# ch4r10t33r/zigz

Hardware: AMD Instinct MI355X
Metric: trace steps/sec proved (BabyBear, 2^20 RV64I trace) (higher is better)
Workload: dtype u32

## Files before the change

bindings/zig/zigz_hip.zig:

```

pub const Status = i32;
pub const BABYBEAR_P = 2013265921;
pub const NUM_COLUMNS = 43;
pub const HASH_SIZE = 32;
pub const ABI_VERSION = 1;
pub const NO_MEM_ACCESS = 4294967295;
pub const NO_MEM_ACCESS16 = 134217727;
pub const RCCL_UNIQUE_ID_BYTES = 128;
pub const BATCH_MAX = 4096;
pub const VERIFY_BATCH_MAX = 4194304;

pub const OK: Status = 0;
pub const ERR_EMPTY_EVALUATIONS: Status = 1;
pub const ERR_LENGTH_NOT_POWER_OF_TWO: Status = 2;
pub const ERR_WRONG_NUMBER_OF_VARIABLES: Status = 3;
pub const ERR_NO_VARIABLES_TO_FIX: Status = 4;
pub const ERR_NO_VARIABLES: Status = 5;
pub const ERR_PROTOCOL_ERROR: Status = 6;
pub const ERR_EMPTY_VALUES: Status = 7;
pub const ERR_TOO_MANY_VALUES: Status = 8;
pub const ERR_INDEX_OUT_OF_BOUNDS: Status = 9;
pub const ERR_POINT_DIMENSION_MISMATCH: Status = 10;
pub const ERR_NO_QUERIES: Status = 11;
pub const ERR_TOO_MANY_QUERIES: Status = 12;
// ... 108 lines not shown
    structure_us: f64,
    list_hash_us: f64,
    list_hash_perms: u64,
    top_us: f64,
    top_perms: u64,
    rebuilds: u64,
    eval_constant_columns: u64,
};
pub const BenchResult = extern struct {
    avg_us: f64,
    min_us: f64,
    max_us: f64,
    algorithmic_bytes: u64,
    units: u64,
    launches: u32,
};
pub const LaunchRec = extern struct {
    cls: u32,
    reserved: u32,
    perms: u64,
    start_us: f64,
    end_us: f64,
};

pub extern "c" fn zigz_abi_version() u32;
pub extern "c" fn zigz_status_name(s: Status) [*c]const u8;
pub extern "c" fn zigz_device_count(count: [*c]c_int) Status;
pub extern "c" fn zigz_ctx_create(device: c_int, out: [*c]?*Ctx) Status;
pub extern "c" fn zigz_device_set_blocking_sync(device: c_int, on: c_int) Status;
pub extern "c" fn zigz_ctx_destroy(ctx: ?*Ctx) void;
pub extern "c" fn zigz_last_error(ctx: ?*const Ctx) [*c]const u8;
pub extern "c" fn zigz_ctx_set_stream(ctx: ?*Ctx, hip_stream: ?*anyopaque) Status;
pub extern "c" fn zigz_ctx_get_stream(ctx: ?*Ctx) ?*anyopaque;
pub extern "c" fn zigz_ctx_synchronize(ctx: ?*Ctx) Status;
pub extern "c" fn zigz_dev_alloc(ctx: ?*Ctx, bytes: usize, d_out: [*c]?*anyopaque) Status;
pub extern "c" fn zigz_dev_free(ctx: ?*Ctx, d_ptr: ?*anyopaque) Status;
pub extern "c" fn zigz_ctx_release_workspaces(ctx: ?*Ctx) Status;
pub extern "c" fn zigz_dev_mem_info(ctx: ?*Ctx, free_bytes: [*c]usize, total_bytes: [*c]usize) Status;
pub extern "c" fn zigz_dev_upload_u64(ctx: ?*Ctx, h_in: [*c]const u64, n: usize, d_out: [*c]u32) Status;
pub extern "c" fn zigz_dev_download_u64(ctx: ?*Ctx, d_in: [*c]const u32, n: usize, h_out: [*c]u64) Status;
pub extern "c" fn zigz_mle_bind(ctx: ?*Ctx, in: [*c]const u64, n: usize, r: u64, out: [*c]u64) Status;
pub extern "c" fn zigz_mle_round_poly(ctx: ?*Ctx, in: [*c]const u64, n: usize, out: [*c]u64) Status;
pub extern "c" fn zigz_mle_sum(ctx: ?*Ctx, in: [*c]const u64, n: usize, out: [*c]u64) Status;
pub extern "c" fn zigz_mle_eval(ctx: ?*Ctx, in: [*c]const u64, n: usize, point: [*c]const u64, point_len: usize, out: [*c]u64) Status;
pub extern "c" fn zigz_sumcheck_prove(ctx: ?*Ctx, in: [*c]const u64, n: usize, rounds: [*c]u64, point: [*c]u64, final_eval: [*c]u64) Status;
pub extern "c" fn zigz_sumcheck_prove_interactive(ctx: ?*Ctx, in: [*c]const u64, n: usize, challenges: [*c]const u64, n_challenges: usize, rounds: [*c]u64, point: [*c]u64, final_eval: [*c]u64) Status;
pub extern "c" fn zigz_merkle_commit(ctx: ?*Ctx, values: [*c]const u64, n: usize, root: [*c]u8, height: [*c]usize, out: [*c]?*Merkle) Status;
pub extern "c" fn zigz_merkle_open(ctx: ?*Ctx, tree: ?*const Merkle, index: usize, siblings: [*c]u8, dirs: [*c]u8, leaf_value: [*c]u64) Status;
pub extern "c" fn zigz_merkle_destroy(ctx: ?*Ctx, tree: ?*Merkle) void;
pub extern "c" fn zigz_commit_open(ctx: ?*Ctx, evals: [*c]const u64, n: usize, tree: ?*const Merkle, point: [*c]const u64, point_len: usize, value: [*c]u64, index: [*c]u64, siblings: [*c]u8, dirs: [*c]u8, leaf_value: [*c]u64) Status;
pub extern "c" fn zigz_commit_begin(ctx: ?*Ctx, cols: [*c]const u64, ncols: usize, col_stride: usize, nv: usize, out: [*c]?*CommitJob) Status;
pub extern "c" fn zigz_commit_begin_dev(ctx: ?*Ctx, d_cols: [*c]const u32, ncols: usize, col_stride: usize, nv: usize, out: [*c]?*CommitJob) Status;
pub extern "c" fn zigz_commit_begin_batch(ctx: ?*Ctx, d_cols: [*c][*c]u32, nproofs: usize, ncols: usize, col_stride: usize, nv: usize, out: [*c]?*CommitJob) Status;
pub extern "c" fn zigz_commit_roots(job: ?*CommitJob, roots: [*c]u8) Status;
pub extern "c" fn zigz_commit_open_all(job: ?*CommitJob, points: [*c]const u64, values: [*c]u64, indices: [*c]u64, leaves: [*c]u64, siblings: [*c]u8, dirs: [*c]u8) Status;
pub extern "c" fn zigz_commit_job_tree(job: ?*CommitJob, d_tree: [*c]?*anyopaque, bytes_per_column: [*c]usize) Status;
pub extern "c" fn zigz_commit_end(job: ?*CommitJob) void;
pub extern "c" fn zigz_lasso_prove(ctx: ?*Ctx, table: [*c]const u64, table_rows: usize, queries: [*c]const u64, n_queries: usize, n_in: usize, n_out: usize, nv_out: [*c]usize, rounds: [*c]u64, point: [*c]u64, final_eval: [*c]u64, query_commitment: [*c]u8, table_commitment: [*c]u8) Status;
pub extern "c" fn zigz_lasso_prove_with_mapping(ctx: ?*Ctx, table: [*c]const u64, table_rows: usize, queries: [*c]const u64, n_queries: usize, n_in: usize, n_out: usize, mapping: [*c]const u64, n_mapping: usize, nv_out: [*c]usize, rounds: [*c]u64, point: [*c]u64, final_eval: [*c]u64, query_commitment: [*c]u8, table_commitment: [*c]u8) Status;
pub extern "c" fn zigz_lasso_fingerprints(ctx: ?*Ctx, rows_in: [*c]const u64, rows: usize, width: usize, out: [*c]u64) Status;
pub extern "c" fn zigz_dev_reduce_u64(ctx: ?*Ctx, h_in: [*c]const u64, n: usize, d_out: [*c]u32) Status;
pub extern "c" fn zigz_dev_witness_from_rows(ctx: ?*Ctx, h_rows: [*c]const u64, num_steps: usize, nv: usize, d_cols: [*c]u32, col_stride: usize) Status;
pub extern "c" fn zigz_dev_witness_from_steps(ctx: ?*Ctx, h_steps: [*c]const TraceStep, num_steps: usize, nv: usize, initial_regs: [*c]const u64, d_cols: [*c]u32, col_stride: usize) Status;
pub extern "c" fn zigz_dev_witness_from_steps_async(ctx: ?*Ctx, h_steps: [*c]const TraceStep, num_steps: usize, nv: usize, initial_regs: [*c]const u64, d_cols: [*c]u32, col_stride: usize) Status;
pub extern "c" fn zigz_dev_witness_from_steps_ws(ctx: ?*Ctx, h_steps: [*c]const TraceStep, num_steps: usize, nv: usize, initial_regs: [*c]const u64, d_cols: [*c][*c]u32, col_stride: [*c]usize) Status;
pub extern "c" fn zigz_dev_witness_from_steps32(ctx: ?*Ctx, h_steps: [*c]const TraceStep32, num_steps: usize, h_mem: [*c]const MemAccess, num_mem: usize, nv: usize, initial_regs: [*c]const u64, d_cols: [*c]u32, col_stride: usize) Status;
pub extern "c" fn zigz_dev_witness_from_steps32_ws(ctx: ?*Ctx, h_steps: [*c]const TraceStep32, num_steps: usize, h_mem: [*c]const MemAccess, num_mem: usize, nv: usize, initial_regs: [*c]const u64, d_cols: [*c][*c]u32, col_stride: [*c]usize) Status;
pub extern "c" fn zigz_dev_witness_from_steps16(ctx: ?*Ctx, h_steps: [*c]const TraceStep16, num_steps: usize, h_mem: [*c]const MemAccess, num_mem: usize, code_base: u64, h_code: [*c]const CodeEntry, num_code: usize, nv: usize, initial_regs: [*c]const u64, d_cols: [*c]u32, col_stride: usize) Status;
pub extern "c" fn zigz_dev_witness_from_steps16_ws(ctx: ?*Ctx, h_steps: [*c]const TraceStep16, num_steps: usize, h_mem: [*c]const MemAccess, num_mem: usize, code_base: u64, h_code: [*c]const CodeEntry, num_code: usize, nv: usize, initial_regs: [*c]const u64, d_cols: [*c][*c]u32, col_stride: [*c]usize) Status;
pub extern "c" fn zigz_host_register(ctx: ?*Ctx, h_ptr: ?*anyopaque, bytes: usize) Status;
pub extern "c" fn zigz_host_unregister(ctx: ?*Ctx, h_ptr: ?*anyopaque) Status;
pub extern "c" fn zigz_dev_mle_bind(ctx: ?*Ctx, d_in: [*c]const u32, n: usize, r: u64, d_out: [*c]u32) Status;
pub extern "c" fn zigz_dev_mle_bind_sums(ctx: ?*Ctx, d_in: [*c]const u32, n: usize, r: u64, d_out: [*c]u32, half_sums: [*c]u64) Status;
pub extern "c" fn zigz_dev_mle_half_sums(ctx: ?*Ctx, d_in: [*c]const u32, n: usize, half_sums: [*c]u64) Status;
pub extern "c" fn zigz_dev_mle_eval(ctx: ?*Ctx, d_in: [*c]const u32, n: usize, point: [*c]const u64, point_len: usize, out: [*c]u64) Status;
pub extern "c" fn zigz_dev_sumcheck_prove(ctx: ?*Ctx, d_in: [*c]const u32, n: usize, d_scratch: [*c]u32, fixed_challenges: [*c]const u64, rounds: [*c]u64, point: [*c]u64, final_eval: [*c]u64) Status;
pub extern "c" fn zigz_dev_sumcheck_prove_sharded(ctx: ?*Ctx, d_local: [*c]const u32, n_local: usize, rank: c_int, world: c_int, allgather: AllgatherFn, user: ?*anyopaque, rounds: [*c]u64, point: [*c]u64, final_eval: [*c]u64) Status;
pub extern "c" fn zigz_shm_comm_create(name: [*c]const u8, rank: c_int, world: c_int, max_bytes: usize, timeout_s: f64, out: [*c]?*ShmComm) Status;
pub extern "c" fn zigz_shm_allgather(comm: ?*anyopaque, send: ?*const anyopaque, bytes: usize, recv: ?*anyopaque) c_int;
pub extern "c" fn zigz_shm_comm_destroy(comm: ?*ShmComm) void;
pub extern "c" fn zigz_rccl_unique_id(id: [*c]u8) Status;
pub extern "c" fn zigz_rccl_comm_create(device: c_int, id: [*c]const u8, rank: c_int, world: c_int, max_bytes: usize, out: [*c]?*RcclComm) Status;
pub extern "c" fn zigz_rccl_allgather(comm: ?*anyopaque, send: ?*const anyopaque, bytes: usize, recv: ?*anyopaque) c_int;
pub extern "c" fn zigz_rccl_allreduce_u64(comm: ?*RcclComm, send: [*c]const u64, n: usize, recv: [*c]u64) c_int;
pub extern "c" fn zigz_rccl_allreduce_u64_dev(comm: ?*RcclComm, d_words: [*c]u64, n: usize, hip_stream: ?*anyopaque) c_int;
pub extern "c" fn zigz_rccl_stream_wait(comm: ?*RcclComm, hip_stream: ?*anyopaque) c_int;
pub extern "c" fn zigz_rccl_comm_set_timeout(comm: ?*RcclComm, seconds: f64) void;
pub extern "c" fn zigz_rccl_comm_abort(comm: ?*RcclComm) void;
pub extern "c" fn zigz_rccl_comm_rank(comm: ?*const RcclComm) c_int;
pub extern "c" fn zigz_rccl_comm_world(comm: ?*const RcclComm) c_int;
pub extern "c" fn zigz_rccl_comm_destroy(comm: ?*RcclComm) void;
pub extern "c" fn zigz_dev_sumcheck_prove_rccl(ctx: ?*Ctx, d_local: [*c]const u32, n_local: usize, comm: ?*RcclComm, rounds: [*c]u64, point: [*c]u64, final_eval: [*c]u64) Status;
pub extern "c" fn zigz_sumcheck_radix_run(ops: [*c]const RadixOps, n_local: usize, rank: c_int, world: c_int, allgather: AllgatherFn, comm_user: ?*anyopaque, fixed_challenges: [*c]const u64, rounds: [*c]u64, point: [*c]u64, final_eval: [*c]u64) Status;
pub extern "c" fn zigz_sumcheck_radix_run_reduced(ops: [*c]const RadixOps, n_local: usize, rank: c_int, world: c_int, allgather: AllgatherFn, comm_user: ?*anyopaque, fixed_challenges: [*c]const u64, rounds: [*c]u64, point: [*c]u64, final_eval: [*c]u64) Status;
pub extern "c" fn zigz_dev_sumcheck_prove_batch(ctx: ?*Ctx, d_tables: [*c][*c]u32, ns: [*c]const usize, k: usize, fixed_challenges: [*c]const u64, rounds: [*c]u64, points: [*c]u64, final_evals: [*c]u64, bad_index: [*c]usize) Status;
pub extern "c" fn zigz_sumcheck_prove_batch(ctx: ?*Ctx, tables: [*c][*c]u64, ns: [*c]const usize, k: usize, fixed_challenges: [*c]const u64, rounds: [*c]u64, points: [*c]u64, final_evals: [*c]u64, bad_index: [*c]usize) Status;
pub extern "c" fn zigz_lasso_prove_batch(ctx: ?*Ctx, k: usize, tables: [*c][*c]u64, table_rows: [*c]const usize, queries: [*c][*c]u64, n_queries: [*c]const usize, n_in: [*c]const usize, n_out: [*c]const usize, mappings: [*c][*c]u64, n_mappings: [*c]const usize, nv_out: [*c]usize, rounds: [*c][*c]u64, points: [*c][*c]u64, final_evals: [*c]u64, query_commitments: [*c]u8, table_commitments: [*c]u8, bad_index: [*c]usize) Status;
pub extern "c" fn zigz_sumcheck_radix_run_batch(user: ?*anyopaque, block_sums: RadixBatchSumsFn, fold: RadixBatchFoldFn, read_tail: RadixBatchTailFn, k: usize, ns: [*c]const usize, fixed_challenges: [*c]const u64, rounds: [*c]u64, points: [*c]u64, final_evals: [*c]u64) Status;
pub extern "c" fn zigz_dev_merkle_commit_batch(ctx: ?*Ctx, d_values: [*c][*c]u32, ns: [*c]const usize, k: usize, roots: [*c]u8, heights: [*c]usize, out: [*c]?*MerkleBatch, bad_index: [*c]usize) Status;
pub extern "c" fn zigz_merkle_commit_batch(ctx: ?*Ctx, values: [*c][*c]u64, ns: [*c]const usize, k: usize, roots: [*c]u8, heights: [*c]usize, out: [*c]?*MerkleBatch, bad_index: [*c]usize) Status;
pub extern "c" fn zigz_merkle_open_batch(ctx: ?*Ctx, b: ?*const MerkleBatch, indices: [*c]const u64, siblings: [*c]u8, dirs: [*c]u8, leaf_values: [*c]u64, bad_index: [*c]usize) Status;
pub extern "c" fn zigz_commit_open_batch(ctx: ?*Ctx, b: ?*const MerkleBatch, points: [*c]const u64, values: [*c]u64, indices: [*c]u64, siblings: [*c]u8, dirs: [*c]u8, leaf_values: [*c]u64, bad_index: [*c]usize) Status;
pub extern "c" fn zigz_merkle_batch_destroy(ctx: ?*Ctx, b: ?*MerkleBatch) void;
pub extern "c" fn zigz_merkle_verify_batch(ctx: ?*Ctx, k: usize, roots: [*c]const u8, heights: [*c]const usize, leaf_values: [*c]const u64, siblings: [*c]const u8, dirs: [*c]const u8, verdicts: [*c]u8, n_rejected: [*c]usize, bad_index: [*c]usize) Status;
pub extern "c" fn zigz_dev_merkle_verify_batch(ctx: ?*Ctx, k: usize, d_roots: [*c]const u8, heights: [*c]const usize, d_leaf_values: [*c]const u64, d_siblings: [*c]const u8, d_dirs: [*c]const u8, verdicts: [*c]u8, n_rejected: [*c]usize, bad_index: [*c]usize) Status;
pub extern "c" fn zigz_transcript_new() ?*Transcript;
// ... 20 lines not shown
```

include/zigz_hip.h:

```cpp
#ifndef ZIGZ_HIP_H
#define ZIGZ_HIP_H

#include <stddef.h>
#include <stdint.h>

#ifdef __cplusplus
extern "C" {
#endif

#define ZIGZ_BABYBEAR_P 2013265921ull
#define ZIGZ_NUM_COLUMNS 43
#define ZIGZ_HASH_SIZE 32
#define ZIGZ_ABI_VERSION 1

typedef int32_t zigz_status;
enum {
    ZIGZ_OK = 0,
    ZIGZ_ERR_EMPTY_EVALUATIONS = 1,
    ZIGZ_ERR_LENGTH_NOT_POWER_OF_TWO = 2,
    ZIGZ_ERR_WRONG_NUMBER_OF_VARIABLES = 3,
    ZIGZ_ERR_NO_VARIABLES_TO_FIX = 4,
    ZIGZ_ERR_NO_VARIABLES = 5,
    ZIGZ_ERR_PROTOCOL_ERROR = 6,
    ZIGZ_ERR_EMPTY_VALUES = 7,
// ... 16 lines not shown
    ZIGZ_ERR_COMM = 105
};

typedef struct zigz_ctx zigz_ctx;
typedef struct zigz_merkle zigz_merkle;
typedef struct zigz_commit_job zigz_commit_job;
typedef struct zigz_transcript zigz_transcript;
typedef struct zigz_merkle_batch zigz_merkle_batch;

uint32_t zigz_abi_version(void);
const char *zigz_status_name(zigz_status s);
zigz_status zigz_device_count(int *count);
zigz_status zigz_ctx_create(int device, zigz_ctx **out);
zigz_status zigz_device_set_blocking_sync(int device, int on);
void zigz_ctx_destroy(zigz_ctx *ctx);
const char *zigz_last_error(const zigz_ctx *ctx);
zigz_status zigz_ctx_set_stream(zigz_ctx *ctx, void *hip_stream);
void *zigz_ctx_get_stream(zigz_ctx *ctx);
zigz_status zigz_ctx_synchronize(zigz_ctx *ctx);
zigz_status zigz_dev_alloc(zigz_ctx *ctx, size_t bytes, void **d_out);
zigz_status zigz_dev_free(zigz_ctx *ctx, void *d_ptr);
zigz_status zigz_ctx_release_workspaces(zigz_ctx *ctx);
zigz_status zigz_dev_mem_info(zigz_ctx *ctx, size_t *free_bytes, size_t *total_bytes);
zigz_status zigz_dev_upload_u64(zigz_ctx *ctx, const uint64_t *h_in, size_t n, uint32_t *d_out);
zigz_status zigz_dev_download_u64(zigz_ctx *ctx, const uint32_t *d_in, size_t n, uint64_t *h_out);

zigz_status zigz_mle_bind(zigz_ctx *ctx, const uint64_t *in, size_t n, uint64_t r, uint64_t *out);
zigz_status zigz_mle_round_poly(zigz_ctx *ctx, const uint64_t *in, size_t n, uint64_t out[2]);
zigz_status zigz_mle_sum(zigz_ctx *ctx, const uint64_t *in, size_t n, uint64_t *out);
zigz_status zigz_mle_eval(zigz_ctx *ctx, const uint64_t *in, size_t n, const uint64_t *point,
                          size_t point_len, uint64_t *out);

zigz_status zigz_sumcheck_prove(zigz_ctx *ctx, const uint64_t *in, size_t n, uint64_t *rounds,
                                uint64_t *point, uint64_t *final_eval);
zigz_status zigz_sumcheck_prove_interactive(zigz_ctx *ctx, const uint64_t *in, size_t n,
                                            const uint64_t *challenges, size_t n_challenges,
                                            uint64_t *rounds, uint64_t *point, uint64_t *final_eval);

zigz_status zigz_merkle_commit(zigz_ctx *ctx, const uint64_t *values, size_t n, uint8_t root[32],
                               size_t *height, zigz_merkle **out);
zigz_status zigz_merkle_open(zigz_ctx *ctx, const zigz_merkle *tree, size_t index, uint8_t *siblings,
                             uint8_t *dirs, uint64_t *leaf_value);
void zigz_merkle_destroy(zigz_ctx *ctx, zigz_merkle *tree);
zigz_status zigz_commit_open(zigz_ctx *ctx, const uint64_t *evals, size_t n, const zigz_merkle *tree,
                             const uint64_t *point, size_t point_len, uint64_t *value, uint64_t *index,
                             uint8_t *siblings, uint8_t *dirs, uint64_t *leaf_value);

zigz_status zigz_commit_begin(zigz_ctx *ctx, const uint64_t *cols, size_t ncols, size_t col_stride,
                              size_t nv, zigz_commit_job **out);
zigz_status zigz_commit_begin_dev(zigz_ctx *ctx, const uint32_t *d_cols, size_t ncols, size_t col_stride,
                                  size_t nv, zigz_commit_job **out);
zigz_status zigz_commit_begin_batch(zigz_ctx *ctx, const uint32_t *const *d_cols, size_t nproofs, size_t ncols,
                                    size_t col_stride, size_t nv, zigz_commit_job **out);
zigz_status zigz_commit_roots(zigz_commit_job *job, uint8_t *roots);
zigz_status zigz_commit_open_all(zigz_commit_job *job, const uint64_t *points, uint64_t *values,
                                 uint64_t *indices, uint64_t *leaves, uint8_t *siblings, uint8_t *dirs);
zigz_status zigz_commit_job_tree(zigz_commit_job *job, const void **d_tree, size_t *bytes_per_column);
void zigz_commit_end(zigz_commit_job *job);

zigz_status zigz_lasso_prove(zigz_ctx *ctx, const uint64_t *table, size_t table_rows, const uint64_t *queries,
                             size_t n_queries, size_t n_in, size_t n_out, size_t *nv_out, uint64_t *rounds,
                             uint64_t *point, uint64_t *final_eval, uint8_t query_commitment[32],
                             uint8_t table_commitment[32]);
zigz_status zigz_lasso_prove_with_mapping(zigz_ctx *ctx, const uint64_t *table, size_t table_rows,
                                          const uint64_t *queries, size_t n_queries, size_t n_in, size_t n_out,
                                          const uint64_t *mapping, size_t n_mapping, size_t *nv_out,
                                          uint64_t *rounds, uint64_t *point, uint64_t *final_eval,
                                          uint8_t query_commitment[32], uint8_t table_commitment[32]);
zigz_status zigz_lasso_fingerprints(zigz_ctx *ctx, const uint64_t *rows_in, size_t rows, size_t width,
                                    uint64_t *out);

zigz_status zigz_dev_reduce_u64(zigz_ctx *ctx, const uint64_t *h_in, size_t n, uint32_t *d_out);
zigz_status zigz_dev_witness_from_rows(zigz_ctx *ctx, const uint64_t *h_rows, size_t num_steps, size_t nv,
                                       uint32_t *d_cols, size_t col_stride);

typedef struct zigz_trace_step {
    uint64_t pc;
    uint64_t rd_value;
    uint64_t mem_addr;
    uint64_t mem_value;
    int64_t imm;
    uint8_t opcode, rd, rs1, rs2, funct3, funct7;
    uint8_t wr_reg;
    uint8_t mem_is_read;
} zigz_trace_step;
zigz_status zigz_dev_witness_from_steps(zigz_ctx *ctx, const zigz_trace_step *h_steps, size_t num_steps, size_t nv,
                                        const uint64_t *initial_regs, uint32_t *d_cols, size_t col_stride);
zigz_status zigz_dev_witness_from_steps_async(zigz_ctx *ctx, const zigz_trace_step *h_steps, size_t num_steps, size_t nv,
                                              const uint64_t *initial_regs, uint32_t *d_cols, size_t col_stride);
zigz_status zigz_dev_witness_from_steps_ws(zigz_ctx *ctx, const zigz_trace_step *h_steps, size_t num_steps, size_t nv,
                                           const uint64_t *initial_regs, const uint32_t **d_cols, size_t *col_stride);
typedef struct zigz_trace_step32 {
    uint64_t pc;
    uint64_t rd_value;
    int32_t imm;
    uint32_t mem_index;
    uint8_t opcode, rd, rs1, rs2, funct3, funct7;
    uint8_t wr_reg;
    uint8_t mem_is_read;
} zigz_trace_step32;
typedef struct zigz_mem_access {
    uint64_t addr, value;
} zigz_mem_access;
#define ZIGZ_NO_MEM_ACCESS 4294967295
zigz_status zigz_dev_witness_from_steps32(zigz_ctx *ctx, const zigz_trace_step32 *h_steps, size_t num_steps,
                                          const zigz_mem_access *h_mem, size_t num_mem, size_t nv, const uint64_t *initial_regs,
// ... 190 lines not shown
```

zigz_amd/_ffi.py:

```python
import ctypes as C
import os

HERE = os.path.dirname(os.path.abspath(__file__))
LIB_PATH = os.path.join(HERE, "lib", "libzigz_hip.so")

if not os.path.exists(LIB_PATH):
    raise ImportError(
        f"{LIB_PATH} is missing: build it with `python -m zigz_amd.build` (hipcc, --offload-arch=gfx950). "
        "zigz_amd has no CPU fallback.")

lib = C.CDLL(LIB_PATH, mode=C.RTLD_GLOBAL)

u64p = C.POINTER(C.c_uint64)
u32p = C.POINTER(C.c_uint32)
u8p = C.POINTER(C.c_uint8)
szp = C.POINTER(C.c_size_t)
vp = C.c_void_p


class LaunchRec(C.Structure):
    _fields_ = [("cls", C.c_uint32), ("reserved", C.c_uint32), ("perms", C.c_uint64), ("start_us", C.c_double), ("end_us", C.c_double)]


class KernelStats(C.Structure):
# ... 11 lines not shown
                ("small_domain_fallback_waves", C.c_uint64),
                ("structure_us", C.c_double), ("list_hash_us", C.c_double), ("list_hash_perms", C.c_uint64),
                ("top_us", C.c_double), ("top_perms", C.c_uint64), ("rebuilds", C.c_uint64),
                ("eval_constant_columns", C.c_uint64)]


class BenchResult(C.Structure):
    _fields_ = [("avg_us", C.c_double), ("min_us", C.c_double), ("max_us", C.c_double), ("algorithmic_bytes", C.c_uint64),
                ("units", C.c_uint64), ("launches", C.c_uint32)]


ALLGATHER_FN = C.CFUNCTYPE(C.c_int, vp, vp, C.c_size_t, vp)
RADIX_BLOCK_SUMS_FN = C.CFUNCTYPE(C.c_int32, vp, C.c_uint, u64p)
RADIX_FOLD_FN = C.CFUNCTYPE(C.c_int32, vp, C.c_uint, u64p, C.c_uint, u64p)
RADIX_READ_TAIL_FN = C.CFUNCTYPE(C.c_int32, vp, C.c_size_t, u64p)


class RadixOps(C.Structure):
    _fields_ = [("user", vp), ("block_sums", RADIX_BLOCK_SUMS_FN), ("fold", RADIX_FOLD_FN), ("read_tail", RADIX_READ_TAIL_FN)]


RB_BLOCK_SUMS_FN = C.CFUNCTYPE(C.c_int32, vp, C.c_size_t, szp, C.POINTER(C.c_uint), u64p)
RB_FOLD_FN = C.CFUNCTYPE(C.c_int32, vp, C.c_size_t, szp, C.POINTER(C.c_uint), u64p, C.POINTER(C.c_uint), u64p)
RB_READ_TAIL_FN = C.CFUNCTYPE(C.c_int32, vp, C.c_size_t, szp, szp, u64p)


SIGNATURES = {
    "zigz_abi_version": (C.c_uint32, []),
    "zigz_status_name": (C.c_char_p, [C.c_int32]),
    "zigz_device_count": (C.c_int32, [C.POINTER(C.c_int)]),
    "zigz_ctx_create": (C.c_int32, [C.c_int, C.POINTER(vp)]),
    "zigz_ctx_destroy": (None, [vp]),
    "zigz_last_error": (C.c_char_p, [vp]),
    "zigz_ctx_set_stream": (C.c_int32, [vp, vp]),
    "zigz_ctx_get_stream": (vp, [vp]),
    "zigz_ctx_synchronize": (C.c_int32, [vp]),
    "zigz_dev_alloc": (C.c_int32, [vp, C.c_size_t, C.POINTER(vp)]),
    "zigz_dev_free": (C.c_int32, [vp, vp]),
    "zigz_dev_upload_u64": (C.c_int32, [vp, u64p, C.c_size_t, vp]),
    "zigz_dev_download_u64": (C.c_int32, [vp, vp, C.c_size_t, u64p]),
    "zigz_mle_bind": (C.c_int32, [vp, u64p, C.c_size_t, C.c_uint64, u64p]),
    "zigz_mle_round_poly": (C.c_int32, [vp, u64p, C.c_size_t, u64p]),
    "zigz_mle_sum": (C.c_int32, [vp, u64p, C.c_size_t, u64p]),
    "zigz_mle_eval": (C.c_int32, [vp, u64p, C.c_size_t, u64p, C.c_size_t, u64p]),
    "zigz_sumcheck_prove": (C.c_int32, [vp, u64p, C.c_size_t, u64p, u64p, u64p]),
    "zigz_sumcheck_prove_interactive": (C.c_int32, [vp, u64p, C.c_size_t, u64p, C.c_size_t, u64p, u64p, u64p]),
    "zigz_merkle_commit": (C.c_int32, [vp, u64p, C.c_size_t, u8p, szp, C.POINTER(vp)]),
    "zigz_merkle_open": (C.c_int32, [vp, vp, C.c_size_t, u8p, u8p, u64p]),
    "zigz_merkle_destroy": (None, [vp, vp]),
    "zigz_commit_open": (C.c_int32, [vp, u64p, C.c_size_t, vp, u64p, C.c_size_t, u64p, u64p, u8p, u8p, u64p]),
    "zigz_commit_begin": (C.c_int32, [vp, u64p, C.c_size_t, C.c_size_t, C.c_size_t, C.POINTER(vp)]),
    "zigz_commit_begin_dev": (C.c_int32, [vp, vp, C.c_size_t, C.c_size_t, C.c_size_t, C.POINTER(vp)]),
    "zigz_commit_begin_batch": (C.c_int32, [vp, C.POINTER(vp), C.c_size_t, C.c_size_t, C.c_size_t, C.c_size_t, C.POINTER(vp)]),
    "zigz_commit_roots": (C.c_int32, [vp, u8p]),
    "zigz_commit_open_all": (C.c_int32, [vp, u64p, u64p, u64p, u64p, u8p, u8p]),
    "zigz_commit_job_tree": (C.c_int32, [vp, C.POINTER(vp), C.POINTER(C.c_size_t)]),
    "zigz_commit_end": (None, [vp]),
    "zigz_lasso_prove": (C.c_int32, [vp, u64p, C.c_size_t, u64p, C.c_size_t, C.c_size_t, C.c_size_t, szp, u64p, u64p,
                                     u64p, u8p, u8p]),
    "zigz_lasso_prove_with_mapping": (C.c_int32, [vp, u64p, C.c_size_t, u64p, C.c_size_t, C.c_size_t, C.c_size_t, u64p,
                                                  C.c_size_t, szp, u64p, u64p, u64p, u8p, u8p]),
    "zigz_lasso_fingerprints": (C.c_int32, [vp, u64p, C.c_size_t, C.c_size_t, u64p]),
    "zigz_dev_reduce_u64": (C.c_int32, [vp, u64p, C.c_size_t, vp]),
    "zigz_dev_witness_from_rows": (C.c_int32, [vp, u64p, C.c_size_t, C.c_size_t, vp, C.c_size_t]),
    "zigz_dev_witness_from_steps": (C.c_int32, [vp, vp, C.c_size_t, C.c_size_t, u64p, vp, C.c_size_t]),
    "zigz_dev_witness_from_steps_async": (C.c_int32, [vp, vp, C.c_size_t, C.c_size_t, u64p, vp, C.c_size_t]),
    "zigz_dev_witness_from_steps32": (C.c_int32, [vp, vp, C.c_size_t, vp, C.c_size_t, C.c_size_t, u64p, vp, C.c_size_t]),
    "zigz_dev_witness_from_steps32_ws": (C.c_int32, [vp, vp, C.c_size_t, vp, C.c_size_t, C.c_size_t, u64p, C.POINTER(vp), szp]),
    "zigz_dev_witness_from_steps16": (C.c_int32, [vp, vp, C.c_size_t, vp, C.c_size_t, C.c_uint64, vp, C.c_size_t, C.c_size_t, u64p, vp, C.c_size_t]),
    "zigz_dev_witness_from_steps16_ws": (C.c_int32, [vp, vp, C.c_size_t, vp, C.c_size_t, C.c_uint64, vp, C.c_size_t, C.c_size_t, u64p,
                                                     C.POINTER(vp), szp]),
    "zigz_dev_witness_from_steps_ws": (C.c_int32, [vp, vp, C.c_size_t, C.c_size_t, u64p, C.POINTER(vp), szp]),
    "zigz_dev_mem_info": (C.c_int32, [vp, szp, szp]),
    "zigz_ctx_set_epoch": (C.c_int32, [vp, vp]),
    "zigz_ctx_launch_log": (C.c_int32, [vp, C.POINTER(LaunchRec), C.c_size_t, szp]),
    "zigz_ctx_release_workspaces": (C.c_int32, [vp]),
    "zigz_host_register": (C.c_int32, [vp, vp, C.c_size_t]),
    "zigz_host_unregister": (C.c_int32, [vp, vp]),
    "zigz_dev_mle_bind": (C.c_int32, [vp, vp, C.c_size_t, C.c_uint64, vp]),
    "zigz_dev_mle_bind_sums": (C.c_int32, [vp, vp, C.c_size_t, C.c_uint64, vp, u64p]),
    "zigz_dev_mle_half_sums": (C.c_int32, [vp, vp, C.c_size_t, u64p]),
    "zigz_dev_mle_eval": (C.c_int32, [vp, vp, C.c_size_t, u64p, C.c_size_t, u64p]),
    "zigz_dev_sumcheck_prove": (C.c_int32, [vp, vp, C.c_size_t, vp, u64p, u64p, u64p, u64p]),
    "zigz_dev_sumcheck_prove_sharded": (C.c_int32, [vp, vp, C.c_size_t, C.c_int, C.c_int, ALLGATHER_FN, vp, u64p, u64p, u64p]),
    "zigz_sumcheck_radix_run": (C.c_int32, [C.POINTER(RadixOps), C.c_size_t, C.c_int, C.c_int, ALLGATHER_FN, vp, u64p, u64p,
                                            u64p, u64p]),
    "zigz_sumcheck_radix_run_reduced": (C.c_int32, [C.POINTER(RadixOps), C.c_size_t, C.c_int, C.c_int, ALLGATHER_FN, vp, u64p, u64p,
                                                    u64p, u64p]),
    "zigz_shm_comm_create": (C.c_int32, [C.c_char_p, C.c_int, C.c_int, C.c_size_t, C.c_double, C.POINTER(vp)]),
    "zigz_shm_allgather": (C.c_int, [vp, vp, C.c_size_t, vp]),
    "zigz_shm_comm_destroy": (None, [vp]),
    "zigz_rccl_unique_id": (C.c_int32, [u8p]),
    "zigz_rccl_comm_create": (C.c_int32, [C.c_int, u8p, C.c_int, C.c_int, C.c_size_t, C.POINTER(vp)]),
    "zigz_rccl_allgather": (C.c_int, [vp, vp, C.c_size_t, vp]),
    "zigz_rccl_allreduce_u64": (C.c_int, [vp, u64p, C.c_size_t, u64p]),
    "zigz_rccl_allreduce_u64_dev": (C.c_int, [vp, vp, C.c_size_t, vp]),
    "zigz_rccl_stream_wait": (C.c_int, [vp, vp]),
    "zigz_rccl_comm_set_timeout": (None, [vp, C.c_double]),
    "zigz_rccl_comm_abort": (None, [vp]),
    "zigz_rccl_comm_rank": (C.c_int, [vp]),
    "zigz_rccl_comm_world": (C.c_int, [vp]),
    "zigz_rccl_comm_destroy": (None, [vp]),
    "zigz_dev_sumcheck_prove_batch": (C.c_int32, [vp, C.POINTER(vp), szp, C.c_size_t, u64p, u64p, u64p, u64p, szp]),
    "zigz_sumcheck_prove_batch": (C.c_int32, [vp, C.POINTER(u64p), szp, C.c_size_t, u64p, u64p, u64p, u64p, szp]),
    "zigz_lasso_prove_batch": (C.c_int32, [vp, C.c_size_t, C.POINTER(u64p), szp, C.POINTER(u64p), szp, szp, szp, C.POINTER(u64p), szp,
                                           szp, C.POINTER(u64p), C.POINTER(u64p), u64p, u8p, u8p, szp]),
# ... 36 lines not shown
```

zigz_amd/build.py:

```python
import os
import shutil
import subprocess
import sys

HERE = os.path.dirname(os.path.abspath(__file__))
ROOT = os.path.dirname(HERE)
CSRC = os.path.join(HERE, "csrc")
LIB = os.path.join(HERE, "lib")
OBJ = os.path.join(HERE, "build")
INC = os.path.join(ROOT, "include")
ARCH = "gfx950"


def _hipcc():
    for c in (shutil.which("hipcc"), "/opt/rocm/bin/hipcc"):
        if c and os.path.exists(c):
            return c
    raise RuntimeError("hipcc not found: the HIP backend cannot be built")


def _newer(target, sources):
    if not os.path.exists(target):
        return True
    t = os.path.getmtime(target)
    return any(os.path.getmtime(s) > t for s in sources)


def _run(cmd):
    print("+", " ".join(cmd), flush=True)
    subprocess.check_call(cmd)


def _headers():
    hs = [os.path.join(INC, f) for f in os.listdir(INC) if f.endswith(".h")]
    for d, _, fs in os.walk(CSRC):
        hs += [os.path.join(d, f) for f in fs if f.endswith(".hpp")]
    return hs


def _host_cxx():
    for c in ("/opt/rocm/lib/llvm/bin/clang++", "/opt/rocm/bin/amdclang++"):
        if os.path.exists(c):
            return c
    return "g++"


def build_hip(force=False):
    os.makedirs(LIB, exist_ok=True)
    os.makedirs(OBJ, exist_ok=True)
    hipcc = _hipcc()
    hdrs = _headers()
    objs = []
    extra = os.environ.get("ZIGZ_EXTRA_HIPCC_FLAGS", "").split()
    units = [
        ("kernels.hip", [hipcc, f"--offload-arch={ARCH}", "-O3", "-std=c++17", "-fPIC", f"-I{INC}", f"-I{CSRC}"] + extra),
        ("merkle_levels.hip", [hipcc, f"--offload-arch={ARCH}", "-O3", "-std=c++17", "-fPIC", f"-I{INC}", f"-I{CSRC}"] + extra),
        ("sumcheck_batch.hip", [hipcc, f"--offload-arch={ARCH}", "-O3", "-std=c++17", "-fPIC", f"-I{INC}", f"-I{CSRC}"] + extra),
        ("merkle_batch.hip", [hipcc, f"--offload-arch={ARCH}", "-O3", "-std=c++17", "-fPIC", f"-I{INC}", f"-I{CSRC}"] + extra),
        ("merkle_verify.hip", [hipcc, f"--offload-arch={ARCH}", "-O3", "-std=c++17", "-fPIC", f"-I{INC}", f"-I{CSRC}"] + extra),
        ("api.cpp", [hipcc, "-O3", "-std=c++17", "-fPIC", f"-I{INC}", f"-I{CSRC}"]),
        ("api_mle.cpp", [hipcc, "-O3", "-std=c++17", "-fPIC", f"-I{INC}", f"-I{CSRC}"]),
        ("api_commit.cpp", [hipcc, "-O3", "-std=c++17", "-fPIC", f"-I{INC}", f"-I{CSRC}"]),
        ("api_misc.cpp", [hipcc, "-O3", "-std=c++17", "-fPIC", f"-I{INC}", f"-I{CSRC}"]),
        ("api_batch.cpp", [hipcc, "-O3", "-std=c++17", "-fPIC", "-pthread", f"-I{INC}", f"-I{CSRC}"]),
        ("api_merkle_batch.cpp", [hipcc, "-O3", "-std=c++17", "-fPIC", "-pthread", f"-I{INC}", f"-I{CSRC}"]),
        ("api_merkle_verify.cpp", [hipcc, "-O3", "-std=c++17", "-fPIC", "-pthread", f"-I{INC}", f"-I{CSRC}"]),
        ("host_hash.cpp", [_host_cxx(), "-O3", "-std=c++17", "-fPIC", f"-I{CSRC}"]),
        ("host_keccak_avx512.cpp", [_host_cxx(), "-O3", "-std=c++17", "-fPIC", f"-I{CSRC}"]),
        ("host_keccak_bmi.cpp", [_host_cxx(), "-O3", "-std=c++17", "-fPIC", f"-I{CSRC}"]),
        ("host_keccak_avx512vl.cpp", [_host_cxx(), "-O3", "-std=c++17", "-fPIC", f"-I{CSRC}"]),
        ("host_sponge_batch.cpp", [_host_cxx(), "-O3", "-std=c++17", "-fPIC", "-pthread", f"-I{CSRC}"]),
        ("shm_comm.cpp", [_host_cxx(), "-O2", "-std=c++17", "-fPIC", f"-I{INC}", f"-I{CSRC}"]),
        ("rccl_comm.cpp", [hipcc, "-O2", "-std=c++17", "-fPIC", f"-I{INC}", f"-I{CSRC}", "-I/opt/rocm/include"]),
    ]
    for src, cmd in units:
        s = os.path.join(CSRC, src)
        o = os.path.join(OBJ, src.replace(".", "_") + ".o")
        if force or _newer(o, [s] + hdrs):
            _run(cmd + ["-c", s, "-o", o])
        objs.append(o)
    so = os.path.join(LIB, "libzigz_hip.so")
    if force or _newer(so, objs):
        _run([hipcc, f"--offload-arch={ARCH}", "-shared", "-fPIC", "-o", so] + objs + ["-lrt", "-pthread", "-ldl"])
    return so


def build_host(force=False):
    hdir = os.path.join(CSRC, "host")
    if not os.path.isdir(hdir):
        return None
    srcs = sorted(os.path.join(hdir, f) for f in os.listdir(hdir) if f.endswith(".cpp"))
    if not srcs:
        return None
    so = os.path.join(LIB, "libzigz_host.so")
    if force or _newer(so, srcs + _headers() + [os.path.join(LIB, "libzigz_hip.so")]):
        _run(["g++", "-O3", "-std=c++17", "-fPIC", "-pthread", "-shared", f"-I{INC}", f"-I{CSRC}", "-o", so] + srcs +
             [f"-L{LIB}", "-lzigz_hip", "-Wl,-rpath,$ORIGIN"])
    return so


def build_all(force=False):
    a = build_hip(force)
    b = build_host(force)
    return a, b


if __name__ == "__main__":
    print(build_all("--force" in sys.argv))
```

zigz_amd/csrc/api.cpp:

```cpp
#include "api_internal.hpp"

using namespace zk;

void set_err(zigz_ctx *ctx, const char *fmt, ...) {
    if (!ctx) return;
    va_list ap;
    va_start(ap, fmt);
    vsnprintf(ctx->err, sizeof(ctx->err), fmt, ap);
    va_end(ap);
}

zigz_status ws_get(zigz_ctx *ctx, int slot, size_t bytes, void **out) {
    if (bytes == 0) bytes = 16;
    if (ctx->ws_bytes[slot] < bytes) {
        if (ctx->ws[slot]) {
            HIPCHK(ctx, hipStreamSynchronize(ctx->stream));
            HIPCHK(ctx, hipFree(ctx->ws[slot]));
            ctx->ws[slot] = nullptr;
            ctx->ws_bytes[slot] = 0;
        }
        size_t want = align256(bytes + bytes / 8);
        hipError_t e = hipMalloc(&ctx->ws[slot], want);
        if (e != hipSuccess) {
            (void)hipGetLastError();
// ... 249 lines not shown
            ctx->ws[i] = nullptr;
            ctx->ws_bytes[i] = 0;
        }
    ctx->cons_table = nullptr;
    ctx->cons_table_bytes = 0;
    return ZIGZ_OK;
}
extern "C" zigz_status zigz_dev_mem_info(zigz_ctx *ctx, size_t *free_bytes, size_t *total_bytes) {
    ZIGZ_ENTER(ctx);
    if (!ctx || !free_bytes || !total_bytes) return ZIGZ_ERR_INVALID_ARGUMENT;
    HIPCHK(ctx, hipMemGetInfo(free_bytes, total_bytes));
    return ZIGZ_OK;
}
extern "C" zigz_status zigz_dev_free(zigz_ctx *ctx, void *d_ptr) {
    ZIGZ_ENTER(ctx);
    if (!ctx) return ZIGZ_ERR_INVALID_ARGUMENT;
    HIPCHK(ctx, hipStreamSynchronize(ctx->stream));
    HIPCHK(ctx, hipFree(d_ptr));
    return ZIGZ_OK;
}

extern "C" zigz_status zigz_ctx_enable_timing(zigz_ctx *ctx, int enable) {
    ZIGZ_ENTER(ctx);
    if (!ctx) return ZIGZ_ERR_INVALID_ARGUMENT;
    ctx->timing = enable != 0;
    if (enable) ctx->events_recorded = true;
    return ZIGZ_OK;
}
extern "C" zigz_status zigz_ctx_set_option(zigz_ctx *ctx, const char *name, int64_t value) {
    if (!ctx || !name) return ZIGZ_ERR_INVALID_ARGUMENT;
    if (strcmp(name, "per_round_sumcheck") == 0) { ctx->per_round_sumcheck = value != 0; return ZIGZ_OK; }
    if (strcmp(name, "fold_eval") == 0) { ctx->fold_eval = value != 0; return ZIGZ_OK; }
    if (strcmp(name, "merkle_dedup") == 0) { ctx->run_aware_mask = value != 0 ? ~0ull : 0; return ZIGZ_OK; }
    if (strcmp(name, "run_aware_mask") == 0) { ctx->run_aware_mask = (uint64_t)value; return ZIGZ_OK; }
    if (strcmp(name, "run_aware_materialize") == 0) { ctx->run_aware_materialize = value != 0; return ZIGZ_OK; }
    if (strcmp(name, "cons_group_mask") == 0) { ctx->cons_group_mask = (uint64_t)value; return ZIGZ_OK; }
    if (strcmp(name, "cons_always") == 0) { ctx->cons_always = value != 0; return ZIGZ_OK; }
    if (strcmp(name, "debug_skip") == 0) { ctx->debug_skip = (int)value; return ZIGZ_OK; }
    if (strcmp(name, "small_domain_mask") == 0) { ctx->small_domain_mask = (uint64_t)value; return ZIGZ_OK; }
    if (strcmp(name, "verify_pause") == 0) { ctx->verify_pause = value == 1 ? 1 : value == 2 ? 2 : 0; return ZIGZ_OK; }
    if (strcmp(name, "batch_reserve") == 0) { ctx->batch_reserve = value < 0 ? 0 : value > BATCH_MAX ? BATCH_MAX : (unsigned)value; return ZIGZ_OK; }
    return ZIGZ_ERR_INVALID_ARGUMENT;
}
extern "C" zigz_status zigz_ctx_get_option(zigz_ctx *ctx, const char *name, int64_t *value) {
    if (!ctx || !name || !value) return ZIGZ_ERR_INVALID_ARGUMENT;
    if (strcmp(name, "per_round_sumcheck") == 0) { *value = ctx->per_round_sumcheck; return ZIGZ_OK; }
    if (strcmp(name, "fold_eval") == 0) { *value = ctx->fold_eval; return ZIGZ_OK; }
    if (strcmp(name, "run_aware_mask") == 0) { *value = (int64_t)ctx->run_aware_mask; return ZIGZ_OK; }
    if (strcmp(name, "run_aware_materialize") == 0) { *value = ctx->run_aware_materialize; return ZIGZ_OK; }
    if (strcmp(name, "cons_group_mask") == 0) { *value = (int64_t)ctx->cons_group_mask; return ZIGZ_OK; }
    if (strcmp(name, "cons_always") == 0) { *value = ctx->cons_always; return ZIGZ_OK; }
    if (strcmp(name, "small_domain_mask") == 0) { *value = (int64_t)ctx->small_domain_mask; return ZIGZ_OK; }
    if (strcmp(name, "verify_pause") == 0) { *value = ctx->verify_pause; return ZIGZ_OK; }
    return ZIGZ_ERR_INVALID_ARGUMENT;
}
extern "C" zigz_status zigz_ctx_set_epoch(zigz_ctx *ctx, zigz_ctx *owner) {
    ZIGZ_ENTER(ctx);
    if (!ctx || !owner || owner->device != ctx->device) return ZIGZ_ERR_INVALID_ARGUMENT;
    if (owner == ctx) {
        HIPCHK(ctx, hipEventRecord(ctx->epoch_own, ctx->stream));
        HIPCHK(ctx, hipEventSynchronize(ctx->epoch_own));
    }
    ctx->epoch = owner->epoch_own;
    return ZIGZ_OK;
}
extern "C" zigz_status zigz_ctx_launch_log(zigz_ctx *ctx, zigz_launch_rec *out, size_t cap, size_t *n) {
    if (!ctx || !n || (cap && !out)) return ZIGZ_ERR_INVALID_ARGUMENT;
    const size_t k = (size_t)ctx->log_n < cap ? (size_t)ctx->log_n : cap;
    if (k) memcpy(out, ctx->log, k * sizeof(zigz_launch_rec));
    *n = (size_t)ctx->log_n;
    return ZIGZ_OK;
}
zigz_status log_launch(zigz_ctx *ctx, int cls, uint64_t perms, hipEvent_t start, hipEvent_t stop, hipEvent_t first, double *dur_us) {
    float d = 0, b = 0;
    HIPCHK(ctx, hipEventElapsedTime(&d, start, stop));
    *dur_us = (double)d * 1000.0;
    if (ctx->log_n >= KEV_MAX + 2) return ZIGZ_OK;
    const hipEvent_t origin = ctx->epoch ? ctx->epoch : first;
    if (origin == stop || hipEventElapsedTime(&b, origin, stop) != hipSuccess) {
        (void)hipGetLastError();
        b = origin == start ? d : 0.0f;
    }
    zigz_launch_rec &r = ctx->log[ctx->log_n++];
    r.cls = (uint32_t)cls;
    r.reserved = 0;
    r.perms = perms;
    r.end_us = (double)b * 1000.0;
    r.start_us = r.end_us - *dur_us;
    return ZIGZ_OK;
}
extern "C" zigz_status zigz_ctx_get_stats(zigz_ctx *ctx, zigz_kernel_stats *out) {
    ZIGZ_ENTER(ctx);
    if (!ctx || !out) return ZIGZ_ERR_INVALID_ARGUMENT;
    *out = ctx->stats;
    return ZIGZ_OK;
}

zigz_status upload_u64(zigz_ctx *ctx, const uint64_t *h_in, size_t n, uint32_t *d_out, bool reduce) {
    if (n == 0) return ZIGZ_OK;
    void *d64;
    CHK(ws_get(ctx, WS_IN64, n * sizeof(uint64_t), &d64));
    HIPCHK(ctx, hipMemcpyAsync(d64, h_in, n * sizeof(uint64_t), hipMemcpyHostToDevice, ctx->stream));
    if (reduce) {
        launch_reduce_u64((const uint64_t *)d64, d_out, n, ctx->stream);
        HIPCHK(ctx, hipGetLastError());
        return ZIGZ_OK;
// ... 258 lines not shown
```

zigz_amd/csrc/api_commit.cpp:

```cpp
#include "api_internal.hpp"

using namespace zk;

static void caps_for(zigz_ctx *ctx, size_t npad, unsigned rn, unsigned gn) {
    ListCaps &c = ctx->caps;
    if (c.npad == npad && c.rn == rn && c.gn == gn) return;
    c.npad = npad;
    c.rn = rn;
    c.gn = gn;
    c.g_slabs = false;
    c.g_drops = c.g_skip = c.g_kept = 0;
    memset(c.r_last, 0, sizeof(c.r_last));
    memset(c.g_last, 0, sizeof(c.g_last));
    c.last_dropped = false;
    const LevelLists rw = runs_lists(npad, rn ? rn : 1), gw = cons_lists(npad);
    for (unsigned l = 0; l < RUN_MAX_LEVELS; l++) {
        c.r[l] = l <= rw.top ? (rw.cap[l] / 8 > 256 ? rw.cap[l] / 8 : 256) : 0;
        c.g[l] = l <= gw.top ? 256 : 0;
    }
}

zigz_status build_trees(zigz_ctx *ctx, const uint32_t *d_vals, size_t val_stride, size_t n_values, size_t npad,
                               uint8_t *d_slab, size_t ncols, bool record, TreeRef *ref) {
    const unsigned height = log2_floor(npad);
// ... 64 lines not shown
    if (whole || !lists) {
        nslab = ncols;
        for (size_t c = 0; c < ncols && c < 64; c++) t.slab_of_col[c] = (signed char)c;
    } else {
        for (size_t c = 0; c < ncols; c++) {
            const int kd = kind(c);
            if (kd == 0 || kd == 1 || (kd == 3 && ctx->caps.g_slabs)) t.slab_of_col[c] = (signed char)nslab++;
        }
    }
    if (d_slab) t.slab = d_slab;
    else if (nslab) {
        void *w;
        CHK(ws_get(ctx, WS_TREE, nslab * stride * 32, &w));
        t.slab = (uint8_t *)w;
    }
    auto slab_map = [&](const ColMap &m) {
        ColMap o{};
        o.n = m.n;
        for (unsigned k = 0; k < m.n; k++) o.c[k] = (uint8_t)t.slab_of_col[m.c[k]];
        return o;
    };
    if (H.n == 0 && R.n == 0 && G.n == 0) {
        launch_keccak_leaves(d_vals, val_stride, n_values, npad, t.slab, stride, ncols, ctx->stream, stamp(0, (uint64_t)ncols * npad));
    } else if (D.n) {
        const ColMap ds = slab_map(D);
        launch_keccak_leaves(d_vals, val_stride, n_values, npad, t.slab, stride, ncols, ctx->stream, stamp(0, (uint64_t)D.n * npad), &D, &ds);
    }
    void *sd_todo = nullptr;
    if (H.n || GS.n) {
        if (!ctx->d_sd_tables) {
            HIPCHK(ctx, hipMalloc((void **)&ctx->d_sd_tables, SD_TABLE_BYTES));
            HIPCHK(ctx, hipMalloc((void **)&ctx->d_sd_fallbacks, 64));
            launch_sd_tables(ctx->d_sd_tables, ctx->stream);
        }
        CHK(ws_get(ctx, WS_DEDUP, (sd_todo_words(npad, H.n) + sd_todo_words(npad, GS.n)) * 4, &sd_todo));
    }
    if (H.n || GS.n || R.n || G.n)
        launch_zero_counters((H.n || GS.n) ? ctx->d_sd_fallbacks : nullptr, R.n ? r_ctr : nullptr,
                             G.n ? g_ctr : nullptr, ctx->stream);
    if (H.n) {
        const ColMap hs = slab_map(H);
        launch_keccak_small_l01(d_vals, val_stride, n_values, npad, t.slab, stride, H, ctx->d_sd_tables, ctx->d_sd_fallbacks,
                                (uint32_t *)sd_todo, ctx->stream, stamp(3, 0), !virt, nullptr, &hs);
        if (virt)
            for (unsigned k = 0; k < H.n; k++) t.virtual_leaves |= 1ull << H.c[k];
        ctx->stats.small_domain_columns = H.n;
    }
    MerkleBuild b{};
    unsigned top = 0;
    if (lists) {
        top = run_top_level(npad);
        t.lists = 1;
        t.top = top;
        b.vals = d_vals;
        b.val_stride = val_stride;
        b.n_values = n_values;
        b.npad = npad;
        b.rcols = R;
        b.gcols = G;
        b.gcols_sd = GS;
        uint64_t level_nodes = 0;
        for (unsigned l = 0; l <= top; l++) level_nodes += npad >> l;
        const bool keep = ref != nullptr;
        const size_t upper_bytes = ncols * 512 * 32;
        if (R.n) {
            t.r_lists = runs_lists(npad, R.n, ref ? ctx->caps.r : nullptr);
            unsigned long long uoff[RUN_MAX_LEVELS] = {0};
            const size_t units = runs_units(npad, R.n, uoff);
            for (unsigned l = 0; l < RUN_MAX_LEVELS; l++) t.ubase_off[l] = uoff[l];
            const size_t list_bytes = (size_t)t.r_lists.entries * 4, stage_bytes = runs_stage_scratch_bytes(npad, R.n);
            const size_t meta_n = runs_meta_words(npad, R.n);
            const size_t kept = meta_n * 12 + units * 4 + 64 + (size_t)t.r_lists.entries * 32 + 64;
            void *w, *mw;
            CHK(ws_get(ctx, WS_RUNS, ((list_bytes + 63) & ~(size_t)63) + stage_bytes + 64 + (keep ? 0 : kept), &w));
            b.r_list = (uint32_t *)w;
            b.r_stage = (uint8_t *)w + ((list_bytes + 63) & ~(size_t)63);
            if (keep) CHK(ws_get(ctx, WS_RUNMETA, kept + upper_bytes, &mw));
            else mw = (uint8_t *)w + ((((list_bytes + 63) & ~(size_t)63) + stage_bytes + 64 + 63) & ~(size_t)63);
            uint8_t *q = (uint8_t *)mw;
            t.bitmap = (unsigned long long *)q; q += meta_n * 8;
            t.prev = (unsigned short *)q; q += meta_n * 2;
            t.woff = (unsigned short *)q; q += meta_n * 2;
            t.ubase = (uint32_t *)q; q += (units * 4 + 63) & ~(size_t)63;
            t.r_store = q; q += (size_t)t.r_lists.entries * 32;
            if (keep) t.upper = (uint8_t *)mw + kept;
            t.ncols = R.n;
            for (unsigned y = 0; y < R.n; y++) t.y_of_col[R.c[y]] = (signed char)y;
            b.r_ctr = r_ctr;
            ctx->stats.run_aware_columns = R.n;
            ctx->stats.run_aware_dense_nodes = (uint64_t)R.n * level_nodes;
        }
        if (G.n) {
            t.g_lists = cons_lists(npad, ref ? ctx->caps.g : nullptr);
            const size_t key_bytes = 2 * npad * 8, idx_bytes = 2 * npad * 4, list_bytes = ((size_t)t.g_lists.entries * 4 + 63) & ~(size_t)63;
            const size_t kept = 2 * npad * 4 + (size_t)t.g_lists.entries * G.n * 32 + 64;
            const bool upper_here = keep && !R.n;
            void *w, *mw;
            CHK(ws_get(ctx, WS_CONS, key_bytes + idx_bytes + list_bytes + 64 + (keep ? 0 : kept), &w));
            b.g_keys = (unsigned long long *)w;
            b.g_idx = (uint32_t *)((uint8_t *)w + key_bytes);
            b.g_list = (uint32_t *)((uint8_t *)w + key_bytes + idx_bytes);
            if (keep) CHK(ws_get(ctx, WS_CONSMETA, kept + (upper_here ? upper_bytes : 0), &mw));
            else mw = (uint8_t *)w + ((key_bytes + idx_bytes + list_bytes + 64 + 63) & ~(size_t)63);
            b.g_rep = (uint32_t *)mw;
            t.g_rep = b.g_rep;
            t.g_store = (uint8_t *)mw + 2 * npad * 4;
            if (upper_here) t.upper = (uint8_t *)mw + kept;
            if (ctx->cons_table != w || ctx->cons_table_bytes != ctx->ws_bytes[WS_CONS] || ctx->cons_gen + RUN_MAX_LEVELS + 1 >= 4096) {
// ... 187 lines not shown
    HIPCHK(ctx, hipMemcpyAsync(hl.data(), d_leaf, leaf_b, hipMemcpyDeviceToHost, ctx->stream));
    HIPCHK(ctx, hipStreamSynchronize(ctx->stream));
    for (size_t c = 0; c < ncols; c++) leaves[c] = hl[c];
    return ZIGZ_OK;
    ZIGZ_NOTHROW_END(ctx)
}

extern "C" zigz_status zigz_merkle_open(zigz_ctx *ctx, const zigz_merkle *t, size_t index, uint8_t *siblings,
                                        uint8_t *dirs, uint64_t *leaf_value) {
    ZIGZ_ENTER(ctx);
    if (!ctx || !t || !leaf_value) return ZIGZ_ERR_INVALID_ARGUMENT;
    if (index >= t->n_values) return ZIGZ_ERR_INDEX_OUT_OF_BOUNDS;
    if (t->height && (!siblings || !dirs)) return ZIGZ_ERR_INVALID_ARGUMENT;
    uint64_t idx = index;
    return open_paths(ctx, slab_tree_ref(t->d_tree, t->npad), t->height, t->d_vals, t->n_values, &idx, 1, siblings, dirs, leaf_value);
}

extern "C" zigz_status zigz_commit_open(zigz_ctx *ctx, const uint64_t *evals, size_t n, const zigz_merkle *tree,
                                        const uint64_t *point, size_t point_len, uint64_t *value, uint64_t *index,
                                        uint8_t *siblings, uint8_t *dirs, uint64_t *leaf_value) {
    ZIGZ_ENTER(ctx);
    if (!ctx || !tree || !value || !index || !leaf_value) return ZIGZ_ERR_INVALID_ARGUMENT;
    CHK(mle_check(n));
    if (point_len != log2_floor(n)) return ZIGZ_ERR_POINT_DIMENSION_MISMATCH;
    const uint32_t *d_ev = tree->d_vals;
    if (evals) {
        uint32_t *d;
        CHK(stage_in(ctx, evals, n, &d));
        d_ev = d;
    } else if (tree->n_values != n) {
        return ZIGZ_ERR_INVALID_ARGUMENT;
    }
    CHK(zigz_dev_mle_eval(ctx, d_ev, n, point, point_len, value));
    size_t idx = point_len == 0 ? 0 : (size_t)(point[0] % ((uint64_t)1 << point_len));
    *index = idx;
    return zigz_merkle_open(ctx, tree, idx, siblings, dirs, leaf_value);
}

struct zigz_commit_job {
    zigz_ctx *ctx;
    size_t ncols, nv, N, col_stride;
    const uint32_t *d_cols;
    int state;
    hipEvent_t built;
    uint64_t const_cols;
    uint64_t roots_seq;
    TreeRef tree;
    bool whole;
    uint64_t m_small, m_run, m_cons;
    bool m_whole;
    uint64_t run_cols, run_dense, sd_cols, cons_hinted, cons_levels_nodes, cons_sd, perms0;
    unsigned nz;
    size_t ncols1, zstride;
    size_t off_r_ctr, off_g_ctr;
    bool no_eval_skip;
};

static zigz_status job_build(zigz_commit_job *job) {
    zigz_ctx *ctx = job->ctx;
    const size_t ncols = job->ncols, nv = job->nv;
    CHK(timed_begin(ctx, 2));
    job->whole = job->m_whole;
    {
        const uint64_t s0 = ctx->small_domain_mask, r0 = ctx->run_aware_mask, c0 = ctx->cons_group_mask;
        const bool w0 = ctx->run_aware_materialize;
        ctx->small_domain_mask = job->m_small;
        ctx->run_aware_mask = job->m_run;
        ctx->cons_group_mask = job->m_cons;
        ctx->run_aware_materialize = job->m_whole;
        const zigz_status bs = build_trees(ctx, job->d_cols, job->col_stride, job->N, job->N, nullptr, ncols, ctx->timing, &job->tree);
        ctx->small_domain_mask = s0;
        ctx->run_aware_mask = r0;
        ctx->cons_group_mask = c0;
        ctx->run_aware_materialize = w0;
        CHK(bs);
    }
    if (ctx->timing) HIPCHK(ctx, hipEventRecord(ctx->ev[3], ctx->stream));
    const DoneFlag done = done_flag(ctx, 0);
    job->roots_seq = done.seq;
    launch_job_summary(job->tree, (unsigned)nv, ctx->h_roots, ncols,
                       ctx->stats.run_aware_columns ? ctx->d_run_count : nullptr,
                       (ctx->stats.small_domain_columns || ctx->build_cons_sd) ? ctx->d_sd_fallbacks : nullptr,
                       ctx->build_cons_hinted ? ctx->d_cons_count : nullptr, ctx->stream, done);
    HIPCHK(ctx, hipGetLastError());
    HIPCHK(ctx, hipEventRecord(job->built, ctx->stream));
    job->run_cols = ctx->stats.run_aware_columns;
    job->run_dense = ctx->stats.run_aware_dense_nodes;
    job->sd_cols = ctx->stats.small_domain_columns;
    job->cons_hinted = ctx->build_cons_hinted;
    job->cons_levels_nodes = ctx->build_cons_levels_nodes;
    job->cons_sd = ctx->build_cons_sd;
    job->perms0 = (uint64_t)ncols * (2 * job->N - 1) - job->sd_cols * (job->N + job->N / 2);
    job->no_eval_skip = ctx->debug_skip == 2;
    return ZIGZ_OK;
}

static zigz_status job_begin(zigz_ctx *ctx, const uint32_t *d_cols, size_t ncols, size_t col_stride, size_t nv,
                             zigz_commit_job **out) {
    if (ctx->active_job) {
        set_err(ctx, "a commit job is already active on this context");
        return ZIGZ_ERR_BAD_STATE;
    }
    zigz_commit_job *job = new (std::nothrow) zigz_commit_job();
    if (!job) return ZIGZ_ERR_OUT_OF_MEMORY;
    memset(job, 0, sizeof(*job));
    job->ctx = ctx;
    job->ncols = ncols;
    job->nv = nv;
    job->N = (size_t)1 << nv;
    job->col_stride = col_stride;
    job->d_cols = d_cols;
    job->m_small = ctx->small_domain_mask;
    job->m_run = ctx->run_aware_mask;
    job->m_cons = ctx->cons_group_mask;
    job->m_whole = ctx->run_aware_materialize;
    auto body = [&]() -> zigz_status {
        HIPCHK(ctx, hipEventCreateWithFlags(&job->built, hipEventDisableTiming));
        return job_build(job);
    };
    zigz_status st = body();
    if (st != ZIGZ_OK) {
        if (job->built) (void)hipEventDestroy(job->built);
        delete job;
        return st;
    }
    ctx->active_job = job;
    *out = job;
    return ZIGZ_OK;
}

static zigz_status job_build_batch_arena(zigz_commit_job *job, const uint32_t *const *srcs, size_t src_stride) {
    zigz_ctx *ctx = job->ctx;
    const size_t nc = job->ncols1, N = job->N, npad = N;
    const unsigned nz = job->nz, height = (unsigned)job->nv;
    ColMap R{}, G{};
    for (size_t c = 0; c < nc; c++) {
        if ((job->m_cons >> c) & 1) G.c[G.n++] = (uint8_t)c;
        else if ((job->m_run >> c) & 1) R.c[R.n++] = (uint8_t)c;
        else return ZIGZ_ERR_INVALID_ARGUMENT;
    }
    const size_t stride = N;
    TreeRef t{};
    t.npad = npad;
    for (int c = 0; c < 64; c++) {
        t.slab_of_col[c] = -1;
        t.y_of_col[c] = -1;
        t.g_j_of_col[c] = -1;
    }
    t.lists = 1;
    t.top = run_top_level(npad);
    size_t at = 0;
    auto take = [&](size_t bytes) { const size_t o = at; at += align256(bytes); return o; };
    const size_t o_cols = take(nc * stride * 4);
    const size_t o_rctr = take(RUN_CTR_WORDS * 8), o_gctr = take(RUN_CTR_WORDS * 8);
    size_t o_rlist = 0, o_rstage = 0, o_bitmap = 0, o_prev = 0, o_woff = 0, o_ubase = 0, o_rstore = 0;
    size_t meta_n = 0;
    if (R.n) {
        t.r_lists = runs_lists(npad, R.n, nullptr);
        unsigned long long uoff[RUN_MAX_LEVELS] = {0};
        const size_t units = runs_units(npad, R.n, uoff);
        for (unsigned l = 0; l < RUN_MAX_LEVELS; l++) t.ubase_off[l] = uoff[l];
        meta_n = runs_meta_words(npad, R.n);
        o_rlist = take((size_t)t.r_lists.entries * 4);
        o_rstage = take(runs_stage_scratch_bytes(npad, R.n) + 64);
        o_bitmap = take(meta_n * 8);
        o_prev = take(meta_n * 2);
        o_woff = take(meta_n * 2);
        o_ubase = take(units * 4 + 64);
        o_rstore = take((size_t)t.r_lists.entries * 32);
        t.ncols = R.n;
        for (unsigned y = 0; y < R.n; y++) t.y_of_col[R.c[y]] = (signed char)y;
    }
    size_t o_keys = 0, o_idx = 0, o_glist = 0, o_grep = 0, o_gstore = 0, o_slab = 0;
    const size_t key_bytes = 2 * npad * 8;
    if (G.n) {
        t.g_lists = cons_lists(npad, nullptr);
        o_keys = take(key_bytes);
        o_idx = take(2 * npad * 4);
        o_glist = take((size_t)t.g_lists.entries * 4);
        o_grep = take(2 * npad * 4);
        o_gstore = take((size_t)t.g_lists.entries * G.n * 32);
        o_slab = take((size_t)G.n * tree_nodes(npad) * 32);
        t.g_ncols = G.n;
        for (unsigned k = 0; k < G.n; k++) {
            t.g_j_of_col[G.c[k]] = (signed char)k;
            t.slab_of_col[G.c[k]] = (signed char)k;
        }
    }
    const size_t o_upper = take(nc * 512 * 32);
    const size_t S = align256(at);
    if ((size_t)nz * S > ((size_t)48 << 30)) return ZIGZ_ERR_OUT_OF_MEMORY;
    void *w;
    const void *w_before = ctx->ws[WS_BATCH];
    const size_t n_res = nz > ctx->batch_reserve ? nz : ctx->batch_reserve;
    if ((size_t)n_res * S <= ((size_t)48 << 30)) CHK(ws_get(ctx, WS_BATCH, (size_t)n_res * S, &w));
    else CHK(ws_get(ctx, WS_BATCH, (size_t)nz * S, &w));
    uint8_t *a0 = (uint8_t *)w;
    if (G.n && (w != w_before || ctx->batch_tab_S != S || ctx->batch_tab_nz < nz || ctx->batch_tab_off != o_keys ||
                ctx->batch_gen == 0 || ctx->batch_gen + RUN_MAX_LEVELS + 1 >= 4096)) {
        const size_t n_tabs = ctx->ws_bytes[WS_BATCH] / S;
        HIPCHK(ctx, hipMemset2DAsync(a0 + o_keys, S, 0, key_bytes, n_tabs, ctx->stream));
        ctx->batch_tab_S = S;
        ctx->batch_tab_nz = (unsigned)n_tabs;
        ctx->batch_tab_off = o_keys;
        ctx->batch_gen = 1;
    }
    t.upper = a0 + o_upper;
    MerkleBuild b{};
    b.vals = (const uint32_t *)(a0 + o_cols);
    b.val_stride = stride;
    b.n_values = N;
    b.npad = npad;
    b.rcols = R;
    b.gcols = G;
    if (R.n) {
        t.bitmap = (unsigned long long *)(a0 + o_bitmap);
        t.prev = (unsigned short *)(a0 + o_prev);
        t.woff = (unsigned short *)(a0 + o_woff);
        t.ubase = (uint32_t *)(a0 + o_ubase);
        t.r_store = a0 + o_rstore;
        b.r_list = (uint32_t *)(a0 + o_rlist);
        b.r_stage = a0 + o_rstage;
        b.r_ctr = (unsigned long long *)(a0 + o_rctr);
    }
    if (G.n) {
        t.slab = a0 + o_slab;
        t.g_rep = (const uint32_t *)(a0 + o_grep);
        t.g_store = a0 + o_gstore;
        t.g_dropped = (const unsigned long long *)(a0 + o_gctr) + 8;
        b.g_keys = (unsigned long long *)(a0 + o_keys);
        b.g_idx = (uint32_t *)(a0 + o_idx);
        b.g_list = (uint32_t *)(a0 + o_glist);
        b.g_rep = (uint32_t *)(a0 + o_grep);
        b.g_ctr = (unsigned long long *)(a0 + o_gctr);
        b.g_has_slabs = 1;
        b.g_gen = ctx->batch_gen;
        ctx->batch_gen += t.top + 1;
    }
    b.t = t;
    set_zstride(b, S, nz);
    t = b.t;
    ColSrcs cs{};
    for (unsigned z = 0; z < nz; z++) cs.p[z] = srcs[z];
    launch_gather_cols(cs, nz, nc, N, src_stride, (uint32_t *)(a0 + o_cols), stride, S, ctx->stream);
    launch_zero_counters(nullptr, R.n ? b.r_ctr : nullptr, G.n ? b.g_ctr : nullptr, ctx->stream, nz, S);
    if (ctx->debug_skip != 2) launch_structure(b, ctx->stream, ctx->debug_skip == 0);
    for (unsigned l = 0; l <= t.top; l++)
        if (ctx->debug_skip != 1) launch_level_hash(b, l, ctx->stream, nullptr, 0, ctx->debug_skip == 0);
    if (height && ctx->debug_skip != 1) launch_merkle_top(t, t.top, height, nc, ctx->stream, nullptr);
    HIPCHK(ctx, hipGetLastError());
    job->tree = t;
    job->d_cols = (const uint32_t *)(a0 + o_cols);
    job->col_stride = stride;
    job->zstride = S;
    job->off_r_ctr = o_rctr;
    job->off_g_ctr = o_gctr;
    job->whole = false;
    const DoneFlag done = done_flag(ctx, 0);
    job->roots_seq = done.seq;
    launch_job_summary(t, height, ctx->h_roots, nc, R.n ? b.r_ctr : nullptr, nullptr, G.n ? b.g_ctr : nullptr, ctx->stream, done);
    HIPCHK(ctx, hipGetLastError());
    HIPCHK(ctx, hipEventRecord(job->built, ctx->stream));
    uint64_t level_nodes = 0;
    for (unsigned l = 0; l <= t.top; l++) level_nodes += npad >> l;
    job->run_cols = R.n;
    job->run_dense = (uint64_t)R.n * level_nodes;
    job->sd_cols = 0;
    job->cons_hinted = G.n;
    job->cons_levels_nodes = level_nodes;
    job->cons_sd = 0;
    job->perms0 = (uint64_t)nc * (2 * N - 1);
    job->no_eval_skip = ctx->debug_skip == 2;
    return ZIGZ_OK;
}

extern "C" zigz_status zigz_commit_begin_batch(zigz_ctx *ctx, const uint32_t *const *d_cols, size_t nproofs, size_t ncols,
                                               size_t col_stride, size_t nv, zigz_commit_job **out) {
    ZIGZ_ENTER(ctx);
    if (!ctx || !d_cols || !out || ncols == 0 || nproofs == 0 || nproofs > BATCH_MAX || nv > 40) return ZIGZ_ERR_INVALID_ARGUMENT;
    if (ncols * nproofs > ROOTS_MAX_COLS || col_stride < ((size_t)1 << nv)) return ZIGZ_ERR_INVALID_ARGUMENT;
    for (size_t z = 0; z < nproofs; z++)
        if (!d_cols[z]) return ZIGZ_ERR_INVALID_ARGUMENT;
    if (nproofs == 1) return job_begin(ctx, d_cols[0], ncols, col_stride, nv, out);
    if (ctx->active_job) {
        set_err(ctx, "a commit job is already active on this context");
        return ZIGZ_ERR_BAD_STATE;
    }
    const size_t N = (size_t)1 << nv;
    const bool arena = N >= RUN_MIN_LEAVES && N <= ((size_t)1 << BATCH_ARENA_MAX_NV) && ncols <= 64 && (ctx->run_aware_mask || ctx->cons_group_mask);
    if (N >= RUN_MIN_LEAVES && !arena) return ZIGZ_ERR_INVALID_ARGUMENT;
    zigz_commit_job *job = new (std::nothrow) zigz_commit_job();
    if (!job) return ZIGZ_ERR_OUT_OF_MEMORY;
    memset(job, 0, sizeof(*job));
    job->ctx = ctx;
    job->nz = (unsigned)nproofs;
    job->ncols1 = ncols;
    job->ncols = ncols * nproofs;
    job->nv = nv;
    job->N = N;
    auto body = [&]() -> zigz_status {
        HIPCHK(ctx, hipEventCreateWithFlags(&job->built, hipEventDisableTiming));
        if (arena) {
            job->m_small = 0;
            job->m_run = ctx->run_aware_mask;
            job->m_cons = ctx->cons_group_mask;
            return job_build_batch_arena(job, d_cols, col_stride);
        }
        const size_t dstride = N < 4 ? 4 : N;
        void *d;
        CHK(ws_get(ctx, WS_COLS, (job->nz > ctx->batch_reserve ? job->nz : ctx->batch_reserve) * ncols * dstride * 4, &d));
        ColSrcs cs{};
        for (size_t z = 0; z < nproofs; z++) cs.p[z] = d_cols[z];
        launch_gather_cols(cs, job->nz, ncols, N, col_stride, (uint32_t *)d, dstride, ncols * dstride * 4, ctx->stream);
        HIPCHK(ctx, hipGetLastError());
        job->d_cols = (const uint32_t *)d;
        job->col_stride = dstride;
        job->m_small = job->m_run = job->m_cons = 0;
        job->m_whole = false;
        return job_build(job);
    };
    const zigz_status st = body();
    if (st != ZIGZ_OK) {
        if (job->built) (void)hipEventDestroy(job->built);
        delete job;
        return st;
    }
    ctx->active_job = job;
    *out = job;
    return ZIGZ_OK;
}

extern "C" zigz_status zigz_commit_begin_dev(zigz_ctx *ctx, const uint32_t *d_cols, size_t ncols, size_t col_stride,
                                             size_t nv, zigz_commit_job **out) {
    ZIGZ_ENTER(ctx);
    if (!ctx || !d_cols || !out || ncols == 0 || nv > 40) return ZIGZ_ERR_INVALID_ARGUMENT;
    if (ncols > ROOTS_MAX_COLS) return ZIGZ_ERR_INVALID_ARGUMENT;
    if (col_stride < ((size_t)1 << nv)) return ZIGZ_ERR_INVALID_ARGUMENT;
    return job_begin(ctx, d_cols, ncols, col_stride, nv, out);
}

extern "C" zigz_status zigz_commit_begin(zigz_ctx *ctx, const uint64_t *cols, size_t ncols, size_t col_stride,
                                         size_t nv, zigz_commit_job **out) {
    ZIGZ_ENTER(ctx);
    if (!ctx || !cols || !out || ncols == 0 || nv > 40) return ZIGZ_ERR_INVALID_ARGUMENT;
    if (ncols > ROOTS_MAX_COLS) return ZIGZ_ERR_INVALID_ARGUMENT;
    const size_t N = (size_t)1 << nv;
    if (col_stride < N) return ZIGZ_ERR_INVALID_ARGUMENT;
    if (ctx->active_job) return ZIGZ_ERR_BAD_STATE;
    const size_t dstride = N < 4 ? 4 : N;
    void *d;
    CHK(ws_get(ctx, WS_COLS, ncols * dstride * 4, &d));
    uint32_t *d_cols = (uint32_t *)d;
    if (col_stride == N && dstride == N) {
        CHK(upload_u64(ctx, cols, ncols * N, d_cols, false));
    } else {
        for (size_t c = 0; c < ncols; c++) CHK(upload_u64(ctx, cols + c * col_stride, N, d_cols + c * dstride, false));
    }
    return job_begin(ctx, d_cols, ncols, dstride, nv, out);
}

extern "C" zigz_status zigz_commit_roots(zigz_commit_job *job, uint8_t *roots) {
    if (job) ZIGZ_ENTER(job->ctx);
    if (!job || !roots) return ZIGZ_ERR_INVALID_ARGUMENT;
    zigz_ctx *ctx = job->ctx;
    if (job->state != 0) return ZIGZ_ERR_BAD_STATE;
    const unsigned long long *h_cnt = (const unsigned long long *)(ctx->h_roots + job->ncols * 32);
    for (int attempt = 0;; attempt++) {
        const unsigned long long *h_done = (const unsigned long long *)(ctx->h_roots + ROOTS_MAX_COLS * 32 + JOB_SUMMARY_WORDS * 8);
        if (!(g_sleep_wait.load() && !ctx->timing && sleep_wait(h_done, job->roots_seq)))
            HIPCHK(ctx, hipEventSynchronize(job->built));
        const unsigned long long flags = h_cnt[6];
        const bool r_over = (flags & 1) != 0, g_over = ((flags >> 8) & 1) != 0, g_noslab = ((flags >> 8) & 2) != 0;
        const bool dropped = h_cnt[4] != 0;
        ListCaps &c = ctx->caps;
        bool again = false;
        if (job->zstride) {
            for (unsigned z = 0; z < job->nz; z++)
                if (h_cnt[(size_t)z * JOB_SUMMARY_WORDS + 6]) {
                    set_err(ctx, "batched commit job: a list ran out of its worst-case room (proof %u)", z);
                    return ZIGZ_ERR_BAD_STATE;
                }
        } else if (job->tree.lists && c.npad == job->N) {
// ... 66 lines not shown
    ctx->stats.small_domain_fallback_waves = job->sd_cols ? h_cnt[1] : 0;
    ctx->stats.list_hash_perms = ctx->stats.run_aware_hashed;
    ctx->stats.cons_columns = ctx->stats.cons_dense_nodes = ctx->stats.cons_hashed = 0;
    ctx->stats.cons_probe_distinct = 0;
    if (job->cons_hinted) {
        ctx->stats.cons_probe_distinct = h_cnt[5];
        if (!h_cnt[4]) {
            ctx->stats.cons_columns = job->cons_hinted;
            ctx->stats.cons_dense_nodes = job->cons_hinted * job->cons_levels_nodes;
            ctx->stats.cons_hashed = h_cnt[3];
            ctx->stats.keccak_permutations -= ctx->stats.cons_dense_nodes - ctx->stats.cons_hashed;
            ctx->stats.list_hash_perms += ctx->stats.cons_hashed;
        } else {
            ctx->stats.small_domain_columns += job->cons_sd;
            ctx->stats.keccak_permutations -= job->cons_sd * (N + N / 2);
            ctx->stats.small_domain_fallback_waves += h_cnt[2];
            ctx->stats.list_hash_perms += job->cons_hinted * job->cons_levels_nodes - job->cons_sd * (N + N / 2);
        }
    }
    if (ctx->timing) {
        float ms = 0;
        HIPCHK(ctx, hipEventElapsedTime(&ms, ctx->ev[2], ctx->ev[3]));
        ctx->stats.merkle_build_us = (double)ms * 1000.0;
        CHK(keccak_times_collect(ctx));
    }
    job->state = 1;
    return ZIGZ_OK;
}

extern "C" zigz_status zigz_commit_open_all(zigz_commit_job *job, const uint64_t *points, uint64_t *values,
                                            uint64_t *indices, uint64_t *leaves, uint8_t *siblings, uint8_t *dirs) {
    ZIGZ_NOTHROW_BEGIN
    if (job) ZIGZ_ENTER(job->ctx);
    if (!job || !values || !indices || !leaves) return ZIGZ_ERR_INVALID_ARGUMENT;
    zigz_ctx *ctx = job->ctx;
    if (job->state != 1) return ZIGZ_ERR_BAD_STATE;
    const size_t nv = job->nv, ncols = job->ncols;
    if (nv && (!points || !siblings || !dirs)) return ZIGZ_ERR_INVALID_ARGUMENT;
    const size_t sib_b = ncols * nv * 32, leaf_b = ncols * 4, val_b = ncols * 4, dir_b = ncols * nv;
    const size_t out_b = sib_b + leaf_b + val_b + dir_b;
    if (out_b <= PIN_WORDS * 8 / 2 && nv * ncols * 4 + ncols * 8 <= PIN_WORDS * 8 / 2) {
        uint8_t *h = (uint8_t *)ctx->h_pin;
        uint8_t *z_sib = h;
        uint32_t *z_leaf = (uint32_t *)(h + sib_b), *z_val = z_leaf + ncols;
        uint8_t *z_dirs = (uint8_t *)(z_val + ncols);
        uint64_t *h_idx = ctx->h_pin + PIN_WORDS - ncols;
        for (size_t c = 0; c < ncols; c++) {
            h_idx[c] = nv == 0 ? 0 : points[c * nv] % ((uint64_t)1 << nv);
            indices[c] = h_idx[c];
        }
        EvalSkip skip;
        if (job->zstride) {
            skip.ncols1 = (unsigned)job->ncols1;
            skip.z_in = job->zstride / 4;
            skip.z_changed = job->zstride / 8;
            memcpy(skip.y_of_col, job->tree.y_of_col, sizeof(skip.y_of_col));
            if (job->run_cols && !job->no_eval_skip) {
                skip.changed = (const unsigned long long *)((const uint8_t *)ctx->ws[WS_BATCH] + job->off_r_ctr) + RUN_CHANGED;
                ctx->stats.eval_constant_columns = job->const_cols;
            } else {
                ctx->stats.eval_constant_columns = 0;
            }
            CHK(timed_begin(ctx, 4));
            CHK(dev_eval_radix(ctx, job->d_cols, job->col_stride, ncols, nv, points, z_val, &skip));
            CHK(timed_end(ctx, 4, &ctx->stats.eval_us));
        } else {
            if (job->tree.lists && job->run_cols && job->col_stride >= job->N && !job->no_eval_skip) {
                skip.changed = ctx->d_run_count + RUN_CHANGED;
                ctx->stats.eval_constant_columns = job->const_cols;
                memcpy(skip.y_of_col, job->tree.y_of_col, sizeof(skip.y_of_col));
            }
            CHK(timed_begin(ctx, 4));
            CHK(dev_eval_folds(ctx, job->d_cols, job->col_stride, ncols, nv, points, z_val, skip.changed ? &skip : nullptr));
            CHK(timed_end(ctx, 4, &ctx->stats.eval_us));
        }
        const DoneFlag done = done_flag(ctx, 1);
        launch_paths(job->tree, job->tree.npad, (unsigned)nv, job->d_cols, job->col_stride, h_idx, z_sib, z_dirs, z_leaf,
                     job->zstride ? job->ncols1 : ncols, ctx->stream, done);
        HIPCHK(ctx, hipGetLastError());
        if (!(g_sleep_wait.load() && !ctx->timing && sleep_wait(done.flag, done.seq)))
            HIPCHK(ctx, hipStreamSynchronize(ctx->stream));
        if (sib_b) memcpy(siblings, z_sib, sib_b);
        for (size_t c = 0; c < ncols; c++) {
            leaves[c] = z_leaf[c];
            values[c] = z_val[c];
        }
        if (dir_b) memcpy(dirs, z_dirs, dir_b);
        CHK(bind_pool_collect(ctx));
        job->state = 2;
        return ZIGZ_OK;
    }
    if (job->zstride) {
        set_err(ctx, "batched commit job: the openings do not fit the staging buffer");
        return ZIGZ_ERR_INVALID_ARGUMENT;
    }
    void *dv;
    CHK(ws_get(ctx, WS_SCRATCH, ncols * 4 + 64, &dv));
    CHK(timed_begin(ctx, 4));
    CHK(dev_eval_folds(ctx, job->d_cols, job->col_stride, ncols, nv, points, (uint32_t *)dv));
    CHK(timed_end(ctx, 4, &ctx->stats.eval_us));
    std::vector<uint32_t> hv(ncols);
    HIPCHK(ctx, hipMemcpyAsync(hv.data(), dv, ncols * 4, hipMemcpyDeviceToHost, ctx->stream));
    std::vector<uint64_t> idx(ncols);
    for (size_t c = 0; c < ncols; c++) {
        idx[c] = nv == 0 ? 0 : points[c * nv] % ((uint64_t)1 << nv);
        indices[c] = idx[c];
    }
    CHK(open_paths(ctx, job->tree, (unsigned)nv, job->d_cols, job->col_stride, idx.data(), ncols, siblings, dirs, leaves));
    for (size_t c = 0; c < ncols; c++) values[c] = hv[c];
    CHK(bind_pool_collect(ctx));
    job->state = 2;
    return ZIGZ_OK;
    ZIGZ_NOTHROW_END(job->ctx)
}

extern "C" zigz_status zigz_commit_job_tree(zigz_commit_job *job, const void **d_tree, size_t *bytes_per_column) {
    if (job) ZIGZ_ENTER(job->ctx);
    if (!job || !d_tree || !bytes_per_column) return ZIGZ_ERR_INVALID_ARGUMENT;
    if (job->tree.lists && !job->whole) return ZIGZ_ERR_BAD_STATE;
    HIPCHK(job->ctx, hipEventSynchronize(job->built));
    *d_tree = job->tree.slab;
    *bytes_per_column = tree_nodes(job->N) * 32;
    return ZIGZ_OK;
}

extern "C" void zigz_commit_end(zigz_commit_job *job) {
    if (job) ZIGZ_ENTER(job->ctx);
    if (!job) return;
    zigz_ctx *ctx = job->ctx;
    (void)hipStreamSynchronize(ctx->stream);
    if (job->built) (void)hipEventDestroy(job->built);
// ... 5 lines not shown
```

zigz_amd/csrc/host/prover.cpp:

```cpp
#include <chrono>
#include <condition_variable>
#include <cstdio>
#include <cstdlib>
#include <cstring>
#include <exception>
#include <functional>
#include <memory>
#include <mutex>
#include <thread>

#include "zigz_host.hpp"
#if defined(__x86_64__)
#include <immintrin.h>
#endif

namespace zigz {

static double now_s() {
    return std::chrono::duration<double>(std::chrono::steady_clock::now().time_since_epoch()).count();
}

namespace {
class Helper {
  public:
// ... 424 lines not shown
        if (g->phase < 0) std::rethrow_exception(g->err);
    }
    memcpy(roots43, g->roots.data() + (size_t)*idx * ZIGZ_NUM_COLUMNS * 32, ZIGZ_NUM_COLUMNS * 32);
    return g;
}

void GpuBatcher::open(const std::shared_ptr<Group> &g, unsigned idx, const F *points, F *values, F *indices, F *leaves,
                      uint8_t *sib, uint8_t *dirs, zigz_kernel_stats *stats) {
    const size_t nc = ZIGZ_NUM_COLUMNS, nv = g->nv, k = g->cols.size();
    bool run_open = false;
    {
        std::unique_lock<std::mutex> lk(m_);
        if (g->phase < 0) std::rethrow_exception(g->err);
        memcpy(g->points.data() + (size_t)idx * nc * nv, points, nc * nv * sizeof(F));
        if (++g->handed_in == k) {
            g->phase = 3;
            run_open = true;
        }
    }
    if (run_open) run_open_all(g);
    {
        std::unique_lock<std::mutex> lk(m_);
        g->cv.wait(lk, [&] { return g->phase == 4 || g->phase < 0; });
        if (g->phase < 0) std::rethrow_exception(g->err);
    }
    memcpy(values, g->values.data() + (size_t)idx * nc, nc * sizeof(F));
    memcpy(indices, g->indices.data() + (size_t)idx * nc, nc * sizeof(F));
    memcpy(leaves, g->leaves.data() + (size_t)idx * nc, nc * sizeof(F));
    if (nv) {
        memcpy(sib, g->sib.data() + (size_t)idx * nc * nv * 32, nc * nv * 32);
        memcpy(dirs, g->dirs.data() + (size_t)idx * nc * nv, nc * nv);
    }
    if (stats) {
        *stats = g->stats;
        stats->keccak_permutations /= k;
        stats->list_hash_perms /= k;
        stats->run_aware_hashed /= k;
        stats->cons_hashed /= k;
    }
}

void GpuBatcher::abandon(const std::shared_ptr<Group> &g, unsigned idx) {
    bool run_open = false;
    {
        std::unique_lock<std::mutex> lk(m_);
        if (idx >= g->present.size() || !g->present[idx] || g->phase < 2 || g->phase >= 3) return;
        g->present[idx] = 0;
        if (++g->handed_in == g->cols.size()) {
            g->phase = 3;
            run_open = true;
        }
    }
    if (run_open) run_open_all(g);
}

Proof Prover::proveWitnessImpl(const PublicIO &io, size_t num_lookups, const Witness *witness, const uint32_t *d_cols,
                               size_t d_col_stride, size_t num_vars, const std::vector<uint64_t> *initial_regs,
                               std::vector<uint8_t> *bytes_out, const TraceRecords &records) {
    const bool steps = (bool)records;
    bindPublicInputs(io.program_hash, io.initial_pc, initial_regs);
    const size_t num_steps = io.num_steps;
    if (num_steps == 0) throw Error(ZIGZ_ERR_EMPTY_TRACE, "error.EmptyTrace");
    Proof proof = Proof::init(num_steps);
    if (proof.metadata.num_vars != num_vars) throw Error(ZIGZ_ERR_INVALID_ARGUMENT, "witness num_vars != log2_int_ceil(num_steps)");
    for (double &t : timings) t = 0;
    GpuSlots::Lease lease;
    struct MaskRestore {
        zigz_ctx *ctx = nullptr;
        int64_t sd = 0, ra = 0, cg = 0;
        void arm(zigz_ctx *c) {
            ctx = c;
            (void)zigz_ctx_get_option(ctx, "small_domain_mask", &sd);
            (void)zigz_ctx_get_option(ctx, "run_aware_mask", &ra);
            (void)zigz_ctx_get_option(ctx, "cons_group_mask", &cg);
        }
        void restore() {
            if (!ctx) return;
            (void)zigz_ctx_set_option(ctx, "small_domain_mask", sd);
            (void)zigz_ctx_set_option(ctx, "run_aware_mask", ra);
            (void)zigz_ctx_set_option(ctx, "cons_group_mask", cg);
            ctx = nullptr;
        }
        ~MaskRestore() { restore(); }
    } mask_restore;
    struct JobGuard {
        zigz_commit_job *job = nullptr;
        ~JobGuard() { if (job) zigz_commit_end(job); }
    } guard;
    size_t c0 = 0, c1 = ZIGZ_NUM_COLUMNS;
    if (shard_.world > 1) {
        if (shard_.rank < 0 || shard_.rank >= shard_.world || shard_.world > (int)ZIGZ_NUM_COLUMNS)
            throw Error(ZIGZ_ERR_INVALID_ARGUMENT, "sharded prove: bad rank / world");
        columnBlock(ZIGZ_NUM_COLUMNS, shard_.world, shard_.rank, c0, c1);
    }
    uint64_t m_small = 0, m_run = 0, m_cons = 0;
    {
        const uint64_t structural = (1ull << 1) | (0x3full << 33) | (1ull << 42), sel = (1ull << (c1 - c0)) - 1;
        if (small_domain_tables) m_small = (structural >> c0) & sel;
        if (run_aware) {
            const uint64_t small = small_domain_tables ? structural : 0;
            const uint64_t regs = 0x7fffffffull << 2, mem = 3ull << 40;
            const uint64_t hinted = run_aware == 2 ? ((1ull << ZIGZ_NUM_COLUMNS) - 1) & ~small : run_aware >= 3 ? regs | mem : regs;
            if (run_aware == 4) m_cons = ((1ull | (1ull << 1) | (0x7full << 33) | (1ull << 42)) >> c0) & sel;
            m_run = (hinted >> c0) & sel;
        }
    }
// ... 436 lines not shown
```

zigz_amd/csrc/kernels.hip:

```cpp
#include "kernels.hpp"
#include <hip/hip_ext.h>

#include "field.hpp"
#include "keccak.hpp"
#include "tree_dev.hpp"

namespace zk {

constexpr int UNROLL = 4;
constexpr size_t VEC_MIN_HALF = 4096;


__device__ __forceinline__ unsigned long long wave_sum(unsigned long long v) {
#pragma unroll
    for (int off = 32; off > 0; off >>= 1) v += __shfl_down(v, off, 64);
    return v;
}

__device__ __forceinline__ void block_add2(unsigned long long s0, unsigned long long s1,
                                           unsigned long long *sums) {
    __shared__ unsigned long long lds[2][TPB / 64];
    s0 = wave_sum(s0);
    s1 = wave_sum(s1);
    int lane = threadIdx.x & 63, wave = threadIdx.x >> 6;
// ... 173 lines not shown
}

SumsLayout half_sums_layout(size_t n, size_t ncols, size_t max_words) {
    if (n < 2048 || (n & (n - 1))) return SumsLayout{2, 1, 0, 1};
    const size_t per_addr = (n / 2) / (256 * block_sums_iters(n, floor_log2(n) - 1, ncols));
    size_t slots = (per_addr + 63) / 64;
    if (slots > 64) slots = 64;
    while (slots > 1 && slots * ncols * 32 > max_words) slots--;
    if (ncols * 32 > max_words) return SumsLayout{2, 1, 0, 1};
    return SumsLayout{32, 16, ncols * 32, (unsigned)(slots < 1 ? 1 : slots)};
}

SumsLayout bind_sums_layout(size_t half, size_t ncols, size_t max_words) {
    const size_t per_addr = half / 2 / 4096;
    if (per_addr <= 64 || ncols * 32 > max_words) return SumsLayout{2, 1, 0, 1};
    size_t slots = (per_addr + 63) / 64;
    if (slots > 64) slots = 64;
    while (slots > 1 && slots * ncols * 32 > max_words) slots--;
    return SumsLayout{32, 16, ncols * 32, (unsigned)slots};
}

void launch_block_sums(const uint32_t *d_in, size_t in_stride, size_t n, unsigned log2_m, size_t ncols,
                       unsigned long long *d_sums, SumsLayout lay, hipStream_t s, const KTime *kt) {
    const size_t iters = block_sums_iters(n, log2_m, ncols);
    const size_t waves = n / (256 * iters);
    if (lay.nslots == 0) lay.nslots = 1;
    dim3 grid((unsigned)((waves + TPB / 64 - 1) / (TPB / 64)), (unsigned)ncols);
    ZK_LAUNCH(kt, k_block_sums, grid, dim3(TPB), 0, s, d_in, in_stride, n, log2_m, (unsigned)iters, d_sums, lay);
}

void launch_half_sums(const uint32_t *d_in, size_t in_stride, size_t n, size_t ncols, unsigned long long *d_sums,
                      hipStream_t s, const KTime *kt, const SumsLayout *lay) {
    if (n == 0 || ncols == 0) return;
    if (n >= 2048 && (n & (n - 1)) == 0 && in_stride % 4 == 0 && aligned16(d_in)) {
        launch_block_sums(d_in, in_stride, n, floor_log2(n) - 1, ncols, d_sums, lay ? *lay : SumsLayout{2, 1, 0, 1}, s, kt);
    } else {
        ZK_LAUNCH(kt, k_half_sums_small, dim3(1, (unsigned)ncols), dim3(TPB), 0, s, d_in, in_stride, n, d_sums);
    }
}

constexpr int RB = 16;
constexpr int RLOOPS = ZK_FOLD_RLOOPS;
__device__ __forceinline__ bool eval_skips(const EvalSkip &skip, size_t col) {
    if (!skip.changed) return false;
    size_t z = 0;
    if (skip.ncols1) {
        z = col / skip.ncols1;
        col -= z * skip.ncols1;
    }
    if (col >= 64) return false;
    const int y = skip.y_of_col[col];
    return y >= 0 && skip.changed[z * skip.z_changed + y] == 0;
}
__device__ __forceinline__ size_t eval_col_off(const EvalSkip &skip, size_t col, size_t stride) {
    if (!skip.ncols1) return col * stride;
    const size_t z = col / skip.ncols1;
    return z * skip.z_in + (col - z * skip.ncols1) * stride;
}
template <bool FULL>
__global__ __launch_bounds__(TPB) void k_radix_fold(const uint32_t *__restrict__ in, size_t in_stride, size_t m, size_t nb,
                                                    const uint32_t *__restrict__ w_m, size_t w_stride,
                                                    unsigned long long *__restrict__ part, size_t part_col_stride, EvalSkip skip,
                                                    int rloops) {
    ZK_PRIO_SMALL();
    const size_t q = (size_t)blockIdx.x * TPB + threadIdx.x;
    if (q * 4 >= m) return;
    const size_t col = blockIdx.z;
    if (eval_skips(skip, col)) return;
    const uint4 *p = reinterpret_cast<const uint4 *>(in + eval_col_off(skip, col, in_stride)) + q;
    const uint32_t *w = w_m + col * w_stride;
    const size_t mq = m / 4;
    unsigned long long lo[4] = {0, 0, 0, 0}, hi[4] = {0, 0, 0, 0};
#pragma unroll 1
    for (int l = 0; l < rloops; l++) {
        const size_t b0 = ((size_t)blockIdx.y * rloops + l) * RB;
        if (!FULL && b0 >= nb) break;
        uint4 v[RB];
#pragma unroll
        for (int j = 0; j < RB; j++) v[j] = ZK_STREAM_LOAD(p + (FULL || b0 + j < nb ? b0 + j : nb - 1) * mq);
#pragma unroll
        for (int j = 0; j < RB; j++) {
            const uint32_t wj = FULL ? w[b0 + j] : (w[b0 + j < nb ? b0 + j : nb - 1] & (b0 + j < nb ? ~0u : 0u));
            const uint32_t e[4] = {v[j].x, v[j].y, v[j].z, v[j].w};
#pragma unroll
            for (int c = 0; c < 4; c++) {
                const unsigned long long pr = (unsigned long long)wj * e[c];
                lo[c] += (uint32_t)pr;
                hi[c] += pr >> 32;
            }
        }
    }
    unsigned long long s[4];
#pragma unroll
    for (int c = 0; c < 4; c++) s[c] = hi[c] + monty_reduce(lo[c]);
    ulonglong2 *o = reinterpret_cast<ulonglong2 *>(part + col * part_col_stride + (size_t)blockIdx.y * m + q * 4);
    o[0] = make_ulonglong2(s[0], s[1]);
    o[1] = make_ulonglong2(s[2], s[3]);
}

size_t radix_fold_groups(size_t nb, int rloops) {
    if (rloops <= 0) rloops = RLOOPS;
    return (nb + (size_t)RB * rloops - 1) / ((size_t)RB * rloops);
}

void launch_radix_fold(const uint32_t *d_in, size_t in_stride, size_t m, size_t nb, const uint32_t *d_w_m,
                       size_t w_stride, unsigned long long *d_part, size_t part_col_stride, size_t ncols, hipStream_t s,
                       hipEvent_t t_start, hipEvent_t t_stop, const EvalSkip *skip, int rloops) {
    if (rloops <= 0) rloops = RLOOPS;
    dim3 grid((unsigned)((m / 4 + TPB - 1) / TPB), (unsigned)radix_fold_groups(nb, rloops), (unsigned)ncols);
    auto kern = nb % ((size_t)RB * rloops) == 0 ? k_radix_fold<true> : k_radix_fold<false>;
    const EvalSkip sk = skip ? *skip : EvalSkip();
    if (t_start && t_stop)
        hipExtLaunchKernelGGL(kern, grid, dim3(TPB), 0, s, t_start, t_stop, 0, d_in, in_stride, m, nb, d_w_m, w_stride,
                              d_part, part_col_stride, sk, rloops);
    else
        hipLaunchKernelGGL(kern, grid, dim3(TPB), 0, s, d_in, in_stride, m, nb, d_w_m, w_stride, d_part, part_col_stride, sk,
                           rloops);
}

__global__ __launch_bounds__(TPB) void k_radix_finalize(const unsigned long long *__restrict__ part, size_t part_col_stride,
                                                        size_t groups, uint32_t *__restrict__ out, size_t out_stride,
                                                        size_t m, unsigned log2_m2, unsigned long long *__restrict__ sums,
                                                        EvalSkip skip, FinalizePublish pub) {
    ZK_PRIO_SMALL();
    __shared__ int s_last;
    const size_t i = (size_t)blockIdx.x * TPB + threadIdx.x;
    const size_t col = blockIdx.z;
    if (eval_skips(skip, col)) return;
    uint32_t v = 0;
    if (i < m) {
        const unsigned long long *pp = part + col * part_col_stride + i;
        unsigned long long t = 0;
        for (size_t g = 0; g < groups; g++) t += pp[g * m];
        v = (uint32_t)(t % (unsigned long long)P);
        out[col * out_stride + i] = v;
    }
    if (sums) {
        unsigned long long t = wave_sum((unsigned long long)v);
        if ((threadIdx.x & 63) == 0 && i < m && t) atomicAdd(&sums[i >> log2_m2], t);
    }
    if (pub.kind) {
        __threadfence();
        __syncthreads();
        if (threadIdx.x == 0) s_last = atomicAdd(pub.count, 1u) == gridDim.x - 1;
        __syncthreads();
        if (s_last) {
            __threadfence();
            if (pub.kind == 1) {
                for (unsigned j = threadIdx.x; j < pub.n; j += TPB) {
                    reinterpret_cast<unsigned long long *>(pub.h_dst)[j] = __hip_atomic_load(&sums[j], __ATOMIC_RELAXED, __HIP_MEMORY_SCOPE_AGENT);
                    sums[j] = 0;
                }
            } else {
                for (unsigned j = threadIdx.x; j < pub.n; j += TPB) reinterpret_cast<uint32_t *>(pub.h_dst)[j] = out[j];
            }
            __threadfence_system();
            __syncthreads();
            if (threadIdx.x == 0) {
                *pub.count = 0;
                __hip_atomic_store(pub.flag, pub.seq, __ATOMIC_RELEASE, __HIP_MEMORY_SCOPE_SYSTEM);
            }
        }
    }
}
// ... 35 lines not shown

__global__ __launch_bounds__(TPB) void k_eq_weights2(const uint32_t *__restrict__ r_m, size_t r_stride, unsigned kA,
                                                     uint32_t *__restrict__ wA, size_t strideA, unsigned kB,
                                                     uint32_t *__restrict__ wB, size_t strideB) {
    ZK_PRIO_SMALL();
    extern __shared__ uint32_t eqw[];
    const size_t col = blockIdx.x;
    const bool second = blockIdx.y != 0;
    const unsigned k = second ? kB : kA;
    const uint32_t *rr = r_m + col * r_stride + (second ? kA : 0);
    uint32_t *w = second ? wB + col * strideB : wA + col * strideA;
    if (threadIdx.x == 0) eqw[0] = R_MOD_P;
    __syncthreads();
    for (unsigned j = 0; j < k; j++) {
        const uint32_t r = rr[j];
        const uint32_t one_minus = sub_mod(R_MOD_P, r);
        const size_t cur = (size_t)1 << j;
        for (size_t base = 0; base < cur; base += TPB) {
            const size_t x = cur - 1 - (base + threadIdx.x);
            uint32_t v = 0;
            const bool live = base + threadIdx.x < cur;
            if (live) v = eqw[x];
            __syncthreads();
            if (live) {
                eqw[2 * x + 1] = mont_mul(v, r);
                eqw[2 * x] = mont_mul(v, one_minus);
            }
            __syncthreads();
        }
    }
    for (size_t i = threadIdx.x; i < ((size_t)1 << k); i += TPB) w[i] = eqw[i];
}
void launch_eq_weights2(const uint32_t *d_r_m, size_t r_stride, unsigned kA, uint32_t *d_wA, size_t strideA, unsigned kB,
                        uint32_t *d_wB, size_t strideB, size_t ncols, hipStream_t s) {
    const unsigned kmax = kA > kB ? kA : kB;
    hipLaunchKernelGGL(k_eq_weights2, dim3((unsigned)ncols, 2), dim3(TPB), ((size_t)1 << kmax) * 4, s, d_r_m, r_stride, kA, d_wA,
                       strideA, kB, d_wB, strideB);
}

void launch_eq_weights(const uint32_t *d_r_m, size_t r_stride, unsigned k, uint32_t *d_w_m, size_t w_stride, size_t ncols,
                       hipStream_t s) {
    hipLaunchKernelGGL(k_eq_weights, dim3((unsigned)ncols), dim3(TPB), ((size_t)1 << k) * 4, s, d_r_m, r_stride, k, d_w_m,
                       w_stride);
}

__global__ __launch_bounds__(TPB) void k_weighted_dot(const uint32_t *__restrict__ in, size_t in_stride,
                                                      const uint32_t *__restrict__ w_m, size_t w_stride, size_t n,
                                                      uint32_t *__restrict__ out, EvalSkip skip, const uint32_t *__restrict__ cols,
                                                      size_t col_stride) {
    ZK_PRIO_SMALL();
    __shared__ unsigned long long red[TPB / 64];
    const size_t col = blockIdx.x;
    if (cols && eval_skips(skip, col)) {
        if (threadIdx.x == 0) out[col] = cols[eval_col_off(skip, col, col_stride)];
        return;
    }
    unsigned long long acc = 0;
    for (size_t i = threadIdx.x; i < n; i += TPB) acc += mont_mul(w_m[col * w_stride + i], in[col * in_stride + i]);
    acc = wave_sum(acc);
    if ((threadIdx.x & 63) == 0) red[threadIdx.x >> 6] = acc;
    __syncthreads();
    if (threadIdx.x == 0) {
        unsigned long long t = 0;
        for (int w = 0; w < TPB / 64; w++) t += red[w];
        out[col] = (uint32_t)(t % (unsigned long long)P);
    }
}

void launch_weighted_dot(const uint32_t *d_in, size_t in_stride, const uint32_t *d_w_m, size_t w_stride, size_t n,
                         uint32_t *d_out, size_t ncols, hipStream_t s, const EvalSkip *skip, const uint32_t *d_cols,
                         size_t col_stride) {
    hipLaunchKernelGGL(k_weighted_dot, dim3((unsigned)ncols), dim3(TPB), 0, s, d_in, in_stride, d_w_m, w_stride, n, d_out,
                       skip ? *skip : EvalSkip(), skip ? d_cols : nullptr, col_stride);
}

__global__ __launch_bounds__(TPB) void k_narrow_u64(const uint64_t *__restrict__ in, uint32_t *__restrict__ out,
                                                    size_t n, uint32_t *flag) {
    size_t i = (size_t)blockIdx.x * TPB + threadIdx.x;
    const size_t step = (size_t)gridDim.x * TPB;
    uint32_t bad = 0;
    for (; i < n; i += step) {
        uint64_t v = in[i];
        bad |= (v >= (uint64_t)P) ? 1u : 0u;
        out[i] = (uint32_t)v;
    }
    if (__any(bad) && (threadIdx.x & 63) == 0) atomicOr(flag, 1u);
}

__global__ __launch_bounds__(TPB) void k_reduce_u64(const uint64_t *__restrict__ in, uint32_t *__restrict__ out,
                                                    size_t n) {
    size_t i = (size_t)blockIdx.x * TPB + threadIdx.x;
    const size_t step = (size_t)gridDim.x * TPB;
    for (; i < n; i += step) out[i] = (uint32_t)(in[i] % (uint64_t)P);
}

__global__ __launch_bounds__(TPB) void k_widen_u32(const uint32_t *__restrict__ in, uint64_t *__restrict__ out,
                                                   size_t n) {
    size_t i = (size_t)blockIdx.x * TPB + threadIdx.x;
    const size_t step = (size_t)gridDim.x * TPB;
    for (; i < n; i += step) out[i] = in[i];
}

constexpr int WROW = 43, WTILE = 64;
__global__ __launch_bounds__(TPB) void k_witness_rows(const uint64_t *__restrict__ rows, size_t num_steps, size_t npad,
                                                      uint32_t *__restrict__ cols, size_t stride) {
    __shared__ uint32_t tile[WTILE * WROW];
    const size_t base = (size_t)blockIdx.x * WTILE;
// ... 376 lines not shown
            }
#pragma unroll
            for (int k = 0; k < 2; k++) nt_store16(nodes + 64 * k + lane, mine[256 + 64 * k + lane]);
        }
    } else if ((threadIdx.x & 63) == 0) {
        const unsigned long long k = atomicAdd(todo_count, 1ull);
        todo[2 * k] = (uint32_t)blockIdx.y;
        todo[2 * k + 1] = (uint32_t)(i >> 6);
    }
}

__global__ __launch_bounds__(TPB) void k_keccak_small_fallback(const uint32_t *__restrict__ vals, size_t val_stride,
                                                               size_t n_values, size_t npad, uint8_t *__restrict__ tree,
                                                               size_t tree_stride_nodes, ColMap cmap,
                                                               const unsigned long long *__restrict__ todo_count,
                                                               const uint32_t *__restrict__ todo, int write_leaves,
                                                               const unsigned long long *__restrict__ only_if, ColMap tmap) {
    if (only_if && !*only_if) return;
    const unsigned long long count = *todo_count;
    const unsigned lane = threadIdx.x & 63;
    for (unsigned long long w = (unsigned long long)blockIdx.x * (TPB / 64) + (threadIdx.x >> 6); w < count;
         w += (unsigned long long)gridDim.x * (TPB / 64)) {
        const size_t col = cmap.c[todo[2 * w]];
        const size_t i = (size_t)todo[2 * w + 1] * 64 + lane;
        if (i >= npad / 2) continue;
        uint8_t *t = tree + (tmap.n ? (size_t)tmap.c[todo[2 * w]] : col) * tree_stride_nodes * 32;
        const uint32_t *v = vals + col * val_stride;
        const uint64_t v0 = 2 * i < n_values ? v[2 * i] : 0, v1 = 2 * i + 1 < n_values ? v[2 * i + 1] : 0;
        const Digest l0 = sha3_leaf(v0), l1 = sha3_leaf(v1);
        if (write_leaves) {
            store_digest(t, 2 * i, l0);
            store_digest(t, 2 * i + 1, l1);
        }
        store_digest(t, npad + i, sha3_node(l0, l1));
    }
}

void launch_keccak_small_l01(const uint32_t *d_vals, size_t val_stride, size_t n_values, size_t npad, uint8_t *d_tree,
                             size_t tree_stride_nodes, const ColMap &cols, const uint8_t *d_tables,
                             unsigned long long *d_todo_count, uint32_t *d_todo, hipStream_t s, const KTime *kt,
                             bool write_leaves, const unsigned long long *d_only_if, const ColMap *slabs) {
    if (cols.n == 0 || npad < 2) return;
    ColMap tm{};
    if (slabs) tm = *slabs;
    dim3 grid((unsigned)((npad / 2 + TPB - 1) / TPB), (unsigned)cols.n);
    ZK_LAUNCH(kt, k_keccak_small_l01, grid, dim3(TPB), 0, s, d_vals, val_stride, n_values, npad, d_tree, tree_stride_nodes, cols,
              d_tables, d_todo_count, d_todo, write_leaves ? 1 : 0, d_only_if, tm);
    hipLaunchKernelGGL(k_keccak_small_fallback, dim3(512), dim3(TPB), 0, s, d_vals, val_stride, n_values, npad, d_tree,
                       tree_stride_nodes, cols, d_todo_count, d_todo, write_leaves ? 1 : 0, d_only_if, tm);
}

__global__ __launch_bounds__(64) void k_paths(TreeRef t, size_t n_values, unsigned height, const uint32_t *__restrict__ vals,
                                              size_t val_stride, const uint64_t *__restrict__ idx, uint8_t *__restrict__ sib,
                                              uint8_t *__restrict__ dirs, uint32_t *__restrict__ leaf, DoneFlag done) {
    ZK_PRIO_SMALL();
    const size_t col = blockIdx.x;
    const size_t fc = (size_t)blockIdx.z * gridDim.x + col;
    if (t.zstride) vals += (size_t)blockIdx.z * (t.zstride / 4);
    const size_t index = idx[fc];
    const unsigned l = threadIdx.x;
    if (l == 0) leaf[fc] = vals[col * val_stride + index];
    if (l < height) {
        const size_t ci = index >> l;
        const size_t node = ci ^ 1;
        bool virt_leaf = l == 0 && col < 64 && ((t.virtual_leaves >> col) & 1);
        if (l == 0 && col < 64 && ((t.g_sd_mask >> col) & 1) && *t.g_dropped) virt_leaf = true;
        Digest d;
        if (virt_leaf) d = sha3_leaf<false>(node < n_values ? (uint64_t)vals[col * val_stride + node] : 0);
        else d = load_digest_at(node_ptr(t, col, l, node));
        d = canonical_digest(d);
        ulonglong2 *q = reinterpret_cast<ulonglong2 *>(sib + (fc * height + l) * 32);
        q[0] = make_ulonglong2(d.w[0], d.w[1]);
        q[1] = make_ulonglong2(d.w[2], d.w[3]);
        dirs[fc * height + l] = (uint8_t)(ci & 1);
    }
    signal_done(done, gridDim.x * gridDim.z);
}

void launch_paths(const TreeRef &t, size_t n_values, unsigned height, const uint32_t *d_vals, size_t val_stride,
                  const uint64_t *d_idx, uint8_t *d_sib, uint8_t *d_dirs, uint32_t *d_leaf, size_t ncols, hipStream_t s,
                  DoneFlag done) {
    hipLaunchKernelGGL(k_paths, dim3((unsigned)ncols, 1, t.nz ? t.nz : 1), dim3(64), 0, s, t, n_values, height, d_vals, val_stride, d_idx,
                       d_sib, d_dirs, d_leaf, done);
}
TreeRef slab_tree_ref(uint8_t *d_tree, size_t npad) {
    TreeRef t{};
    t.npad = npad;
    t.slab = d_tree;
    for (int c = 0; c < 64; c++) {
        t.slab_of_col[c] = (signed char)c;
        t.y_of_col[c] = -1;
        t.g_j_of_col[c] = -1;
    }
    return t;
}

__global__ void k_gather_nodes(const uint8_t *__restrict__ tree, size_t tree_stride_nodes, size_t node,
                               uint8_t *__restrict__ out, size_t ncols) {
    size_t c = (size_t)blockIdx.x * blockDim.x + threadIdx.x;
    if (c >= ncols) return;
    const Digest d = canonical_digest(load_digest(tree + c * tree_stride_nodes * 32, node));
    ulonglong2 *q = reinterpret_cast<ulonglong2 *>(out + c * 32);
    q[0] = make_ulonglong2(d.w[0], d.w[1]);
    q[1] = make_ulonglong2(d.w[2], d.w[3]);
}
__global__ __launch_bounds__(64) void k_job_summary(TreeRef t, unsigned height, uint8_t *__restrict__ out, size_t ncols,
                                                    const unsigned long long *r_ctr, const unsigned long long *sd_ctr,
                                                    const unsigned long long *g_ctr, DoneFlag done) {
    ZK_PRIO_SMALL();
    const size_t c = (size_t)blockIdx.x * blockDim.x + threadIdx.x;
    const unsigned z = blockIdx.z, nz = gridDim.z;
    if (t.zstride && z) {
        const size_t o = (size_t)z * t.zstride;
        if (r_ctr) r_ctr = reinterpret_cast<const unsigned long long *>(reinterpret_cast<uintptr_t>(r_ctr) + o);
        if (sd_ctr) sd_ctr = reinterpret_cast<const unsigned long long *>(reinterpret_cast<uintptr_t>(sd_ctr) + o);
        if (g_ctr) g_ctr = reinterpret_cast<const unsigned long long *>(reinterpret_cast<uintptr_t>(g_ctr) + o);
    }
    if (c < ncols) {
        const Digest d = canonical_digest(load_digest_at(node_ptr(t, c, height, 0)));
        ulonglong2 *q = reinterpret_cast<ulonglong2 *>(out + ((size_t)z * ncols + c) * 32);
        q[0] = make_ulonglong2(d.w[0], d.w[1]);
        q[1] = make_ulonglong2(d.w[2], d.w[3]);
    }
    unsigned long long *cnt = reinterpret_cast<unsigned long long *>(out + (size_t)nz * ncols * 32) + (size_t)z * JOB_SUMMARY_WORDS;
    if (c == 0) {
        cnt[0] = r_ctr ? r_ctr[0] : 0;
        cnt[1] = sd_ctr ? sd_ctr[0] : 0;
        cnt[2] = sd_ctr ? sd_ctr[1] : 0;
        cnt[3] = g_ctr ? g_ctr[0] : 0;
        cnt[4] = g_ctr ? g_ctr[8] : 0;
        cnt[5] = g_ctr ? g_ctr[9] : 0;
        cnt[6] = (r_ctr ? r_ctr[10] : 0) | ((g_ctr ? g_ctr[10] : 0) << 8);
        unsigned long long constant = 0;
        if (r_ctr)
            for (unsigned y = 0; y < t.ncols && y < 64; y++) constant += r_ctr[RUN_CHANGED + y] == 0;
        cnt[7] = constant;
// ... 6 lines not shown
            for (unsigned sub = 0; sub < RUN_SUBS; sub++) {
                const unsigned long long v = ctr[run_ctr_index(l, sub)];
                mx = v > mx ? v : mx;
            }
        cnt[8 + threadIdx.x] = mx;
    }
    signal_done(done, gridDim.x * gridDim.z);
}
template <int W>
__global__ __launch_bounds__(TPB) void k_publish(void *d_src, size_t n, void *h_dst, int rezero, DoneFlag done) {
    ZK_PRIO_SMALL();
    const size_t i = (size_t)blockIdx.x * TPB + threadIdx.x;
    if (i < n) {
        if (W == 8) {
            unsigned long long *s = reinterpret_cast<unsigned long long *>(d_src);
            reinterpret_cast<unsigned long long *>(h_dst)[i] = s[i];
            if (rezero) s[i] = 0;
        } else {
            uint32_t *s = reinterpret_cast<uint32_t *>(d_src);
            reinterpret_cast<uint32_t *>(h_dst)[i] = s[i];
            if (rezero) s[i] = 0;
        }
    }
    signal_done_block(done, gridDim.x);
}
void launch_publish_u64(unsigned long long *d_src, size_t n, unsigned long long *h_dst, bool rezero, hipStream_t s, DoneFlag done) {
    hipLaunchKernelGGL(k_publish<8>, dim3((unsigned)((n + TPB - 1) / TPB)), dim3(TPB), 0, s, (void *)d_src, n, (void *)h_dst, rezero ? 1 : 0, done);
}
void launch_publish_u32(const uint32_t *d_src, size_t n, uint32_t *h_dst, hipStream_t s, DoneFlag done) {
    hipLaunchKernelGGL(k_publish<4>, dim3((unsigned)((n + TPB - 1) / TPB)), dim3(TPB), 0, s, (void *)d_src, n, (void *)h_dst, 0, done);
}

__global__ __launch_bounds__(TPB) void k_zero_counters(unsigned long long *sd, unsigned long long *r, unsigned long long *g, size_t zstride) {
    ZK_PRIO_SMALL();
    const unsigned i = blockIdx.x * TPB + threadIdx.x;
    if (zstride && blockIdx.y) {
        const size_t o = (size_t)blockIdx.y * zstride / 8;
        if (sd) sd += o;
        if (r) r += o;
        if (g) g += o;
    }
    if (i < RUN_CTR_WORDS) {
        if (r) r[i] = 0;
        if (g) g[i] = 0;
    }
    if (sd && i < 2) sd[i] = 0;
}
void launch_zero_counters(unsigned long long *d_sd_ctr, unsigned long long *d_r_ctr, unsigned long long *d_g_ctr, hipStream_t s,
                          unsigned nz, size_t zstride) {
    hipLaunchKernelGGL(k_zero_counters, dim3((RUN_CTR_WORDS + TPB - 1) / TPB, nz ? nz : 1), dim3(TPB), 0, s, d_sd_ctr, d_r_ctr, d_g_ctr,
                       nz > 1 ? zstride : (size_t)0);
}
template <bool VEC>
__global__ __launch_bounds__(TPB) void k_gather_cols(ColSrcs srcs, size_t n, size_t src_stride, uint32_t *__restrict__ dst, size_t dst_stride,
                                                     size_t zstride) {
    const size_t i = (size_t)blockIdx.x * TPB + threadIdx.x;
    const uint32_t *sp = srcs.p[blockIdx.z] + (size_t)blockIdx.y * src_stride;
    uint32_t *dp = reinterpret_cast<uint32_t *>(reinterpret_cast<uint8_t *>(dst) + (size_t)blockIdx.z * zstride) + (size_t)blockIdx.y * dst_stride;
    if (VEC) {
        if (i < n / 4) reinterpret_cast<uint4 *>(dp)[i] = reinterpret_cast<const uint4 *>(sp)[i];
    } else if (i < n) {
        dp[i] = sp[i];
    }
}
void launch_gather_cols(const ColSrcs &srcs, unsigned nz, size_t ncols, size_t n, size_t src_stride, uint32_t *d_dst,
                        size_t dst_stride, size_t zstride, hipStream_t s) {
    bool vec = n % 4 == 0 && src_stride % 4 == 0 && dst_stride % 4 == 0 && zstride % 16 == 0 && aligned16(d_dst);
    for (unsigned z = 0; z < nz; z++) vec = vec && aligned16(srcs.p[z]);
    if (vec)
        hipLaunchKernelGGL(k_gather_cols<true>, dim3((unsigned)((n / 4 + TPB - 1) / TPB), (unsigned)ncols, nz), dim3(TPB), 0, s, srcs, n,
                           src_stride, d_dst, dst_stride, zstride);
    else
        hipLaunchKernelGGL(k_gather_cols<false>, dim3((unsigned)((n + TPB - 1) / TPB), (unsigned)ncols, nz), dim3(TPB), 0, s, srcs, n,
                           src_stride, d_dst, dst_stride, zstride);
}
void launch_job_summary(const TreeRef &t, unsigned height, uint8_t *d_out, size_t ncols, const unsigned long long *d_r_ctr,
                        const unsigned long long *d_sd_ctr, const unsigned long long *d_g_ctr, hipStream_t s, DoneFlag done) {
    hipLaunchKernelGGL(k_job_summary, dim3((unsigned)((ncols + 63) / 64), 1, t.nz ? t.nz : 1), dim3(64), 0, s, t, height, d_out, ncols, d_r_ctr,
                       d_sd_ctr, d_g_ctr, done);
}
void launch_gather_nodes(const uint8_t *d_tree, size_t tree_stride_nodes, size_t node, uint8_t *d_out, size_t ncols,
                         hipStream_t s) {
    hipLaunchKernelGGL(k_gather_nodes, dim3((unsigned)((ncols + 63) / 64)), dim3(64), 0, s, d_tree, tree_stride_nodes, node,
                       d_out, ncols);
}

__global__ void k_gather_first(const uint32_t *__restrict__ in, size_t stride, uint32_t *__restrict__ out,
                               size_t ncols) {
    size_t c = (size_t)blockIdx.x * blockDim.x + threadIdx.x;
    if (c < ncols) out[c] = in[c * stride];
}
void launch_gather_first(const uint32_t *d_in, size_t stride, uint32_t *d_out, size_t ncols, hipStream_t s) {
    hipLaunchKernelGGL(k_gather_first, dim3((unsigned)((ncols + 63) / 64)), dim3(64), 0, s, d_in, stride, d_out, ncols);
}

__device__ __forceinline__ uint64_t xxh3_64_of_u64(uint64_t h) {
    const uint64_t bitflip = 0x1cad21f72c81017cull ^ 0xdb979083e96dd4deull;
    uint64_t in64 = (h >> 32) + (h << 32);
    uint64_t k = in64 ^ bitflip;
    k ^= rotl64(k, 49) ^ rotl64(k, 24);
    k *= 0x9FB21C651E98DF25ull;
    k ^= (k >> 35) + 8;
    k *= 0x9FB21C651E98DF25ull;
    return k ^ (k >> 28);
}

__global__ __launch_bounds__(TPB) void k_lasso_fingerprints(const uint32_t *__restrict__ rows, size_t n_rows,
                                                            size_t width, uint32_t *__restrict__ out) {
    size_t i = (size_t)blockIdx.x * TPB + threadIdx.x;
    if (i >= n_rows) return;
    uint64_t h = 0;
    for (size_t f = 0; f < width; f++) {
        h ^= rows[i * width + f];
        h = xxh3_64_of_u64(h);
    }
    out[i] = (uint32_t)(h % (uint64_t)P);
}

void launch_lasso_fingerprints(const uint32_t *d_rows, size_t rows, size_t width, uint32_t *d_out, hipStream_t s,
                               const KTime *kt) {
    if (rows)
        ZK_LAUNCH(kt, k_lasso_fingerprints, dim3((unsigned)((rows + TPB - 1) / TPB)), dim3(TPB), 0, s, d_rows, rows, width,
                  d_out);
}

__global__ __launch_bounds__(TPB) void k_fill_pattern(uint32_t *__restrict__ out, size_t n, uint32_t seed) {
    size_t i = (size_t)blockIdx.x * TPB + threadIdx.x;
// ... 15 lines not shown
```

zigz_amd/csrc/kernels.hpp:

```cpp
#pragma once
#include <hip/hip_runtime.h>
#include <stddef.h>
#include <stdint.h>

namespace zk {

struct KTime {
    hipEvent_t start, stop;
};

inline size_t tree_level_offset(size_t npad, unsigned level) { return 2 * npad - 2 * (npad >> level); }
inline size_t tree_nodes(size_t npad) { return 2 * npad; }

void launch_narrow_u64(const uint64_t *d_in, uint32_t *d_out, size_t n, uint32_t *d_flag, hipStream_t s);
void launch_reduce_u64(const uint64_t *d_in, uint32_t *d_out, size_t n, hipStream_t s);
void launch_witness_rows(const uint64_t *d_rows, size_t num_steps, size_t npad, uint32_t *d_cols, size_t stride,
                         hipStream_t s);
void launch_widen_u32(const uint32_t *d_in, uint64_t *d_out, size_t n, hipStream_t s);
struct TraceStep {
    uint64_t pc, rd_value, mem_addr, mem_value;
    int64_t imm;
    uint8_t opcode, rd, rs1, rs2, funct3, funct7, wr_reg, mem_is_read;
};
static_assert(sizeof(TraceStep) == 48, "TraceStep must mirror zigz_trace_step (48 bytes)");
struct TraceStep32 {
    uint64_t pc, rd_value;
    int32_t imm;
    uint32_t mem_index;
    uint8_t opcode, rd, rs1, rs2, funct3, funct7, wr_reg, mem_is_read;
};
static_assert(sizeof(TraceStep32) == 32, "TraceStep32 must mirror zigz_trace_step32 (32 bytes)");
struct MemAccess {
    uint64_t addr, value;
};
void launch_steps_widen(const TraceStep32 *d_in, size_t num_steps, const MemAccess *d_mem, size_t num_mem, TraceStep *d_out,
                        hipStream_t s);
struct TraceStep16 {
    uint32_t pc_word, mem_wr;
    uint64_t rd_value;
};
struct CodeEntry {
    int32_t imm;
    uint8_t opcode, rd, rs1, rs2, funct3, funct7, reserved[2];
};
static_assert(sizeof(TraceStep16) == 16 && sizeof(CodeEntry) == 12, "16-byte record / code entry mirrors");
void launch_steps_widen16(const TraceStep16 *d_in, size_t num_steps, const MemAccess *d_mem, size_t num_mem, uint64_t code_base,
                          const CodeEntry *d_code, size_t num_code, TraceStep *d_out, hipStream_t s);
struct Regs32 {
    uint32_t v[32];
};
inline size_t witness_steps_ws_words(size_t npad) {
    const size_t nchunks = (npad + 63) / 64;
    return 65 * nchunks + 64 + 32 * ((nchunks + 255) / 256) + 64;
}
void launch_witness_steps(const TraceStep *d_steps, size_t num_steps, size_t npad, const Regs32 &init, uint32_t *d_ws,
                          uint32_t *d_cols, size_t stride, hipStream_t s, const KTime *kt_expand = nullptr);

struct SumsLayout {
    size_t col_stride, bin_stride, slot_stride;
    unsigned nslots;
};
void launch_bind(const uint32_t *d_in, size_t in_stride, uint32_t *d_out, size_t out_stride, size_t half,
                 size_t ncols, uint32_t r_m, const uint32_t *d_r_m, unsigned long long *d_sums, hipStream_t s,
                 const KTime *kt = nullptr, const SumsLayout *lay = nullptr);
SumsLayout bind_sums_layout(size_t half, size_t ncols, size_t max_words);
bool bind_uses_vec(size_t half, bool with_sums, size_t in_stride, size_t out_stride, const void *in, const void *out);
inline bool aligned16(const void *p) { return ((uintptr_t)p & 15) == 0; }
SumsLayout half_sums_layout(size_t n, size_t ncols, size_t max_words);
void launch_half_sums(const uint32_t *d_in, size_t in_stride, size_t n, size_t ncols,
                      unsigned long long *d_sums, hipStream_t s, const KTime *kt = nullptr, const SumsLayout *lay = nullptr);

void launch_block_sums(const uint32_t *d_in, size_t in_stride, size_t n, unsigned log2_m, size_t ncols,
                       unsigned long long *d_sums, SumsLayout lay, hipStream_t s, const KTime *kt = nullptr);
size_t radix_fold_groups(size_t nb, int rloops = 0);
struct EvalSkip {
    const unsigned long long *changed = nullptr;
    signed char y_of_col[64];
    unsigned ncols1 = 0;
    size_t z_in = 0, z_changed = 0;
};
void launch_radix_fold(const uint32_t *d_in, size_t in_stride, size_t m, size_t nb, const uint32_t *d_w_m,
                       size_t w_stride, unsigned long long *d_part, size_t part_col_stride, size_t ncols, hipStream_t s,
                       hipEvent_t t_start = nullptr, hipEvent_t t_stop = nullptr, const EvalSkip *skip = nullptr, int rloops = 0);
struct DoneFlag;
struct FinalizePublish {
    int kind = 0;
    unsigned n = 0;
    void *h_dst = nullptr;
    unsigned *count = nullptr;
    unsigned long long *flag = nullptr;
    unsigned long long seq = 0;
};
void launch_radix_finalize(const unsigned long long *d_part, size_t part_col_stride, size_t groups, uint32_t *d_out,
                           size_t out_stride, size_t m, unsigned log2_m2, unsigned long long *d_sums, size_t ncols,
                           hipStream_t s, const EvalSkip *skip = nullptr, const FinalizePublish *pub = nullptr);
void launch_eq_weights(const uint32_t *d_r_m, size_t r_stride, unsigned k, uint32_t *d_w_m, size_t w_stride, size_t ncols,
                       hipStream_t s);
void launch_eq_weights2(const uint32_t *d_r_m, size_t r_stride, unsigned kA, uint32_t *d_wA, size_t strideA, unsigned kB,
                        uint32_t *d_wB, size_t strideB, size_t ncols, hipStream_t s);
void launch_weighted_dot(const uint32_t *d_in, size_t in_stride, const uint32_t *d_w_m, size_t w_stride, size_t n,
                         uint32_t *d_out, size_t ncols, hipStream_t s, const EvalSkip *skip = nullptr,
                         const uint32_t *d_cols = nullptr, size_t col_stride = 0);

struct ColMap {
    uint8_t n;
    uint8_t c[64];
};
constexpr unsigned RUN_SEG = 4096;
constexpr unsigned RUN_STAGE_LEVELS = 6;
constexpr unsigned RUN_MAX_LEVELS = 20;
constexpr unsigned RUN_SUBS = 32;
constexpr unsigned RUN_NODE_BITS = 26;
constexpr size_t RUN_MIN_LEAVES = 32768;
constexpr size_t RUN_MAX_LEAVES = (size_t)1 << RUN_NODE_BITS;
constexpr unsigned RUN_CTRS = (1 + RUN_MAX_LEVELS * RUN_SUBS) * 16;
constexpr unsigned RUN_CHANGED = RUN_CTRS;
constexpr unsigned RUN_CTR_WORDS = RUN_CTRS + 64;
__host__ __device__ inline size_t run_ctr_index(unsigned level, unsigned sub) { return (size_t)(1 + level * RUN_SUBS + sub) * 16; }
inline unsigned run_top_level(size_t npad) { unsigned v = 0; while (((size_t)1 << v) < npad) v++; return v - 8; }
__host__ __device__ inline size_t run_tile_nodes(size_t npad, unsigned l) {
    if (l == 0) return RUN_SEG;
    const unsigned s = (l - 1) / RUN_STAGE_LEVELS;
    const size_t n_in = npad >> (s * RUN_STAGE_LEVELS);
    const size_t seg = n_in < RUN_SEG ? n_in : RUN_SEG;
    return seg >> (l - s * RUN_STAGE_LEVELS);
}
struct LevelLists {
    unsigned top;
    unsigned long long base[RUN_MAX_LEVELS];
    unsigned cap[RUN_MAX_LEVELS];
    unsigned long long entries;
};
template <class T>
struct ZPtr {
    T *p;
    size_t zs;
    __host__ __device__ ZPtr &operator=(T *q) {
        p = q;
        return *this;
    }
    __host__ __device__ operator T *() const {
#if defined(__HIP_DEVICE_COMPILE__)
        return reinterpret_cast<T *>(reinterpret_cast<uintptr_t>(p) + (size_t)blockIdx.z * zs);
#else
        return p;
#endif
    }
};
struct TreeRef {
    size_t npad;
    ZPtr<uint8_t> slab;
    signed char slab_of_col[64];
    int lists;
    unsigned top;
    ZPtr<uint8_t> upper;
    ZPtr<unsigned long long> bitmap;
    ZPtr<unsigned short> prev;
    ZPtr<unsigned short> woff;
    ZPtr<uint32_t> ubase;
    unsigned long long ubase_off[RUN_MAX_LEVELS];
    unsigned ncols;
    signed char y_of_col[64];
    ZPtr<uint8_t> r_store;
    LevelLists r_lists;
    signed char g_j_of_col[64];
    unsigned g_ncols;
    ZPtr<const uint32_t> g_rep;
    ZPtr<uint8_t> g_store;
    LevelLists g_lists;
    ZPtr<const unsigned long long> g_dropped;
    unsigned long long g_sd_mask;
    unsigned long long virtual_leaves;
    size_t zstride;
    unsigned nz;
};
__host__ __device__ inline size_t run_meta_base(size_t npad, unsigned ncols, unsigned l) {
    return (size_t)ncols * ((2 * npad - 2 * (npad >> l)) / 64);
}
inline size_t runs_meta_words(size_t npad, size_t ncols) { return ncols * (2 * npad / 64); }
LevelLists runs_lists(size_t npad, size_t ncols, const unsigned *cap_in = nullptr);
LevelLists cons_lists(size_t npad, const unsigned *cap_in = nullptr);
size_t runs_units(size_t npad, size_t ncols, unsigned long long ubase_off[RUN_MAX_LEVELS]);
size_t runs_stage_scratch_bytes(size_t npad, size_t ncols);

struct MerkleBuild {
    ZPtr<const uint32_t> vals;
    size_t val_stride, n_values, npad;
    TreeRef t;
    ColMap rcols;
    ZPtr<uint32_t> r_list;
    ZPtr<unsigned long long> r_ctr;
    ZPtr<uint8_t> r_stage;
    ColMap gcols;
    ColMap gcols_sd;
    int g_has_slabs;
    int g_no_probe;
    ZPtr<unsigned long long> g_keys;
    ZPtr<uint32_t> g_idx;
    ZPtr<uint32_t> g_rep;
    ZPtr<uint32_t> g_list;
    ZPtr<unsigned long long> g_ctr;
    unsigned g_gen;
};
inline void set_zstride(MerkleBuild &b, size_t zs, unsigned nz) {
    TreeRef &t = b.t;
    t.zstride = zs;
    t.nz = nz;
    t.slab.zs = t.upper.zs = t.bitmap.zs = t.prev.zs = t.woff.zs = t.ubase.zs = t.r_store.zs = t.g_rep.zs = t.g_store.zs = t.g_dropped.zs = zs;
    b.vals.zs = b.r_list.zs = b.r_ctr.zs = b.r_stage.zs = b.g_keys.zs = b.g_idx.zs = b.g_rep.zs = b.g_list.zs = b.g_ctr.zs = zs;
}
void launch_runs_structure(const MerkleBuild &b, hipStream_t s, const KTime *kt = nullptr);
void launch_cons_structure(const MerkleBuild &b, hipStream_t s, const KTime *kt = nullptr);
void launch_structure(const MerkleBuild &b, hipStream_t s, bool fused, const KTime *kt = nullptr);
void launch_level_hash(const MerkleBuild &b, unsigned L, hipStream_t s, const KTime *kt = nullptr, size_t expect = 0,
                       bool fused = false);
void launch_fill_virtual(const MerkleBuild &b, hipStream_t s);
void launch_merkle_top(const TreeRef &t, unsigned first_level, unsigned height, size_t ncols, hipStream_t s, const KTime *kt = nullptr);
void launch_keccak_leaves(const uint32_t *d_vals, size_t val_stride, size_t n_values, size_t npad,
                          uint8_t *d_tree, size_t tree_stride_nodes, size_t ncols, hipStream_t s, const KTime *kt = nullptr,
                          const ColMap *cols = nullptr, const ColMap *slabs = nullptr);
void launch_keccak_level(uint8_t *d_tree, size_t tree_stride_nodes, size_t in_off, size_t out_off, size_t n_out,
                         size_t ncols, hipStream_t s, const KTime *kt = nullptr, const ColMap *slabs = nullptr);
constexpr unsigned SD_DOMAIN = 128;
constexpr size_t SD_TABLE_BYTES = (size_t)(SD_DOMAIN + SD_DOMAIN * SD_DOMAIN) * 32;
void launch_sd_tables(uint8_t *d_tables, hipStream_t s);
inline size_t sd_todo_words(size_t npad, size_t ncols) { return 2 * ncols * ((npad / 2 + 63) / 64) + 2; }
void launch_keccak_small_l01(const uint32_t *d_vals, size_t val_stride, size_t n_values, size_t npad, uint8_t *d_tree,
                             size_t tree_stride_nodes, const ColMap &cols, const uint8_t *d_tables,
                             unsigned long long *d_todo_count, uint32_t *d_todo, hipStream_t s, const KTime *kt = nullptr,
                             bool write_leaves = true, const unsigned long long *d_only_if = nullptr,
                             const ColMap *slabs = nullptr);
bool keccak_level_is_wide(size_t n_out, size_t ncols);
struct DoneFlag {
    unsigned *count = nullptr;
    unsigned long long *flag = nullptr;
    unsigned long long seq = 0;
};
void launch_publish_u64(unsigned long long *d_src, size_t n, unsigned long long *h_dst, bool rezero, hipStream_t s, DoneFlag done);
void launch_publish_u32(const uint32_t *d_src, size_t n, uint32_t *h_dst, hipStream_t s, DoneFlag done);
void launch_paths(const TreeRef &t, size_t n_values, unsigned height, const uint32_t *d_vals, size_t val_stride,
                  const uint64_t *d_idx, uint8_t *d_sib, uint8_t *d_dirs, uint32_t *d_leaf, size_t ncols, hipStream_t s,
                  DoneFlag done = DoneFlag());
TreeRef slab_tree_ref(uint8_t *d_tree, size_t npad);
void launch_gather_nodes(const uint8_t *d_tree, size_t tree_stride_nodes, size_t node, uint8_t *d_out, size_t ncols,
                         hipStream_t s);
constexpr unsigned JOB_SUMMARY_WORDS = 8 + 2 * RUN_MAX_LEVELS;
void launch_zero_counters(unsigned long long *d_sd_ctr, unsigned long long *d_r_ctr, unsigned long long *d_g_ctr, hipStream_t s,
                          unsigned nz = 0, size_t zstride = 0);
struct ColSrcs {
    const uint32_t *p[32];
};
void launch_gather_cols(const ColSrcs &srcs, unsigned nz, size_t ncols, size_t n, size_t src_stride, uint32_t *d_dst,
                        size_t dst_stride, size_t zstride, hipStream_t s);
void launch_job_summary(const TreeRef &t, unsigned height, uint8_t *d_out, size_t ncols, const unsigned long long *d_r_ctr,
                        const unsigned long long *d_sd_ctr, const unsigned long long *d_g_ctr, hipStream_t s,
                        DoneFlag done = DoneFlag());
void launch_gather_first(const uint32_t *d_in, size_t stride, uint32_t *d_out, size_t ncols, hipStream_t s);
void launch_lasso_fingerprints(const uint32_t *d_rows, size_t rows, size_t width, uint32_t *d_out, hipStream_t s,
                               const KTime *kt = nullptr);
void launch_fill_pattern(uint32_t *d_out, size_t n, uint32_t seed, hipStream_t s);

constexpr unsigned BATCH_WG = 256;
struct BatchTab {
    const uint32_t *in;
    uint32_t *out;
    unsigned long long *part;
    unsigned long long *sums;
    const uint32_t *w;
    uint64_t tail_off;
    uint32_t log2_n;
    uint32_t k;
    uint32_t log2_m2;
    uint32_t iters;
    uint32_t first_wg;
    uint32_t reserved;
};
struct BatchPublish {
    void *h_dst = nullptr;
    unsigned long long *d_sums = nullptr;
    size_t n = 0;
    unsigned *count = nullptr;
    unsigned long long *flag = nullptr;
    unsigned long long seq = 0;
};
void launch_batch_block_sums(const BatchTab *d_tabs, unsigned nt, unsigned nwg, hipStream_t s);
void launch_batch_fold(const BatchTab *d_tabs, unsigned nt, unsigned nwg, hipStream_t s);
void launch_batch_finalize(const BatchTab *d_tabs, unsigned nt, unsigned nwg, hipStream_t s);
void launch_batch_publish(const BatchPublish &pub, hipStream_t s);
void launch_batch_tails(const BatchTab *d_tabs, unsigned nt, unsigned nwg, const BatchPublish &pub, hipStream_t s);
struct FpTab {
    const uint32_t *in;
    uint32_t *out;
    uint64_t rows, padded;
    uint32_t width, first_wg;
};
void launch_batch_fingerprints(const FpTab *d_tabs, unsigned nt, unsigned nwg, hipStream_t s);

constexpr unsigned MB_BLOCK = 512;
constexpr unsigned MB_STAGE_LEVELS = 9;
constexpr unsigned MB_EVAL_CHUNK = 4096;
struct MBatchTab {
    const uint32_t *src;
    uint32_t *vals;
    uint8_t *tree;
    uint64_t n, npad;
    uint32_t lin;
// ... 51 lines not shown
```

zigz_amd/csrc/merkle_levels.hip:

```cpp
#include "kernels.hpp"
#include "tree_dev.hpp"

namespace zk {

#ifndef ZK_CONS_TPB
#define ZK_CONS_TPB 256
#endif
constexpr int CONS_TPB = ZK_CONS_TPB;

static unsigned log2u(size_t n) { unsigned l = 0; while (((size_t)1 << l) < n) l++; return l; }

static size_t stage_fv_bytes(size_t npad, size_t ncols, unsigned s) { return ncols * (npad >> (s * RUN_STAGE_LEVELS)) * 4; }
static size_t stage_inner_bytes(size_t npad, size_t ncols, unsigned s) {
    const size_t n = npad >> (s * RUN_STAGE_LEVELS);
    return ncols * ((n + 63) / 64) * 8;
}
static size_t stage_off(size_t npad, size_t ncols, unsigned s) {
    size_t off = 0;
    for (unsigned t = 1; t < s; t++) off += stage_fv_bytes(npad, ncols, t) + stage_inner_bytes(npad, ncols, t);
    return off;
}
size_t runs_stage_scratch_bytes(size_t npad, size_t ncols) {
    const unsigned top = run_top_level(npad);
    size_t b = 64;
    for (unsigned s = 1; s * RUN_STAGE_LEVELS < top; s++) b += stage_fv_bytes(npad, ncols, s) + stage_inner_bytes(npad, ncols, s);
    return b;
}

static void stage_shape(size_t npad, unsigned l, size_t &seg, size_t &nseg, unsigned &rel) {
    const unsigned s = l == 0 ? 0 : (l - 1) / RUN_STAGE_LEVELS;
    const size_t n_in = npad >> (s * RUN_STAGE_LEVELS);
    seg = n_in < RUN_SEG ? n_in : RUN_SEG;
    nseg = n_in / seg;
    rel = l - s * RUN_STAGE_LEVELS;
}
LevelLists runs_lists(size_t npad, size_t ncols, const unsigned *cap_in) {
    LevelLists L{};
    L.top = run_top_level(npad);
    unsigned long long at = 0;
    for (unsigned l = 0; l <= L.top; l++) {
        size_t seg, nseg;
        unsigned rel;
        stage_shape(npad, l, seg, nseg, rel);
        const size_t units = ncols * nseg;
        const size_t worst = (units + RUN_SUBS - 1) / RUN_SUBS * (seg >> rel);
        L.base[l] = at;
        L.cap[l] = (unsigned)(cap_in && cap_in[l] && cap_in[l] < worst ? cap_in[l] : worst);
        at += (unsigned long long)L.cap[l] * RUN_SUBS;
    }
    L.entries = at;
    return L;
}
size_t runs_units(size_t npad, size_t ncols, unsigned long long ubase_off[RUN_MAX_LEVELS]) {
    size_t at = 0;
    const unsigned top = run_top_level(npad);
    for (unsigned l = 0; l <= top; l++) {
        size_t seg, nseg;
        unsigned rel;
        stage_shape(npad, l, seg, nseg, rel);
        ubase_off[l] = at;
        at += ncols * nseg;
// ... 16 lines not shown

constexpr unsigned long long BITS_ODD = 0xAAAAAAAAAAAAAAAAull;
__device__ __forceinline__ unsigned long long compress_even64(unsigned long long x) {
    x &= 0x5555555555555555ull;
    x = (x | (x >> 1)) & 0x3333333333333333ull;
    x = (x | (x >> 2)) & 0x0f0f0f0f0f0f0f0full;
    x = (x | (x >> 4)) & 0x00ff00ff00ff00ffull;
    x = (x | (x >> 8)) & 0x0000ffff0000ffffull;
    x = (x | (x >> 16)) & 0x00000000ffffffffull;
    return x;
}

template <int CTRL, int ROW_MASK, int BANK_MASK>
__device__ __forceinline__ int dpp_i32(int old, int v) { return __builtin_amdgcn_update_dpp(old, v, CTRL, ROW_MASK, BANK_MASK, false); }
__device__ __forceinline__ unsigned wave_scan_add(unsigned v) {
    int s = (int)v;
    s += dpp_i32<0x111, 0xf, 0xf>(0, s);
    s += dpp_i32<0x112, 0xf, 0xf>(0, s);
    s += dpp_i32<0x114, 0xf, 0xf>(0, s);
    s += dpp_i32<0x118, 0xf, 0xf>(0, s);
    s += dpp_i32<0x142, 0xa, 0xf>(0, s);
    s += dpp_i32<0x143, 0xc, 0xf>(0, s);
    return (unsigned)s;
}
__device__ __forceinline__ int wave_scan_max(int v) {
    int s = v, t;
    t = dpp_i32<0x111, 0xf, 0xf>(-1, s); s = s > t ? s : t;
    t = dpp_i32<0x112, 0xf, 0xf>(-1, s); s = s > t ? s : t;
    t = dpp_i32<0x114, 0xf, 0xf>(-1, s); s = s > t ? s : t;
    t = dpp_i32<0x118, 0xf, 0xf>(-1, s); s = s > t ? s : t;
    t = dpp_i32<0x142, 0xa, 0xf>(-1, s); s = s > t ? s : t;
    t = dpp_i32<0x143, 0xc, 0xf>(-1, s); s = s > t ? s : t;
    return s;
}

constexpr int RUNS_WAVES = TPB / 64;
template <bool STAGE0>
__device__ __forceinline__ void runs_stage_wg(const MerkleBuild &b, unsigned bx, unsigned y, unsigned stage, unsigned seg_log2,
                                              unsigned rmax, unsigned nseg, size_t in_off, size_t out_off) {
    ZK_PRIO_SMALL();
    const unsigned lane = threadIdx.x & 63, wave = threadIdx.x >> 6;
    const unsigned segi = bx * RUNS_WAVES + wave;
    if (segi >= nseg) return;
    const unsigned seg = 1u << seg_log2, words = seg / 64;
    const unsigned l_in = stage * RUN_STAGE_LEVELS;
    const size_t n_in = b.npad >> l_in;
    const size_t first = (size_t)segi * seg;
    unsigned long long E = 0, I = 0;
    uint32_t fv_mine = 0;
    {
        const uint32_t *src;
        size_t limit;
        if (STAGE0) {
            src = b.vals + (size_t)b.rcols.c[y] * b.val_stride + first;
            limit = b.n_values > first ? b.n_values - first : 0;
        } else {
            src = reinterpret_cast<const uint32_t *>(b.r_stage + in_off) + (size_t)y * n_in + first;
            limit = seg;
            const unsigned long long *inner = reinterpret_cast<const unsigned long long *>(
                b.r_stage + in_off + (size_t)b.rcols.n * n_in * 4) + ((size_t)y * n_in + first) / 64;
            if (lane < words) I = inner[lane];
        }
        uint32_t prev_last = 0;
        for (unsigned q0 = 0; q0 < words; q0 += 32) {
            uint32_t x[32];
#pragma unroll
            for (unsigned j = 0; j < 32; j++) {
                const unsigned i = (q0 + j) * 64 + lane;
                x[j] = (q0 + j < words && i < limit) ? src[i] : 0u;
            }
#pragma unroll
            for (unsigned j = 0; j < 32; j++) {
                const unsigned q = q0 + j;
                uint32_t left = (uint32_t)__builtin_amdgcn_update_dpp(0, (int)x[j], 0x138 , 0xf, 0xf, false);
                if (lane == 0) left = prev_last;
                const bool c = (q == 0 && lane == 0) || x[j] != left;
                const unsigned long long m = __ballot(c);
                const uint32_t x_first = (uint32_t)__builtin_amdgcn_readfirstlane((int)x[j]);
                if (q < words) {
                    if (lane == q) { E = m; fv_mine = x_first; }
                    prev_last = (uint32_t)__builtin_amdgcn_readlane((int)x[j], 63);
                }
            }
        }
    }
    if (STAGE0) {
        const unsigned long long inside = lane < words ? (lane == 0 ? E & ~1ull : E) : 0;
        const uint32_t col_first = b.n_values ? b.vals[(size_t)b.rcols.c[y] * b.val_stride] : 0u;
        const uint32_t seg_first = (uint32_t)__builtin_amdgcn_readfirstlane((int)fv_mine);
        if (__ballot(inside != 0) || seg_first != col_first)
            if (lane == 0) b.r_ctr[RUN_CHANGED + y] = 1;
    }
    unsigned w = words;
    unsigned long long need_r[RUN_STAGE_LEVELS + 1];
    unsigned off_r[RUN_STAGE_LEVELS + 1];
    unsigned my_tot = 0;
#pragma unroll
    for (unsigned r = 0; r <= RUN_STAGE_LEVELS; r++) {
        need_r[r] = 0;
        off_r[r] = 0;
        if (r > rmax) continue;
        if (r) {
            const unsigned long long t = I | (E & BITS_ODD);
            const unsigned long long i32 = compress_even64(t | (t >> 1)), e32 = compress_even64(E);
            const unsigned long long ilo = __shfl(i32, (2 * lane) & 63), ihi = __shfl(i32, (2 * lane + 1) & 63);
            const unsigned long long elo = __shfl(e32, (2 * lane) & 63), ehi = __shfl(e32, (2 * lane + 1) & 63);
            w >>= 1;
            I = lane < w ? (ilo | (ihi << 32)) : 0;
            E = lane < w ? (elo | (ehi << 32)) : 0;
        }
        if (!STAGE0 && r == 0) continue;
        unsigned carry = (unsigned)__builtin_amdgcn_update_dpp(0, (int)(I >> 63), 0x138 , 0xf, 0xf, false);
        if (lane == 0) carry = 1;
        const unsigned long long need = lane < w ? (I | (I << 1) | carry | E) : 0;
        const unsigned cnt = (unsigned)__builtin_popcountll(need);
        const unsigned incl = wave_scan_add(cnt);
        const int last = wave_scan_max(need ? (int)(lane * 64 + 63 - __builtin_clzll(need)) : -1);
        int prev = __builtin_amdgcn_update_dpp(0, last, 0x138 , 0xf, 0xf, false);
        if (lane == 0) prev = 0;
        const unsigned tot = (unsigned)__builtin_amdgcn_readlane((int)incl, 63);
        if (lane == r) my_tot = tot;
        const unsigned l_abs = l_in + r;
        if (lane < w) {
            const size_t e = run_meta_base(b.npad, b.t.ncols, l_abs) + ((size_t)y * (b.npad >> l_abs) + (first >> r)) / 64 + lane;
            b.t.bitmap[e] = need;
            b.t.prev[e] = (unsigned short)prev;
            b.t.woff[e] = (unsigned short)(incl - cnt);
        }
        need_r[r] = need;
        off_r[r] = incl - cnt;
    }
    if (out_off != ~(size_t)0) {
        const size_t n_out = n_in >> RUN_STAGE_LEVELS;
        uint32_t *fv = reinterpret_cast<uint32_t *>(b.r_stage + out_off) + (size_t)y * n_out + (size_t)segi * 64;
        unsigned long long *inner = reinterpret_cast<unsigned long long *>(b.r_stage + out_off + (size_t)b.rcols.n * n_out * 4) +
                                    ((size_t)y * n_out) / 64 + segi;
        fv[lane] = fv_mine;
        if (lane == 0) *inner = I;
    }
    unsigned my_slot = 0, my_room = 0;
    if (lane <= rmax && (STAGE0 || lane != 0)) {
// ... 34 lines not shown
    unsigned stage, seg_log2, rmax, nseg, wgs;
    size_t in_off, out_off;
};
static unsigned runs_nstages(const MerkleBuild &b) {
    unsigned nstages = 1;
    while (nstages * RUN_STAGE_LEVELS < b.t.r_lists.top) nstages++;
    return b.rcols.n ? nstages : 0;
}
static RunsStage runs_stage_shape(const MerkleBuild &b, unsigned st) {
    RunsStage r{};
    if (st >= runs_nstages(b)) return r;
    const unsigned top = b.t.r_lists.top;
    const size_t n_in = b.npad >> (st * RUN_STAGE_LEVELS);
    const size_t seg = n_in < RUN_SEG ? n_in : RUN_SEG;
    r.stage = st;
    r.seg_log2 = log2u(seg);
    r.rmax = top - st * RUN_STAGE_LEVELS < RUN_STAGE_LEVELS ? top - st * RUN_STAGE_LEVELS : RUN_STAGE_LEVELS;
    r.nseg = (unsigned)(n_in / seg);
    r.wgs = (r.nseg + RUNS_WAVES - 1) / RUNS_WAVES;
    r.in_off = st ? stage_off(b.npad, b.rcols.n, st) : 0;
    r.out_off = st + 1 < runs_nstages(b) ? stage_off(b.npad, b.rcols.n, st + 1) : ~(size_t)0;
    return r;
}

void launch_runs_structure(const MerkleBuild &b, hipStream_t s, const KTime *kt) {
    if (b.rcols.n == 0) return;
    const unsigned nstages = runs_nstages(b);
    for (unsigned st = 0; st < nstages; st++) {
        const RunsStage r = runs_stage_shape(b, st);
        const dim3 grid(r.wgs, b.rcols.n, b.t.nz ? b.t.nz : 1);
        hipEvent_t e0 = kt && st == 0 ? kt->start : nullptr, e1 = kt && st + 1 == nstages ? kt->stop : nullptr;
        if (st == 0) {
            if (e0 || e1) hipExtLaunchKernelGGL(k_runs_stage<true>, grid, dim3(TPB), 0, s, e0, e1, 0, b, st, r.seg_log2, r.rmax, r.nseg, r.in_off, r.out_off);
            else hipLaunchKernelGGL(k_runs_stage<true>, grid, dim3(TPB), 0, s, b, st, r.seg_log2, r.rmax, r.nseg, r.in_off, r.out_off);
        } else {
            if (e0 || e1) hipExtLaunchKernelGGL(k_runs_stage<false>, grid, dim3(TPB), 0, s, e0, e1, 0, b, st, r.seg_log2, r.rmax, r.nseg, r.in_off, r.out_off);
            else hipLaunchKernelGGL(k_runs_stage<false>, grid, dim3(TPB), 0, s, b, st, r.seg_log2, r.rmax, r.nseg, r.in_off, r.out_off);
        }
    }
}

constexpr unsigned CONS_GEN_SHIFT = 52;
__device__ __forceinline__ unsigned long long cons_mix(unsigned long long x) {
    x ^= x >> 30; x *= 0xbf58476d1ce4e5b9ull;
    x ^= x >> 27; x *= 0x94d049bb133111ebull;
    return x ^ (x >> 31);
}
constexpr unsigned CONS_TUP = 16;
__device__ __forceinline__ unsigned long long cons_leaf_payload(const MerkleBuild &b, size_t k, uint32_t *tup = nullptr) {
    unsigned long long h = 0x243f6a8885a308d3ull;
    if (tup && b.gcols.n <= CONS_TUP) {
#pragma unroll
        for (unsigned j = 0; j < CONS_TUP; j++) {
            tup[j] = (j < b.gcols.n && k < b.n_values) ? b.vals[(size_t)b.gcols.c[j] * b.val_stride + k] : 0u;
            if (j < b.gcols.n) h = cons_mix(h ^ tup[j]);
        }
    } else {
        for (unsigned j = 0; j < b.gcols.n; j++)
            h = cons_mix(h ^ (k < b.n_values ? b.vals[(size_t)b.gcols.c[j] * b.val_stride + k] : 0u));
    }
    return h & ((1ull << CONS_GEN_SHIFT) - 1);
}
__device__ __forceinline__ unsigned wave_leader(unsigned long long key, bool valid, unsigned lane) {
    unsigned long long pend = __ballot(valid);
    unsigned mine = lane;
    while (pend) {
        const unsigned ld = (unsigned)__builtin_ctzll(pend);
        const unsigned long long kk = __shfl(key, ld);
        const bool same = valid && key == kk;
        if (same) mine = ld;
        pend &= ~__ballot(same);
    }
    return mine;
}
__device__ __forceinline__ unsigned cons_take_slot(const MerkleBuild &b, unsigned l, bool want, unsigned lane, size_t wave_global) {
    const unsigned long long m = __ballot(want);
    if (!m) return 0;
    const unsigned sub = (unsigned)(wave_global % RUN_SUBS);
    const unsigned cap = b.t.g_lists.cap[l];
    unsigned long long base = 0;
    if (lane == (unsigned)__builtin_ctzll(m)) base = atomicAdd(&b.g_ctr[run_ctr_index(l, sub)], (unsigned long long)__builtin_popcountll(m));
    base = __shfl(base, (unsigned)__builtin_ctzll(m));
    unsigned long long pos = base + (unsigned)__builtin_popcountll(m & ((1ull << lane) - 1));
    if (want && pos >= cap) {
        atomicOr(&b.g_ctr[10], 1ull);
        pos = cap - 1;
    }
    return sub * cap + (unsigned)pos;
}
__device__ __forceinline__ bool cons_insert(unsigned long long *keys, size_t mask, unsigned long long key, unsigned g_cur, unsigned g_prev,
                                            size_t *where) {
    size_t slot = cons_mix(key) & mask;
    for (size_t tries = 0; tries <= mask; tries++) {
        if (keys[slot] == key) return false;
        unsigned long long cur = __atomic_load_n(&keys[slot], __ATOMIC_RELAXED);
        for (;;) {
            if (cur == key) return false;
            const unsigned g = (unsigned)(cur >> CONS_GEN_SHIFT);
            if (g == g_cur || g == g_prev) break;
            const unsigned long long old = atomicCAS(&keys[slot], cur, key);
            if (old == cur) {
                *where = slot;
                return true;
            }
            cur = old;
        }
        slot = (slot + 1) & mask;
    }
    return false;
}
__device__ __forceinline__ uint32_t cons_lookup(const unsigned long long *keys, const uint32_t *idx, size_t mask, unsigned long long key) {
    size_t slot = cons_mix(key) & mask;
// ... 28 lines not shown

constexpr unsigned CONS_SAMPLE = 16;
__device__ __forceinline__ void cons_leaf_insert_wg(const MerkleBuild &b, int sample, unsigned bx, unsigned long long *s_set) {
    ZK_PRIO_SMALL();
    if (!sample && b.g_ctr[8]) return;
    for (unsigned i = threadIdx.x; i < CONS_SET; i += CONS_TPB) s_set[i] = 0;
    __syncthreads();
    const size_t k = (size_t)bx * CONS_TPB + threadIdx.x;
    if (sample && ((k / 64) % CONS_SAMPLE) != 0) return;
    const unsigned lane = threadIdx.x & 63;
    const bool valid = k < b.npad;
    const unsigned long long key = ((unsigned long long)b.g_gen << CONS_GEN_SHIFT) | (valid ? cons_leaf_payload(b, k) : 0);
    const unsigned ld = wave_leader(key, valid, lane);
    cons_insert_level(b, s_set, 0, key, valid && ld == lane, (uint32_t)k, lane, k / 64);
}
__global__ __launch_bounds__(CONS_TPB) void k_cons_leaf_insert(MerkleBuild b, int sample) {
    __shared__ unsigned long long s_set[CONS_SET];
    cons_leaf_insert_wg(b, sample, blockIdx.x, s_set);
}

template <bool LEAF>
__device__ __forceinline__ void cons_pass_wg(const MerkleBuild &b, unsigned lr, int do_insert, unsigned bx, unsigned long long *s_set) {
    ZK_PRIO_SMALL();
    if (b.g_ctr[8]) return;
    for (unsigned i = threadIdx.x; i < CONS_SET; i += CONS_TPB) s_set[i] = 0;
    __syncthreads();
    const size_t n = b.npad >> lr, c = (size_t)bx * CONS_TPB + threadIdx.x;
    const unsigned lane = threadIdx.x & 63;
    const bool valid = c < n;
    const size_t mask = 2 * b.npad - 1;
    const unsigned g_r = b.g_gen + lr;
    const size_t off = 2 * b.npad - 2 * n;
    const size_t off_in = LEAF ? 0 : 2 * b.npad - 2 * (b.npad >> (lr - 1));
    unsigned long long key = (unsigned long long)g_r << CONS_GEN_SHIFT;
    uint32_t tup[CONS_TUP];
    if (valid) {
        if (LEAF) key |= cons_leaf_payload(b, c, tup);
        else {
            const uint2 p = *reinterpret_cast<const uint2 *>(b.g_rep + off_in + 2 * c);
            key |= ((unsigned long long)p.x << RUN_NODE_BITS) | p.y;
        }
    }
    const unsigned ld = wave_leader(key, valid, lane);
    uint32_t r = 0xffffffffu;
    if (valid && ld == lane) r = cons_lookup(b.g_keys, b.g_idx, mask, key);
    r = __shfl(r, ld);
    bool alone = false;
    if (LEAF && valid && r != 0xffffffffu) {
        const size_t rn = b.g_list[b.t.g_lists.base[0] + r];
        if (rn != c) {
            if (b.gcols.n <= CONS_TUP) {
#pragma unroll
                for (unsigned j = 0; j < CONS_TUP; j++)
                    if (j < b.gcols.n && tup[j] != (rn < b.n_values ? b.vals[(size_t)b.gcols.c[j] * b.val_stride + rn] : 0u)) alone = true;
            } else {
                for (unsigned j = 0; j < b.gcols.n; j++) {
                    const uint32_t *v = b.vals + (size_t)b.gcols.c[j] * b.val_stride;
                    if ((c < b.n_values ? v[c] : 0u) != (rn < b.n_values ? v[rn] : 0u)) { alone = true; break; }
                }
            }
        }
    }
    if (valid && r == 0xffffffffu) alone = true;
    const unsigned own = cons_take_slot(b, lr, alone, lane, c / 64);
    if (LEAF) {
        const unsigned long long am = __ballot(alone);
        if (am && lane == (unsigned)__builtin_ctzll(am)) atomicAdd(&b.g_ctr[11], (unsigned long long)__builtin_popcountll(am));
    }
    if (alone) {
        r = own;
        b.g_list[b.t.g_lists.base[lr] + own] = (uint32_t)c;
    }
    if (valid) b.g_rep[off + c] = r;
    if (do_insert) {
        const uint32_t r_hi = __shfl_down(r, 1);
        const bool mine = valid && !(c & 1);
        const unsigned long long k2 = ((unsigned long long)(g_r + 1) << CONS_GEN_SHIFT) | ((unsigned long long)r << RUN_NODE_BITS) | r_hi;
        const unsigned ld2 = wave_leader(k2, mine, lane);
        cons_insert_level(b, s_set, lr + 1, k2, mine && ld2 == lane, (uint32_t)(c >> 1), lane, c / 128);
    }
}
template <bool LEAF>
__global__ __launch_bounds__(CONS_TPB) void k_cons_pass(MerkleBuild b, unsigned lr, int do_insert) {
    __shared__ unsigned long long s_set[CONS_SET];
    cons_pass_wg<LEAF>(b, lr, do_insert, blockIdx.x, s_set);
}

__global__ __launch_bounds__(64) void k_cons_decide(MerkleBuild b, int sample) {
    ZK_PRIO_SMALL();
    unsigned long long c = threadIdx.x < RUN_SUBS ? b.g_ctr[run_ctr_index(0, threadIdx.x)] : 0;
#pragma unroll
    for (int off = 32; off > 0; off >>= 1) c += __shfl_down(c, off);
    if (threadIdx.x == 0) {
        if (sample) {
            const bool drop = c > b.npad / CONS_SAMPLE / 4;
            b.g_ctr[8] = drop ? 1 : 0;
            b.g_ctr[9] = drop ? c * CONS_SAMPLE : 0;
        } else if (!b.g_ctr[8]) {
            const bool out_of_room = (b.g_ctr[10] & 1) != 0;
            if (out_of_room) c -= b.g_ctr[11] < c ? b.g_ctr[11] : c;
            b.g_ctr[9] = c;
            b.g_ctr[8] = c > b.npad / 4 ? 1 : 0;
        }
        if (!sample && b.g_ctr[8] && !b.g_has_slabs) atomicOr(&b.g_ctr[10], 2ull);
    }
}

static bool cons_probe(const MerkleBuild &b) { return b.npad >= ((size_t)1 << 16) && !b.g_no_probe; }

void launch_cons_structure(const MerkleBuild &b, hipStream_t s, const KTime *kt) {
// ... 76 lines not shown
            out = b.t.upper + (e & 4095) * 32;
            in0 = b.t.upper + ((2 * e) & 4095) * 32;
            in1 = in0 + 32;
        } else
#endif
        if (e < cR) {
            unsigned sub = 0;
#pragma unroll
            for (unsigned step = RUN_SUBS / 2; step; step >>= 1)
                if (s_r[sub + step] <= e) sub += step;
            const size_t slot = (size_t)sub * r_cap + (e - s_r[sub]);
            const uint32_t ent = b.r_list[rl.list_base + slot];
            const unsigned y = ent >> RUN_NODE_BITS;
            col = b.rcols.c[y];
            k = ent & ((1u << RUN_NODE_BITS) - 1);
            out = r_slot_ptr(b.t, rl, slot);
            if (!LEAF) {
                size_t c0, c1;
                r_slot_pair(b.t, rc, y, 2 * k, &c0, &c1);
                in0 = r_slot_ptr(b.t, rc, c0);
                in1 = r_slot_ptr(b.t, rc, c1);
            }
        } else if (e < cR + cG) {
            const unsigned t32 = (unsigned)(e - cR);
            unsigned ei = __umulhi(t32, g_magic), j = t32 - ei * gn;
            if (j >= gn) {
                ei++;
                j -= gn;
            }
            col = b.gcols.c[j];
            unsigned sub = 0;
#pragma unroll
            for (unsigned step = RUN_SUBS / 2; step; step >>= 1)
                if (s_g[sub + step] <= ei) sub += step;
            const size_t slot = (size_t)sub * g_cap + (ei - s_g[sub]);
            k = b.g_list[g_base + slot];
            out = b.t.g_store + ((g_base + slot) * gn + j) * 32;
            if (!LEAF) {
                const uint2 p = *reinterpret_cast<const uint2 *>(b.g_rep + g_rep_c + 2 * k);
                in0 = b.t.g_store + ((g_base_c + p.x) * gn + j) * 32;
                in1 = b.t.g_store + ((g_base_c + p.y) * gn + j) * 32;
            }
        } else {
            const size_t t = e - cR - cG;
            col = gdense.c[t >> n_L_log2];
            k = t & (n_L - 1);
            out = slab_ptr(b.t, col, L, k);
            if (!LEAF) {
                in0 = slab_ptr(b.t, col, L - 1, 2 * k);
                in1 = in0 + 32;
            }
        }
        Digest d;
        if (LEAF) d = sha3_leaf<PAUSE>((uint64_t)(k < b.n_values ? b.vals[col * b.val_stride + k] : 0u));
        else d = sha3_node<PAUSE>(load_digest_at(in0), load_digest_at(in1));
        store_digest_at(out, d);
    }
}
template <bool LEAF, bool PAUSE>
__global__ __launch_bounds__(TPB, ZK_LEVEL_HASH_MIN_WAVES) void k_level_hash(MerkleBuild b, unsigned L, ColMap gdense, int prio) {
    level_hash_wg<LEAF, PAUSE>(b, L, gdense, prio, blockIdx.x, gridDim.x);
}

#ifndef ZK_STRUCT_SEPARATE
static_assert(CONS_TPB == TPB, "the fused structure launches share the 256-thread workgroups of the hash and runs kernels "
                               "(build with -DZK_STRUCT_SEPARATE for another ZK_CONS_TPB)");
template <bool FIRST>
__global__ __launch_bounds__(TPB) void k_structure(MerkleBuild b, unsigned nruns, RunsStage rs) {
    __shared__ unsigned long long s_set[CONS_SET];
    if (blockIdx.x < nruns) {
        runs_stage_wg<FIRST>(b, blockIdx.x % rs.wgs, blockIdx.x / rs.wgs, rs.stage, rs.seg_log2, rs.rmax, rs.nseg, rs.in_off, rs.out_off);
        return;
    }
    const unsigned w = blockIdx.x - nruns;
    if (FIRST) cons_leaf_insert_wg(b, 0, w, s_set);
    else cons_pass_wg<true>(b, 0u, b.t.g_lists.top >= 1 ? 1 : 0, w, s_set);
}
static_assert((RUN_NODE_BITS - 8 + RUN_STAGE_LEVELS - 1) / RUN_STAGE_LEVELS <= 3, "a runs stage would ride above level 0");
template <bool LEAF, bool PAUSE, bool STAGE>
__global__ __launch_bounds__(TPB, ZK_LEVEL_HASH_MIN_WAVES) void k_level_hash_rides(MerkleBuild b, unsigned L, ColMap gdense, int prio,
                                                                                   unsigned npass, RunsStage rs) {
    extern __shared__ unsigned long long s_dyn[];
    if (blockIdx.x < npass) {
        cons_pass_wg<false>(b, L + 1, L + 1 < b.t.g_lists.top ? 1 : 0, blockIdx.x, s_dyn);
        return;
    }
    const unsigned w = blockIdx.x - npass, nrs = STAGE ? rs.wgs * b.rcols.n : 0;
    if (STAGE && w < nrs) {
        runs_stage_wg<false>(b, w % rs.wgs, w / rs.wgs, rs.stage, rs.seg_log2, rs.rmax, rs.nseg, rs.in_off, rs.out_off);
        return;
    }
    level_hash_wg<LEAF, PAUSE>(b, L, gdense, prio, w - nrs, gridDim.x - npass - nrs);
}
#endif

#define ZK_LAUNCH_EV(e0, e1, kern, grid, block, lds, s, ...)                                                      \
    do {                                                                                                          \
        const hipEvent_t ev0_ = (e0), ev1_ = (e1);                                                                \
        if (ev0_ || ev1_) hipExtLaunchKernelGGL(kern, grid, block, lds, s, ev0_, ev1_, 0, __VA_ARGS__);           \
        else hipLaunchKernelGGL(kern, grid, block, lds, s, __VA_ARGS__);                                          \
    } while (0)

static RunsStage runs_stage_riding(const MerkleBuild &b, unsigned L) { return runs_stage_shape(b, L + 2); }

void launch_structure(const MerkleBuild &b, hipStream_t s, bool fused, const KTime *kt) {
#ifdef ZK_STRUCT_SEPARATE
    fused = false;
// ... 136 lines not shown
```

zigz_amd/hip.py:

```python
import ctypes as C

import numpy as np

from . import errors
from ._ffi import BenchResult, KernelStats, lib, u8p, u64p, vp

P = 2013265921
NUM_COLUMNS = 43
TRACE_STEP_DTYPE = np.dtype([("pc", "<u8"), ("rd_value", "<u8"), ("mem_addr", "<u8"), ("mem_value", "<u8"), ("imm", "<i8"),
                             ("opcode", "u1"), ("rd", "u1"), ("rs1", "u1"), ("rs2", "u1"), ("funct3", "u1"), ("funct7", "u1"),
                             ("wr_reg", "u1"), ("mem_is_read", "u1")])
assert TRACE_STEP_DTYPE.itemsize == 48
TRACE_STEP32_DTYPE = np.dtype([("pc", "<u8"), ("rd_value", "<u8"), ("imm", "<i4"), ("mem_index", "<u4"), ("opcode", "u1"), ("rd", "u1"),
                               ("rs1", "u1"), ("rs2", "u1"), ("funct3", "u1"), ("funct7", "u1"), ("wr_reg", "u1"), ("mem_is_read", "u1")])
MEM_ACCESS_DTYPE = np.dtype([("addr", "<u8"), ("value", "<u8")])
assert TRACE_STEP32_DTYPE.itemsize == 32 and MEM_ACCESS_DTYPE.itemsize == 16
NO_MEM_ACCESS = 0xFFFFFFFF


def compact_steps32(steps, has_access):
    steps = np.ascontiguousarray(steps, dtype=TRACE_STEP_DTYPE)
    has_access = np.asarray(has_access, dtype=bool)
    out = np.zeros(len(steps), dtype=TRACE_STEP32_DTYPE)
    for f in ("pc", "rd_value", "opcode", "rd", "rs1", "rs2", "funct3", "funct7", "wr_reg", "mem_is_read"):
# ... 549 lines not shown

    def open(self, indices):
        k, tot = len(self.heights), sum(self.heights)
        ix, ixp = _u64(np.asarray(indices, dtype=np.uint64).reshape(-1))
        if len(indices) != k:
            raise ValueError(f"{len(indices)} indices for {k} trees")
        leaf, lp = _out_u64(k)
        sib, sp = _out_u8(32 * tot)
        dirs, dp = _out_u8(tot)
        bad = C.c_size_t(0)
        self.ctx.check_batch(lib.zigz_merkle_open_batch(self.ctx.h, self.h, ixp, sp, dp, lp, C.byref(bad)), bad)
        out, o = [], 0
        for i, v in enumerate(self.heights):
            out.append(dict(index=int(ix[i]), value=int(leaf[i]), siblings=sib[32 * o: 32 * (o + v)].tobytes(),
                            directions=dirs[o: o + v].tobytes()))
            o += v
        return out

    def deinit(self):
        if self.h:
            lib.zigz_merkle_batch_destroy(self.ctx.h, self.h)
            self.h = None

    def __del__(self):
        try:
            self.deinit()
        except Exception:
            pass


class CommitmentScheme:

    @staticmethod
    def commit(ctx, evals):
        tree = SimpleMerkleTree(ctx, evals)
        return tree.root_hash, tree

    @staticmethod
    def open(ctx, evals, tree, point):
        nv = len(point)
        a, ap = (None, None) if evals is None else _u64(evals)
        n = tree.n_values if evals is None else len(evals)
        q, qp = _u64(point)
        sib, sp = _out_u8(32 * nv)
        dirs, dp = _out_u8(nv)
        val, idx, leaf = C.c_uint64(), C.c_uint64(), C.c_uint64()
        ctx.check(lib.zigz_commit_open(ctx.h, ap, n, tree.t, qp, nv, C.byref(val), C.byref(idx), sp, dp, C.byref(leaf)))
        return dict(value=val.value, index=idx.value, leaf=leaf.value, siblings=sib[: 32 * nv].tobytes(),
                    directions=dirs[:nv].tobytes())


class CommitJob:

    def __init__(self, ctx, cols=None, d_cols=None, ncols=NUM_COLUMNS, nv=None, col_stride=None, d_cols_list=None):
        self.ctx = ctx
        j = vp()
        if d_cols_list is not None:
            k = len(d_cols_list)
            arr = (vp * k)(*[vp(d) for d in d_cols_list])
            ctx.check(lib.zigz_commit_begin_batch(ctx.h, arr, k, ncols, col_stride or (1 << nv), nv, C.byref(j)))
            ncols = ncols * k
        elif cols is not None:
            cols = np.ascontiguousarray(cols, dtype=np.uint64)
            ncols, N = cols.shape
            nv = N.bit_length() - 1
            self._keep = cols
            ctx.check(lib.zigz_commit_begin(ctx.h, cols.ctypes.data_as(u64p), ncols, N, nv, C.byref(j)))
        else:
            ctx.check(lib.zigz_commit_begin_dev(ctx.h, vp(d_cols), ncols, col_stride or (1 << nv), nv, C.byref(j)))
        self.j, self.ncols, self.nv = j, ncols, nv

    def roots(self):
        r, rp = _out_u8(self.ncols * 32)
        self.ctx.check(lib.zigz_commit_roots(self.j, rp))
        return r[: self.ncols * 32].reshape(self.ncols, 32)

    def open_all(self, points):
        nc, nv = self.ncols, self.nv
        p, pp = _u64(np.asarray(points, dtype=np.uint64).reshape(-1))
        values, vpp = _out_u64(nc)
        idx, ip = _out_u64(nc)
        leaves, lp = _out_u64(nc)
        sib, sp = _out_u8(nc * nv * 32)
        dirs, dp = _out_u8(nc * nv)
        self.ctx.check(lib.zigz_commit_open_all(self.j, pp, vpp, ip, lp, sp, dp))
        return dict(values=values[:nc], indices=idx[:nc], leaves=leaves[:nc],
                    siblings=sib[: nc * nv * 32].reshape(nc, nv, 32), dirs=dirs[: nc * nv].reshape(nc, nv))

    def tree(self):
        d, n = vp(), C.c_size_t()
        self.ctx.check(lib.zigz_commit_job_tree(self.j, C.byref(d), C.byref(n)))
        return d.value, n.value

    def end(self):
        if self.j:
            lib.zigz_commit_end(self.j)
            self.j = None

    def __del__(self):
        try:
            self.end()
        except Exception:
            pass


class Transcript:

    def __init__(self):
        self.h = lib.zigz_transcript_new()

    def __del__(self):
        if getattr(self, "h", None):
            lib.zigz_transcript_free(self.h)
# ... 26 lines not shown
```

Baseline: 2.296 billion.

## Read batch commit columns in place via per-proof source pointers instead of gathering

```diff
diff --git a/bindings/zig/zigz_hip.zig b/bindings/zig/zigz_hip.zig
--- a/bindings/zig/zigz_hip.zig
+++ b/bindings/zig/zigz_hip.zig
@@ -184,6 +184,7 @@
 pub extern "c" fn zigz_commit_begin(ctx: ?*Ctx, cols: [*c]const u64, ncols: usize, col_stride: usize, nv: usize, out: [*c]?*CommitJob) Status;
 pub extern "c" fn zigz_commit_begin_dev(ctx: ?*Ctx, d_cols: [*c]const u32, ncols: usize, col_stride: usize, nv: usize, out: [*c]?*CommitJob) Status;
 pub extern "c" fn zigz_commit_begin_batch(ctx: ?*Ctx, d_cols: [*c][*c]u32, nproofs: usize, ncols: usize, col_stride: usize, nv: usize, out: [*c]?*CommitJob) Status;
+pub extern "c" fn zigz_commit_begin_batch_strided(ctx: ?*Ctx, d_cols: [*c][*c]u32, col_strides: [*c]const usize, nproofs: usize, ncols: usize, nv: usize, out: [*c]?*CommitJob) Status;
 pub extern "c" fn zigz_commit_roots(job: ?*CommitJob, roots: [*c]u8) Status;
 pub extern "c" fn zigz_commit_open_all(job: ?*CommitJob, points: [*c]const u64, values: [*c]u64, indices: [*c]u64, leaves: [*c]u64, siblings: [*c]u8, dirs: [*c]u8) Status;
 pub extern "c" fn zigz_commit_job_tree(job: ?*CommitJob, d_tree: [*c]?*anyopaque, bytes_per_column: [*c]usize) Status;
diff --git a/include/zigz_hip.h b/include/zigz_hip.h
--- a/include/zigz_hip.h
+++ b/include/zigz_hip.h
@@ -92,6 +92,8 @@
                                   size_t nv, zigz_commit_job **out);
 zigz_status zigz_commit_begin_batch(zigz_ctx *ctx, const uint32_t *const *d_cols, size_t nproofs, size_t ncols,
                                     size_t col_stride, size_t nv, zigz_commit_job **out);
+zigz_status zigz_commit_begin_batch_strided(zigz_ctx *ctx, const uint32_t *const *d_cols, const size_t *col_strides,
+                                            size_t nproofs, size_t ncols, size_t nv, zigz_commit_job **out);
 zigz_status zigz_commit_roots(zigz_commit_job *job, uint8_t *roots);
 zigz_status zigz_commit_open_all(zigz_commit_job *job, const uint64_t *points, uint64_t *values,
                                  uint64_t *indices, uint64_t *leaves, uint8_t *siblings, uint8_t *dirs);
diff --git a/zigz_amd/_ffi.py b/zigz_amd/_ffi.py
--- a/zigz_amd/_ffi.py
+++ b/zigz_amd/_ffi.py
@@ -87,6 +87,8 @@
     "zigz_commit_begin": (C.c_int32, [vp, u64p, C.c_size_t, C.c_size_t, C.c_size_t, C.POINTER(vp)]),
     "zigz_commit_begin_dev": (C.c_int32, [vp, vp, C.c_size_t, C.c_size_t, C.c_size_t, C.POINTER(vp)]),
     "zigz_commit_begin_batch": (C.c_int32, [vp, C.POINTER(vp), C.c_size_t, C.c_size_t, C.c_size_t, C.c_size_t, C.POINTER(vp)]),
+    "zigz_commit_begin_batch_strided": (C.c_int32, [vp, C.POINTER(vp), C.POINTER(C.c_size_t), C.c_size_t, C.c_size_t, C.c_size_t,
+                                                    C.POINTER(vp)]),
     "zigz_commit_roots": (C.c_int32, [vp, u8p]),
     "zigz_commit_open_all": (C.c_int32, [vp, u64p, u64p, u64p, u64p, u8p, u8p]),
     "zigz_commit_job_tree": (C.c_int32, [vp, C.POINTER(vp), C.POINTER(C.c_size_t)]),
diff --git a/zigz_amd/build.py b/zigz_amd/build.py
--- a/zigz_amd/build.py
+++ b/zigz_amd/build.py
@@ -60,7 +60,7 @@
         ("merkle_verify.hip", [hipcc, f"--offload-arch={ARCH}", "-O3", "-std=c++17", "-fPIC", f"-I{INC}", f"-I{CSRC}"] + extra),
         ("api.cpp", [hipcc, "-O3", "-std=c++17", "-fPIC", f"-I{INC}", f"-I{CSRC}"]),
         ("api_mle.cpp", [hipcc, "-O3", "-std=c++17", "-fPIC", f"-I{INC}", f"-I{CSRC}"]),
-        ("api_commit.cpp", [hipcc, "-O3", "-std=c++17", "-fPIC", f"-I{INC}", f"-I{CSRC}"]),
+        ("api_commit.cpp", [hipcc, "-O3", "-std=c++17", "-fPIC", f"-I{INC}", f"-I{CSRC}"] + [f for f in extra if f.startswith("-D")]),
         ("api_misc.cpp", [hipcc, "-O3", "-std=c++17", "-fPIC", f"-I{INC}", f"-I{CSRC}"]),
         ("api_batch.cpp", [hipcc, "-O3", "-std=c++17", "-fPIC", "-pthread", f"-I{INC}", f"-I{CSRC}"]),
         ("api_merkle_batch.cpp", [hipcc, "-O3", "-std=c++17", "-fPIC", "-pthread", f"-I{INC}", f"-I{CSRC}"]),
diff --git a/zigz_amd/csrc/api.cpp b/zigz_amd/csrc/api.cpp
--- a/zigz_amd/csrc/api.cpp
+++ b/zigz_amd/csrc/api.cpp
@@ -325,6 +325,7 @@
     if (strcmp(name, "cons_always") == 0) { *value = ctx->cons_always; return ZIGZ_OK; }
     if (strcmp(name, "small_domain_mask") == 0) { *value = (int64_t)ctx->small_domain_mask; return ZIGZ_OK; }
     if (strcmp(name, "verify_pause") == 0) { *value = ctx->verify_pause; return ZIGZ_OK; }
+    if (strcmp(name, "batch_workspace_bytes") == 0) { *value = (int64_t)ctx->ws_bytes[WS_BATCH]; return ZIGZ_OK; }
     return ZIGZ_ERR_INVALID_ARGUMENT;
 }
 extern "C" zigz_status zigz_ctx_set_epoch(zigz_ctx *ctx, zigz_ctx *owner) {
diff --git a/zigz_amd/csrc/api_commit.cpp b/zigz_amd/csrc/api_commit.cpp
--- a/zigz_amd/csrc/api_commit.cpp
+++ b/zigz_amd/csrc/api_commit.cpp
@@ -140,8 +140,8 @@
         top = run_top_level(npad);
         t.lists = 1;
         t.top = top;
-        b.vals = d_vals;
-        b.val_stride = val_stride;
+        b.srcs.p[0] = d_vals;
+        b.srcs.stride[0] = val_stride;
         b.n_values = n_values;
         b.npad = npad;
         b.rcols = R;
@@ -435,6 +435,7 @@
     uint64_t run_cols, run_dense, sd_cols, cons_hinted, cons_levels_nodes, cons_sd, perms0;
     unsigned nz;
     size_t ncols1, zstride;
+    ColSrcs srcs;
     size_t off_r_ctr, off_g_ctr;
     bool no_eval_skip;
 };
@@ -512,7 +513,7 @@
     return ZIGZ_OK;
 }
 
-static zigz_status job_build_batch_arena(zigz_commit_job *job, const uint32_t *const *srcs, size_t src_stride) {
+static zigz_status job_build_batch_arena(zigz_commit_job *job) {
     zigz_ctx *ctx = job->ctx;
     const size_t nc = job->ncols1, N = job->N, npad = N;
     const unsigned nz = job->nz, height = (unsigned)job->nv;
@@ -522,7 +523,6 @@
         else if ((job->m_run >> c) & 1) R.c[R.n++] = (uint8_t)c;
         else return ZIGZ_ERR_INVALID_ARGUMENT;
     }
-    const size_t stride = N;
     TreeRef t{};
     t.npad = npad;
     for (int c = 0; c < 64; c++) {
@@ -534,7 +534,9 @@
     t.top = run_top_level(npad);
     size_t at = 0;
     auto take = [&](size_t bytes) { const size_t o = at; at += align256(bytes); return o; };
-    const size_t o_cols = take(nc * stride * 4);
+#ifdef ZK_BATCH_COPY_COLS
+    const size_t o_cols = take(nc * N * 4);
+#endif
     const size_t o_rctr = take(RUN_CTR_WORDS * 8), o_gctr = take(RUN_CTR_WORDS * 8);
     size_t o_rlist = 0, o_rstage = 0, o_bitmap = 0, o_prev = 0, o_woff = 0, o_ubase = 0, o_rstore = 0;
     size_t meta_n = 0;
@@ -590,8 +592,14 @@
     }
     t.upper = a0 + o_upper;
     MerkleBuild b{};
-    b.vals = (const uint32_t *)(a0 + o_cols);
-    b.val_stride = stride;
+#ifdef ZK_BATCH_COPY_COLS
+    launch_gather_cols(job->srcs, nz, nc, N, (uint32_t *)(a0 + o_cols), N, S, ctx->stream);
+    for (unsigned z = 0; z < nz; z++) {
+        job->srcs.p[z] = (const uint32_t *)(a0 + o_cols + (size_t)z * S);
+        job->srcs.stride[z] = N;
+    }
+#endif
+    b.srcs = job->srcs;
     b.n_values = N;
     b.npad = npad;
     b.rcols = R;
@@ -623,9 +631,6 @@
     b.t = t;
     set_zstride(b, S, nz);
     t = b.t;
-    ColSrcs cs{};
-    for (unsigned z = 0; z < nz; z++) cs.p[z] = srcs[z];
-    launch_gather_cols(cs, nz, nc, N, src_stride, (uint32_t *)(a0 + o_cols), stride, S, ctx->stream);
     launch_zero_counters(nullptr, R.n ? b.r_ctr : nullptr, G.n ? b.g_ctr : nullptr, ctx->stream, nz, S);
     if (ctx->debug_skip != 2) launch_structure(b, ctx->stream, ctx->debug_skip == 0);
     for (unsigned l = 0; l <= t.top; l++)
@@ -633,8 +638,8 @@
     if (height && ctx->debug_skip != 1) launch_merkle_top(t, t.top, height, nc, ctx->stream, nullptr);
     HIPCHK(ctx, hipGetLastError());
     job->tree = t;
-    job->d_cols = (const uint32_t *)(a0 + o_cols);
-    job->col_stride = stride;
+    job->d_cols = job->srcs.p[0];
+    job->col_stride = job->srcs.stride[0];
     job->zstride = S;
     job->off_r_ctr = o_rctr;
     job->off_g_ctr = o_gctr;
@@ -657,14 +662,18 @@
     return ZIGZ_OK;
 }
 
-extern "C" zigz_status zigz_commit_begin_batch(zigz_ctx *ctx, const uint32_t *const *d_cols, size_t nproofs, size_t ncols,
-                                               size_t col_stride, size_t nv, zigz_commit_job **out) {
+extern "C" zigz_status zigz_commit_begin_batch_strided(zigz_ctx *ctx, const uint32_t *const *d_cols, const size_t *col_strides,
+                                                       size_t nproofs, size_t ncols, size_t nv, zigz_commit_job **out) {
     ZIGZ_ENTER(ctx);
-    if (!ctx || !d_cols || !out || ncols == 0 || nproofs == 0 || nproofs > BATCH_MAX || nv > 40) return ZIGZ_ERR_INVALID_ARGUMENT;
-    if (ncols * nproofs > ROOTS_MAX_COLS || col_stride < ((size_t)1 << nv)) return ZIGZ_ERR_INVALID_ARGUMENT;
-    for (size_t z = 0; z < nproofs; z++)
-        if (!d_cols[z]) return ZIGZ_ERR_INVALID_ARGUMENT;
-    if (nproofs == 1) return job_begin(ctx, d_cols[0], ncols, col_stride, nv, out);
+    if (!ctx || !d_cols || !col_strides || !out || ncols == 0 || nproofs == 0 || nproofs > BATCH_MAX || nv > 40) return ZIGZ_ERR_INVALID_ARGUMENT;
+    if (ncols * nproofs > ROOTS_MAX_COLS) return ZIGZ_ERR_INVALID_ARGUMENT;
+    ColSrcs cs{};
+    for (size_t z = 0; z < nproofs; z++) {
+        if (!d_cols[z] || col_strides[z] < ((size_t)1 << nv)) return ZIGZ_ERR_INVALID_ARGUMENT;
+        cs.p[z] = d_cols[z];
+        cs.stride[z] = col_strides[z];
+    }
+    if (nproofs == 1) return job_begin(ctx, d_cols[0], ncols, col_strides[0], nv, out);
     if (ctx->active_job) {
         set_err(ctx, "a commit job is already active on this context");
         return ZIGZ_ERR_BAD_STATE;
@@ -672,6 +681,9 @@
     const size_t N = (size_t)1 << nv;
     const bool arena = N >= RUN_MIN_LEAVES && N <= ((size_t)1 << BATCH_ARENA_MAX_NV) && ncols <= 64 && (ctx->run_aware_mask || ctx->cons_group_mask);
     if (N >= RUN_MIN_LEAVES && !arena) return ZIGZ_ERR_INVALID_ARGUMENT;
+    if (arena)
+        for (size_t z = 0; z < nproofs; z++)
+            if (!aligned16(cs.p[z]) || cs.stride[z] % 4) return ZIGZ_ERR_INVALID_ARGUMENT;
     zigz_commit_job *job = new (std::nothrow) zigz_commit_job();
     if (!job) return ZIGZ_ERR_OUT_OF_MEMORY;
     memset(job, 0, sizeof(*job));
@@ -681,20 +693,19 @@
     job->ncols = ncols * nproofs;
     job->nv = nv;
     job->N = N;
+    job->srcs = cs;
     auto body = [&]() -> zigz_status {
         HIPCHK(ctx, hipEventCreateWithFlags(&job->built, hipEventDisableTiming));
         if (arena) {
             job->m_small = 0;
             job->m_run = ctx->run_aware_mask;
             job->m_cons = ctx->cons_group_mask;
-            return job_build_batch_arena(job, d_cols, col_stride);
+            return job_build_batch_arena(job);
         }
         const size_t dstride = N < 4 ? 4 : N;
         void *d;
         CHK(ws_get(ctx, WS_COLS, (job->nz > ctx->batch_reserve ? job->nz : ctx->batch_reserve) * ncols * dstride * 4, &d));
-        ColSrcs cs{};
-        for (size_t z = 0; z < nproofs; z++) cs.p[z] = d_cols[z];
-        launch_gather_cols(cs, job->nz, ncols, N, col_stride, (uint32_t *)d, dstride, ncols * dstride * 4, ctx->stream);
+        launch_gather_cols(cs, job->nz, ncols, N, (uint32_t *)d, dstride, ncols * dstride * 4, ctx->stream);
         HIPCHK(ctx, hipGetLastError());
         job->d_cols = (const uint32_t *)d;
         job->col_stride = dstride;
@@ -711,6 +722,14 @@
     ctx->active_job = job;
     *out = job;
     return ZIGZ_OK;
+}
+
+extern "C" zigz_status zigz_commit_begin_batch(zigz_ctx *ctx, const uint32_t *const *d_cols, size_t nproofs, size_t ncols,
+                                               size_t col_stride, size_t nv, zigz_commit_job **out) {
+    if (nproofs > BATCH_MAX) return ZIGZ_ERR_INVALID_ARGUMENT;
+    size_t strides[BATCH_MAX];
+    for (size_t z = 0; z < nproofs; z++) strides[z] = col_stride;
+    return zigz_commit_begin_batch_strided(ctx, d_cols, strides, nproofs, ncols, nv, out);
 }
 
 extern "C" zigz_status zigz_commit_begin_dev(zigz_ctx *ctx, const uint32_t *d_cols, size_t ncols, size_t col_stride,
@@ -883,7 +902,7 @@
         EvalSkip skip;
         if (job->zstride) {
             skip.ncols1 = (unsigned)job->ncols1;
-            skip.z_in = job->zstride / 4;
+            skip.srcs = job->srcs;
             skip.z_changed = job->zstride / 8;
             memcpy(skip.y_of_col, job->tree.y_of_col, sizeof(skip.y_of_col));
             if (job->run_cols && !job->no_eval_skip) {
@@ -907,7 +926,7 @@
         }
         const DoneFlag done = done_flag(ctx, 1);
         launch_paths(job->tree, job->tree.npad, (unsigned)nv, job->d_cols, job->col_stride, h_idx, z_sib, z_dirs, z_leaf,
-                     job->zstride ? job->ncols1 : ncols, ctx->stream, done);
+                     job->zstride ? job->ncols1 : ncols, ctx->stream, done, job->zstride ? &job->srcs : nullptr);
         HIPCHK(ctx, hipGetLastError());
         if (!(g_sleep_wait.load() && !ctx->timing && sleep_wait(done.flag, done.seq)))
             HIPCHK(ctx, hipStreamSynchronize(ctx->stream));
diff --git a/zigz_amd/csrc/host/prover.cpp b/zigz_amd/csrc/host/prover.cpp
--- a/zigz_amd/csrc/host/prover.cpp
+++ b/zigz_amd/csrc/host/prover.cpp
@@ -500,6 +500,8 @@
         }
     }
     if (run_open) run_open_all(g);
+    std::unique_lock<std::mutex> lk(m_);
+    g->cv.wait(lk, [&] { return g->phase == 4 || g->phase < 0; });
 }
 
 Proof Prover::proveWitnessImpl(const PublicIO &io, size_t num_lookups, const Witness *witness, const uint32_t *d_cols,
diff --git a/zigz_amd/csrc/kernels.hip b/zigz_amd/csrc/kernels.hip
--- a/zigz_amd/csrc/kernels.hip
+++ b/zigz_amd/csrc/kernels.hip
@@ -249,12 +249,12 @@
     const int y = skip.y_of_col[col];
     return y >= 0 && skip.changed[z * skip.z_changed + y] == 0;
 }
-__device__ __forceinline__ size_t eval_col_off(const EvalSkip &skip, size_t col, size_t stride) {
-    if (!skip.ncols1) return col * stride;
+__device__ __forceinline__ const uint32_t *eval_col(const EvalSkip &skip, const uint32_t *in, size_t col, size_t stride) {
+    if (!skip.ncols1) return in + col * stride;
     const size_t z = col / skip.ncols1;
-    return z * skip.z_in + (col - z * skip.ncols1) * stride;
-}
-template <bool FULL>
+    return skip.srcs.p[z] + (col - z * skip.ncols1) * skip.srcs.stride[z];
+}
+template <bool FULL, bool BATCHED>
 __global__ __launch_bounds__(TPB) void k_radix_fold(const uint32_t *__restrict__ in, size_t in_stride, size_t m, size_t nb,
                                                     const uint32_t *__restrict__ w_m, size_t w_stride,
                                                     unsigned long long *__restrict__ part, size_t part_col_stride, EvalSkip skip,
@@ -264,7 +264,7 @@
     if (q * 4 >= m) return;
     const size_t col = blockIdx.z;
     if (eval_skips(skip, col)) return;
-    const uint4 *p = reinterpret_cast<const uint4 *>(in + eval_col_off(skip, col, in_stride)) + q;
+    const uint4 *p = reinterpret_cast<const uint4 *>(BATCHED ? eval_col(skip, in, col, in_stride) : in + col * in_stride) + q;
     const uint32_t *w = w_m + col * w_stride;
     const size_t mq = m / 4;
     unsigned long long lo[4] = {0, 0, 0, 0}, hi[4] = {0, 0, 0, 0};
@@ -305,8 +305,10 @@
                        hipEvent_t t_start, hipEvent_t t_stop, const EvalSkip *skip, int rloops) {
     if (rloops <= 0) rloops = RLOOPS;
     dim3 grid((unsigned)((m / 4 + TPB - 1) / TPB), (unsigned)radix_fold_groups(nb, rloops), (unsigned)ncols);
-    auto kern = nb % ((size_t)RB * rloops) == 0 ? k_radix_fold<true> : k_radix_fold<false>;
     const EvalSkip sk = skip ? *skip : EvalSkip();
+    const bool full = nb % ((size_t)RB * rloops) == 0;
+    auto kern = sk.ncols1 ? (full ? k_radix_fold<true, true> : k_radix_fold<false, true>)
+                          : (full ? k_radix_fold<true, false> : k_radix_fold<false, false>);
     if (t_start && t_stop)
         hipExtLaunchKernelGGL(kern, grid, dim3(TPB), 0, s, t_start, t_stop, 0, d_in, in_stride, m, nb, d_w_m, w_stride,
                               d_part, part_col_stride, sk, rloops);
@@ -448,7 +450,7 @@
     __shared__ unsigned long long red[TPB / 64];
     const size_t col = blockIdx.x;
     if (cols && eval_skips(skip, col)) {
-        if (threadIdx.x == 0) out[col] = cols[eval_col_off(skip, col, col_stride)];
+        if (threadIdx.x == 0) out[col] = *eval_col(skip, cols, col, col_stride);
         return;
     }
     unsigned long long acc = 0;
@@ -931,11 +933,14 @@
 
 __global__ __launch_bounds__(64) void k_paths(TreeRef t, size_t n_values, unsigned height, const uint32_t *__restrict__ vals,
                                               size_t val_stride, const uint64_t *__restrict__ idx, uint8_t *__restrict__ sib,
-                                              uint8_t *__restrict__ dirs, uint32_t *__restrict__ leaf, DoneFlag done) {
+                                              uint8_t *__restrict__ dirs, uint32_t *__restrict__ leaf, DoneFlag done, ColSrcs srcs) {
     ZK_PRIO_SMALL();
     const size_t col = blockIdx.x;
     const size_t fc = (size_t)blockIdx.z * gridDim.x + col;
-    if (t.zstride) vals += (size_t)blockIdx.z * (t.zstride / 4);
+    if (t.zstride) {
+        vals = srcs.p[blockIdx.z];
+        val_stride = srcs.stride[blockIdx.z];
+    }
     const size_t index = idx[fc];
     const unsigned l = threadIdx.x;
     if (l == 0) leaf[fc] = vals[col * val_stride + index];
@@ -958,9 +963,9 @@
 
 void launch_paths(const TreeRef &t, size_t n_values, unsigned height, const uint32_t *d_vals, size_t val_stride,
                   const uint64_t *d_idx, uint8_t *d_sib, uint8_t *d_dirs, uint32_t *d_leaf, size_t ncols, hipStream_t s,
-                  DoneFlag done) {
+                  DoneFlag done, const ColSrcs *srcs) {
     hipLaunchKernelGGL(k_paths, dim3((unsigned)ncols, 1, t.nz ? t.nz : 1), dim3(64), 0, s, t, n_values, height, d_vals, val_stride, d_idx,
-                       d_sib, d_dirs, d_leaf, done);
+                       d_sib, d_dirs, d_leaf, done, srcs ? *srcs : ColSrcs{});
 }
 TreeRef slab_tree_ref(uint8_t *d_tree, size_t npad) {
     TreeRef t{};
@@ -1073,10 +1078,9 @@
                        nz > 1 ? zstride : (size_t)0);
 }
 template <bool VEC>
-__global__ __launch_bounds__(TPB) void k_gather_cols(ColSrcs srcs, size_t n, size_t src_stride, uint32_t *__restrict__ dst, size_t dst_stride,
-                                                     size_t zstride) {
+__global__ __launch_bounds__(TPB) void k_gather_cols(ColSrcs srcs, size_t n, uint32_t *__restrict__ dst, size_t dst_stride, size_t zstride) {
     const size_t i = (size_t)blockIdx.x * TPB + threadIdx.x;
-    const uint32_t *sp = srcs.p[blockIdx.z] + (size_t)blockIdx.y * src_stride;
+    const uint32_t *sp = srcs.p[blockIdx.z] + (size_t)blockIdx.y * srcs.stride[blockIdx.z];
     uint32_t *dp = reinterpret_cast<uint32_t *>(reinterpret_cast<uint8_t *>(dst) + (size_t)blockIdx.z * zstride) + (size_t)blockIdx.y * dst_stride;
     if (VEC) {
         if (i < n / 4) reinterpret_cast<uint4 *>(dp)[i] = reinterpret_cast<const uint4 *>(sp)[i];
@@ -1084,16 +1088,16 @@
         dp[i] = sp[i];
     }
 }
-void launch_gather_cols(const ColSrcs &srcs, unsigned nz, size_t ncols, size_t n, size_t src_stride, uint32_t *d_dst,
-                        size_t dst_stride, size_t zstride, hipStream_t s) {
-    bool vec = n % 4 == 0 && src_stride % 4 == 0 && dst_stride % 4 == 0 && zstride % 16 == 0 && aligned16(d_dst);
-    for (unsigned z = 0; z < nz; z++) vec = vec && aligned16(srcs.p[z]);
+void launch_gather_cols(const ColSrcs &srcs, unsigned nz, size_t ncols, size_t n, uint32_t *d_dst, size_t dst_stride,
+                        size_t zstride, hipStream_t s) {
+    bool vec = n % 4 == 0 && dst_stride % 4 == 0 && zstride % 16 == 0 && aligned16(d_dst);
+    for (unsigned z = 0; z < nz; z++) vec = vec && aligned16(srcs.p[z]) && srcs.stride[z] % 4 == 0;
     if (vec)
         hipLaunchKernelGGL(k_gather_cols<true>, dim3((unsigned)((n / 4 + TPB - 1) / TPB), (unsigned)ncols, nz), dim3(TPB), 0, s, srcs, n,
-                           src_stride, d_dst, dst_stride, zstride);
+                           d_dst, dst_stride, zstride);
     else
         hipLaunchKernelGGL(k_gather_cols<false>, dim3((unsigned)((n + TPB - 1) / TPB), (unsigned)ncols, nz), dim3(TPB), 0, s, srcs, n,
-                           src_stride, d_dst, dst_stride, zstride);
+                           d_dst, dst_stride, zstride);
 }
 void launch_job_summary(const TreeRef &t, unsigned height, uint8_t *d_out, size_t ncols, const unsigned long long *d_r_ctr,
                         const unsigned long long *d_sd_ctr, const unsigned long long *d_g_ctr, hipStream_t s, DoneFlag done) {
diff --git a/zigz_amd/csrc/kernels.hpp b/zigz_amd/csrc/kernels.hpp
--- a/zigz_amd/csrc/kernels.hpp
+++ b/zigz_amd/csrc/kernels.hpp
@@ -73,11 +73,16 @@
 void launch_block_sums(const uint32_t *d_in, size_t in_stride, size_t n, unsigned log2_m, size_t ncols,
                        unsigned long long *d_sums, SumsLayout lay, hipStream_t s, const KTime *kt = nullptr);
 size_t radix_fold_groups(size_t nb, int rloops = 0);
+struct ColSrcs {
+    const uint32_t *p[32];
+    size_t stride[32];
+};
 struct EvalSkip {
     const unsigned long long *changed = nullptr;
     signed char y_of_col[64];
     unsigned ncols1 = 0;
-    size_t z_in = 0, z_changed = 0;
+    size_t z_changed = 0;
+    ColSrcs srcs{};
 };
 void launch_radix_fold(const uint32_t *d_in, size_t in_stride, size_t m, size_t nb, const uint32_t *d_w_m,
                        size_t w_stride, unsigned long long *d_part, size_t part_col_stride, size_t ncols, hipStream_t s,
@@ -184,8 +189,8 @@
 size_t runs_stage_scratch_bytes(size_t npad, size_t ncols);
 
 struct MerkleBuild {
-    ZPtr<const uint32_t> vals;
-    size_t val_stride, n_values, npad;
+    ColSrcs srcs;
+    size_t n_values, npad;
     TreeRef t;
     ColMap rcols;
     ZPtr<uint32_t> r_list;
@@ -207,7 +212,7 @@
     t.zstride = zs;
     t.nz = nz;
     t.slab.zs = t.upper.zs = t.bitmap.zs = t.prev.zs = t.woff.zs = t.ubase.zs = t.r_store.zs = t.g_rep.zs = t.g_store.zs = t.g_dropped.zs = zs;
-    b.vals.zs = b.r_list.zs = b.r_ctr.zs = b.r_stage.zs = b.g_keys.zs = b.g_idx.zs = b.g_rep.zs = b.g_list.zs = b.g_ctr.zs = zs;
+    b.r_list.zs = b.r_ctr.zs = b.r_stage.zs = b.g_keys.zs = b.g_idx.zs = b.g_rep.zs = b.g_list.zs = b.g_ctr.zs = zs;
 }
 void launch_runs_structure(const MerkleBuild &b, hipStream_t s, const KTime *kt = nullptr);
 void launch_cons_structure(const MerkleBuild &b, hipStream_t s, const KTime *kt = nullptr);
@@ -240,18 +245,15 @@
 void launch_publish_u32(const uint32_t *d_src, size_t n, uint32_t *h_dst, hipStream_t s, DoneFlag done);
 void launch_paths(const TreeRef &t, size_t n_values, unsigned height, const uint32_t *d_vals, size_t val_stride,
                   const uint64_t *d_idx, uint8_t *d_sib, uint8_t *d_dirs, uint32_t *d_leaf, size_t ncols, hipStream_t s,
-                  DoneFlag done = DoneFlag());
+                  DoneFlag done = DoneFlag(), const ColSrcs *srcs = nullptr);
 TreeRef slab_tree_ref(uint8_t *d_tree, size_t npad);
 void launch_gather_nodes(const uint8_t *d_tree, size_t tree_stride_nodes, size_t node, uint8_t *d_out, size_t ncols,
                          hipStream_t s);
 constexpr unsigned JOB_SUMMARY_WORDS = 8 + 2 * RUN_MAX_LEVELS;
 void launch_zero_counters(unsigned long long *d_sd_ctr, unsigned long long *d_r_ctr, unsigned long long *d_g_ctr, hipStream_t s,
                           unsigned nz = 0, size_t zstride = 0);
-struct ColSrcs {
-    const uint32_t *p[32];
-};
-void launch_gather_cols(const ColSrcs &srcs, unsigned nz, size_t ncols, size_t n, size_t src_stride, uint32_t *d_dst,
-                        size_t dst_stride, size_t zstride, hipStream_t s);
+void launch_gather_cols(const ColSrcs &srcs, unsigned nz, size_t ncols, size_t n, uint32_t *d_dst, size_t dst_stride,
+                        size_t zstride, hipStream_t s);
 void launch_job_summary(const TreeRef &t, unsigned height, uint8_t *d_out, size_t ncols, const unsigned long long *d_r_ctr,
                         const unsigned long long *d_sd_ctr, const unsigned long long *d_g_ctr, hipStream_t s,
                         DoneFlag done = DoneFlag());
diff --git a/zigz_amd/csrc/merkle_levels.hip b/zigz_amd/csrc/merkle_levels.hip
--- a/zigz_amd/csrc/merkle_levels.hip
+++ b/zigz_amd/csrc/merkle_levels.hip
@@ -7,6 +7,10 @@
 #define ZK_CONS_TPB 256
 #endif
 constexpr int CONS_TPB = ZK_CONS_TPB;
+
+__device__ __forceinline__ const uint32_t *build_col(const MerkleBuild &b, size_t col) {
+    return b.srcs.p[blockIdx.z] + col * b.srcs.stride[blockIdx.z];
+}
 
 static unsigned log2u(size_t n) { unsigned l = 0; while (((size_t)1 << l) < n) l++; return l; }
 
@@ -129,7 +133,7 @@
         const uint32_t *src;
         size_t limit;
         if (STAGE0) {
-            src = b.vals + (size_t)b.rcols.c[y] * b.val_stride + first;
+            src = build_col(b, b.rcols.c[y]) + first;
             limit = b.n_values > first ? b.n_values - first : 0;
         } else {
             src = reinterpret_cast<const uint32_t *>(b.r_stage + in_off) + (size_t)y * n_in + first;
@@ -163,7 +167,7 @@
     }
     if (STAGE0) {
         const unsigned long long inside = lane < words ? (lane == 0 ? E & ~1ull : E) : 0;
-        const uint32_t col_first = b.n_values ? b.vals[(size_t)b.rcols.c[y] * b.val_stride] : 0u;
+        const uint32_t col_first = b.n_values ? *build_col(b, b.rcols.c[y]) : 0u;
         const uint32_t seg_first = (uint32_t)__builtin_amdgcn_readfirstlane((int)fv_mine);
         if (__ballot(inside != 0) || seg_first != col_first)
             if (lane == 0) b.r_ctr[RUN_CHANGED + y] = 1;
@@ -304,12 +308,12 @@
     if (tup && b.gcols.n <= CONS_TUP) {
 #pragma unroll
         for (unsigned j = 0; j < CONS_TUP; j++) {
-            tup[j] = (j < b.gcols.n && k < b.n_values) ? b.vals[(size_t)b.gcols.c[j] * b.val_stride + k] : 0u;
+            tup[j] = (j < b.gcols.n && k < b.n_values) ? build_col(b, b.gcols.c[j])[k] : 0u;
             if (j < b.gcols.n) h = cons_mix(h ^ tup[j]);
         }
     } else {
         for (unsigned j = 0; j < b.gcols.n; j++)
-            h = cons_mix(h ^ (k < b.n_values ? b.vals[(size_t)b.gcols.c[j] * b.val_stride + k] : 0u));
+            h = cons_mix(h ^ (k < b.n_values ? build_col(b, b.gcols.c[j])[k] : 0u));
     }
     return h & ((1ull << CONS_GEN_SHIFT) - 1);
 }
@@ -444,10 +448,10 @@
             if (b.gcols.n <= CONS_TUP) {
 #pragma unroll
                 for (unsigned j = 0; j < CONS_TUP; j++)
-                    if (j < b.gcols.n && tup[j] != (rn < b.n_values ? b.vals[(size_t)b.gcols.c[j] * b.val_stride + rn] : 0u)) alone = true;
+                    if (j < b.gcols.n && tup[j] != (rn < b.n_values ? build_col(b, b.gcols.c[j])[rn] : 0u)) alone = true;
             } else {
                 for (unsigned j = 0; j < b.gcols.n; j++) {
-                    const uint32_t *v = b.vals + (size_t)b.gcols.c[j] * b.val_stride;
+                    const uint32_t *v = build_col(b, b.gcols.c[j]);
                     if ((c < b.n_values ? v[c] : 0u) != (rn < b.n_values ? v[rn] : 0u)) { alone = true; break; }
                 }
             }
@@ -630,7 +634,7 @@
             }
         }
         Digest d;
-        if (LEAF) d = sha3_leaf<PAUSE>((uint64_t)(k < b.n_values ? b.vals[col * b.val_stride + k] : 0u));
+        if (LEAF) d = sha3_leaf<PAUSE>((uint64_t)(k < b.n_values ? build_col(b, col)[k] : 0u));
         else d = sha3_node<PAUSE>(load_digest_at(in0), load_digest_at(in1));
         store_digest_at(out, d);
     }
diff --git a/zigz_amd/hip.py b/zigz_amd/hip.py
--- a/zigz_amd/hip.py
+++ b/zigz_amd/hip.py
@@ -625,13 +625,17 @@
 
 class CommitJob:
 
-    def __init__(self, ctx, cols=None, d_cols=None, ncols=NUM_COLUMNS, nv=None, col_stride=None, d_cols_list=None):
+    def __init__(self, ctx, cols=None, d_cols=None, ncols=NUM_COLUMNS, nv=None, col_stride=None, d_cols_list=None, col_strides=None):
         self.ctx = ctx
         j = vp()
         if d_cols_list is not None:
             k = len(d_cols_list)
             arr = (vp * k)(*[vp(d) for d in d_cols_list])
-            ctx.check(lib.zigz_commit_begin_batch(ctx.h, arr, k, ncols, col_stride or (1 << nv), nv, C.byref(j)))
+            if col_strides is not None:
+                st = (C.c_size_t * k)(*[int(x) for x in col_strides])
+                ctx.check(lib.zigz_commit_begin_batch_strided(ctx.h, arr, st, k, ncols, nv, C.byref(j)))
+            else:
+                ctx.check(lib.zigz_commit_begin_batch(ctx.h, arr, k, ncols, col_stride or (1 << nv), nv, C.byref(j)))
             ncols = ncols * k
         elif cols is not None:
             cols = np.ascontiguousarray(cols, dtype=np.uint64)
```

Result: slower. 2.216 billion (-3.5%).
